# Genie-Kim/PintheMemory

Hardware: AMD Instinct MI355X
Metric: train imgs/sec 768x768 bs=8 R50-DeepLabV3+ +mem (higher is better)
Workload: dtype f32

## Files before the change

include/pinmem_hip.h:

```cpp
#ifndef PINMEM_HIP_H
#define PINMEM_HIP_H
#include <stddef.h>
#include <stdint.h>

#ifdef __cplusplus
extern "C" {
#endif

typedef enum pm_status { PM_OK = 0, PM_EINVAL = -1, PM_EWORKSPACE = -2, PM_ELAUNCH = -3, PM_EUNSUPPORTED = -4 } pm_status;

typedef enum pm_dtype { PM_F32 = 0, PM_BF16 = 1 } pm_dtype;
#define PM_TF_ZERO_PAD64 1

typedef struct pm_tensor {
  void* ptr;
  int32_t n, h, w, c;
  int64_t pitch;
  int32_t dtype;
  int32_t flags;
} pm_tensor;

#define PM_ABI_VERSION 410

typedef struct pm_conv_params {
  int32_t struct_size;
  int32_t kh, kw, stride, pad, dil;
  int32_t prec;
  void* wino_v;
  int64_t wino_v_bytes;
  void* wxf;
  int64_t wxf_bytes;
  int32_t wxf_valid;
} pm_conv_params;

typedef struct pm_conv_epilogue {
  int64_t struct_size;
  const float* bias;
  const float* scale;
  const float* shift;
  const float* residual;
  int64_t residual_pitch;
  int32_t relu;
  float* bn_partials;
  int64_t bn_partials_bytes;
} pm_conv_epilogue;

const char* pm_last_error(void);
int pm_version(void);

size_t pm_conv_workspace(const pm_tensor* x, const pm_tensor* y, const pm_conv_params* p, int which );
size_t pm_conv_winograd_v_bytes(const pm_tensor* x, const pm_tensor* y, const pm_conv_params* p);
size_t pm_conv_wxf_bytes(const pm_tensor* x, const pm_tensor* y, const pm_conv_params* p);
size_t pm_conv_wxf_bytes_dgrad(const pm_tensor* dy, const pm_tensor* dx, const pm_conv_params* p);
typedef struct pm_wxf_job {
  const float* w;
  void* wxf;
  int64_t wxf_bytes;
  int32_t cout, kh, kw, cin;
  int32_t dgrad;
  int32_t reserved;
} pm_wxf_job;
int pm_conv_wxf_refresh_bf16(const pm_wxf_job* jobs, int n, void* stream);
int pm_conv_wxf_refresh_f32(const pm_wxf_job* jobs, int n, void* stream);
size_t pm_conv_bn_partials_bytes(const pm_tensor* x, const pm_tensor* y, const pm_conv_params* p);
int pm_conv_fwd(const pm_tensor* x, const float* w_krsc, const pm_tensor* y, const pm_conv_params* p,
                const pm_conv_epilogue* ep, void* ws, size_t ws_bytes, void* stream);
int pm_conv_bwd_data(const pm_tensor* dy, const float* w_krsc, const pm_tensor* dx, const pm_conv_params* p,
                     const pm_tensor* add, void* ws, size_t ws_bytes, void* stream);
int pm_conv_bwd_data_masked(const pm_tensor* dy, const float* w_krsc, const pm_tensor* dx, const pm_conv_params* p,
                            const pm_tensor* add, const uint8_t* add_mask, void* ws, size_t ws_bytes, void* stream);
int pm_conv_bwd_weight(const pm_tensor* x, const pm_tensor* dy, float* dw_krsc, float* dbias, const pm_conv_params* p,
                       void* ws, size_t ws_bytes, void* stream);

typedef struct pm_routing {
  int32_t struct_size;
  int32_t winograd;
  int32_t winograd_fused;
  int32_t conv16;
  int32_t conv16_wide;
  int32_t conv16_persistent;
  int32_t wgrad16;
  int32_t bf16_wgrad;
  int32_t split;
} pm_routing;
int pm_routing_get(pm_routing* out);
int pm_routing_set(const pm_routing* r);


int pm_set_winograd(int mode);
int pm_set_winograd_fused(int on);
int pm_set_conv16(int on);
int pm_set_bf16_wgrad(int on);
int pm_set_wgrad16(int on);
int pm_set_split(int on);

int pm_profile_enable(int on);
int pm_profile_dump(const char* csv_path);
int pm_profile_read(int mode, int bm, int bn, int km, int nst, double* total_ms, double* total_flops, int64_t* launches, int clear);
int pm_profile_read_prec(int mode, int bm, int bn, int km, int nst, int prec, double* total_ms, double* total_flops, int64_t* launches, int clear);
int pm_profile_read_bytes(int mode, int bm, int bn, int km, int nst, int prec, double* total_bytes);

size_t pm_bn_workspace(const pm_tensor* x);
int pm_bn_stats(const pm_tensor* x, float* moments, void* ws, size_t ws_bytes, void* stream);
int pm_bn_stats_finalize(const pm_tensor* x, float eps, float* mean, float* invstd, float* running_mean , float* running_var ,
                         float momentum, void* ws, size_t ws_bytes, void* stream);
int pm_bn_merge(const float* parts, int world, int c, float* moments, void* stream);
int pm_bn_merge_finalize(const float* parts, int world, int c, float eps, float* mean, float* invstd, float* running_mean ,
                         float* running_var , float momentum, void* stream);
int pm_bn_finalize(const float* moments, int c, float eps, float* mean, float* invstd,
                   float* running_mean, float* running_var, float momentum, void* stream);
int pm_bn_apply(const pm_tensor* x, const float* mean, const float* invstd, const float* gamma, const float* beta,
                const pm_tensor* residual , int relu, const pm_tensor* y, void* stream);
int pm_bn_apply_mask(const pm_tensor* x, const float* mean, const float* invstd, const float* gamma, const float* beta,
                     const pm_tensor* residual , int relu, const pm_tensor* y, uint8_t* mask , void* stream);
int pm_bn_bwd_reduce_mask(const pm_tensor* dy, const uint8_t* mask, const pm_tensor* x, const float* mean, const float* invstd,
                          const pm_tensor* gmask , float* sums, void* ws, size_t ws_bytes, void* stream);
int pm_bn_apply_mask_affine(const pm_tensor* x, const float* mean, const float* invstd, const float* gamma, const float* beta,
                            const pm_tensor* r, const float* r_mean, const float* r_invstd, const float* r_gamma, const float* r_beta,
                            int relu, const pm_tensor* y, uint8_t* mask , void* stream);
int pm_bn_bwd_apply_mask(const pm_tensor* dy, const uint8_t* mask, const pm_tensor* x, const float* mean, const float* invstd, const float* gamma,
                         const float* sums, float count, const pm_tensor* dx, void* stream);
int pm_bn_bwd_reduce(const pm_tensor* dy, const pm_tensor* y , const pm_tensor* x, const float* mean, const float* invstd,
                     const float* gamma , const float* beta , int relu, const pm_tensor* gmask ,
                     float* sums, void* ws, size_t ws_bytes, void* stream);
int pm_bn_bwd_apply(const pm_tensor* dy, const pm_tensor* y , const pm_tensor* x, const float* mean, const float* invstd,
                    const float* gamma, const float* beta , const float* sums, float count, int relu, const pm_tensor* dx,
                    const pm_tensor* dres , void* stream);
int pm_bn_partials_finalize(const float* partials, int64_t pixels, int c, float eps, float* mean, float* invstd, float* running_mean ,
                            float* running_var , float momentum, float* moments , void* stream);
int pm_bn_fold(const float* gamma, const float* beta, const float* running_mean, const float* running_var, const float* conv_bias,
               int c, float eps, float* scale, float* shift, void* stream);
int pm_bn_fold_multi(const void* table, const int* cs, const int* offs, int n, int max_c, int total, float eps, float* arena, void* stream);
int pm_relu_bwd(const pm_tensor* dy, const pm_tensor* y, const pm_tensor* dx, void* stream);
int pm_add(const pm_tensor* a, const pm_tensor* b, const pm_tensor* y, void* stream);
int pm_add_n(const pm_tensor* const* xs, int n, const pm_tensor* y, void* stream);
int pm_copy(const pm_tensor* src, const pm_tensor* dst, void* stream);
int pm_scale_shift_act(const pm_tensor* x, const float* scale, const float* shift, const pm_tensor* residual, int relu,
                       const pm_tensor* y, void* stream);

int pm_cast(const pm_tensor* x, const pm_tensor* y, void* stream);

int pm_maxpool3x3s2_fwd(const pm_tensor* x, const pm_tensor* y, uint8_t* argmax, void* stream);
int pm_maxpool3x3s2_bwd(const pm_tensor* dy, const uint8_t* argmax, const pm_tensor* dx, void* stream);
int pm_maxpool3x3s2_bn_relu_fwd(const pm_tensor* x, const float* mean, const float* invstd, const float* gamma, const float* beta, const pm_tensor* y,
                                uint8_t* argmax, void* stream);
int pm_bn_bwd_reduce_pool(const pm_tensor* dy_pooled, const uint8_t* argmax, const pm_tensor* x, const float* mean, const float* invstd, const float* gamma,
                          const float* beta, float* sums, void* ws, size_t ws_bytes, void* stream);
int pm_bn_bwd_apply_pool(const pm_tensor* dy_pooled, const uint8_t* argmax, const pm_tensor* x, const float* mean, const float* invstd, const float* gamma,
                         const float* beta, const float* sums, float count, const pm_tensor* dx, void* stream);
int pm_global_avgpool_fwd(const pm_tensor* x, const pm_tensor* y , void* stream);
int pm_global_avgpool_bwd(const pm_tensor* dy, const pm_tensor* dx, int accumulate, void* stream);

int pm_resize_bilinear_fwd(const pm_tensor* x, const pm_tensor* y, void* stream);
int pm_resize_bilinear_bwd(const pm_tensor* dy, const pm_tensor* dx, int accumulate, void* stream);
size_t pm_resize_bilinear_bwd_workspace(const pm_tensor* dy, const pm_tensor* dx);
int pm_resize_bilinear_bwd_separable(const pm_tensor* dy, const pm_tensor* dx, int accumulate, void* ws, size_t ws_bytes, void* stream);

int pm_resize_bilinear_hp_fwd(const pm_tensor* x, const pm_tensor* y, int flip_w, void* stream);
int pm_softmax_mean_update(const pm_tensor* logits, double* buffer, int counter, void* stream);
int pm_sliding_stitch(const pm_tensor* logits, const int32_t* tiles_xyxy, int ntiles, int H, int W, int flip_w, double* acc, int accumulate, void* stream);
int pm_argmax_f64(const double* buffer, int n, int h, int w, int c, int64_t* out_cls, double* out_prob , void* stream);

int pm_image_u8_to_nhwc4(const uint8_t* img_nhw3, int64_t pixels, const float* mean3, const float* std3, float* out_nhwc4, void* stream);
int pm_labels_u8_to_i64(const uint8_t* lab, int64_t n, int64_t* out, void* stream);

typedef struct pm_aug_image {
  uint8_t order[4];
  uint8_t enabled;
  uint8_t flip;
  uint8_t hue_shift;
  uint8_t reserved;
  float brightness, contrast, saturation;
  int32_t radius;
  double w[6];
} pm_aug_image;
int pm_aug_blur_weights(double sigma, int32_t* radius, double* w6);
size_t pm_augment_workspace(int n);
int pm_augment_u8(const uint8_t* img_nhw3, int n, int H, int W, const pm_aug_image* params_dev, int32_t struct_size, const float* mean3, const float* std3,
                  float* out_nhwc4, uint8_t* out_u8, void* ws, size_t ws_bytes, void* stream);
int pm_labels_u8_flip_to_i64(const uint8_t* lab, int n, int H, int W, const pm_aug_image* params_dev, int32_t struct_size, int64_t* out, void* stream);

int pm_nchw_to_nhwc(const float* x_nchw, int c_src, const pm_tensor* y, void* stream);
int pm_nhwc_to_nchw(const pm_tensor* x, float* y_nchw, void* stream);
int pm_label_nearest(const int64_t* lab, int n, int H, int W, int64_t* out, int h, int w, void* stream);

// ... 69 lines not shown
```

pinthememory_amd/csrc/conv_igemm.hip:

```cpp
#include <stdlib.h>
#include <algorithm>
#include <type_traits>
#include <vector>

#include "pm_common.h"

#include "conv_igemm_kernel.h"

namespace {

template <int ZL, bool O16 = false>
__global__ __launch_bounds__(256) void splitk_reduce_vec_kernel(const float* __restrict__ ws, int ksplit, long slab, int M, int Nn,
                                                                float* __restrict__ C, long c_pitch, const float* bias,
                                                                const float* scale, const float* shift, const float* residual,
                                                                long res_pitch, int relu, const unsigned char* res_mask) {
  constexpr int GP = 256 / ZL;
  __shared__ float4 red[ZL > 1 ? ZL : 1][GP];
  const int gl = threadIdx.x % GP, zl = threadIdx.x / GP;
  const long groups = (long)M * Nn / 4;
  for (long g0 = (long)blockIdx.x * GP; g0 < groups; g0 += (long)gridDim.x * GP) {
    const long grp = g0 + gl;
    float4 v = make_float4(0.f, 0.f, 0.f, 0.f);
    if (grp < groups)
#pragma unroll 8
// ... 268 lines not shown
constexpr int NST1_MAX_STEPS = 64;
constexpr bool has_nst1(int mode, int kmode, int bn) { return mode != MODE_WGRAD && kmode == K_FAST && bn >= 64; }
inline int lds_stages(int mode, int kmode, int bn, int kper) { return has_nst1(mode, kmode, bn) && kper <= NST1_MAX_STEPS * BK ? 1 : 2; }
template <int MODE, int BM, int BN, int WM, int WN, int KM, int PREC>
void launch_prec(const ConvK& k, dim3 grid, size_t smem, hipStream_t st) {
  if constexpr (has_nst1(MODE, KM, BN)) {
    if (lds_stages(MODE, KM, BN, k.kper) == 1) return launch_nst<MODE, BM, BN, WM, WN, KM, PREC, 1>(k, grid, smem, st);
  }
  launch_nst<MODE, BM, BN, WM, WN, KM, PREC, 2>(k, grid, smem, st);
}
template <int MODE, int BM, int BN, int WM, int WN, int KM>
void launch_inst(const ConvK& k, dim3 grid, size_t smem, hipStream_t st) {
  if constexpr (MODE == MODE_FWD && KM == K_FAST && BN >= 64) {
    if (k.prec == 2) return launch_prec<MODE, BM, BN, WM, WN, KM, 2>(k, grid, smem, st);
  }
  if constexpr (MODE == MODE_WGRAD && BN >= 64) {
    if (k.prec == 3) return launch_prec<MODE, BM, BN, WM, WN, KM, 3>(k, grid, smem, st);
    if (k.prec == 4) return launch_prec<MODE, BM, BN, WM, WN, KM, 4>(k, grid, smem, st);
  }
  if (k.prec != 0) launch_prec<MODE, BM, BN, WM, WN, KM, 1>(k, grid, smem, st);
  else launch_prec<MODE, BM, BN, WM, WN, KM, 0>(k, grid, smem, st);
}
template <int MODE, int BM, int BN, int WM, int WN>
void launch_one(const ConvK& k, dim3 grid, size_t smem, hipStream_t st) {
  if (k.kmode == K_SMALL) launch_inst<MODE, BM, BN, WM, WN, K_SMALL>(k, grid, smem, st);
  else if (k.kmode == K_FAST && MODE != MODE_WGRAD) launch_inst<MODE, BM, BN, WM, WN, (MODE != MODE_WGRAD ? K_FAST : K_MID)>(k, grid, smem, st);
  else launch_inst<MODE, BM, BN, WM, WN, K_MID>(k, grid, smem, st);
}

struct ProfRec {
  hipEvent_t a, b;
  int mode, bm, bn, km, prec, nst;
  int M, Nn, K, batch, ksplit;
  double flops;
  double bytes;
};
bool g_prof_on = false;
std::vector<ProfRec> g_prof;
struct ProfScope {
  ProfRec rec{};
  hipStream_t st;
  ProfScope(hipStream_t st_, int mode, int bm, int bn, int km, int prec, int nst, long M, long Nn, long K, int batch, int ksplit, double flops, double bytes = 0.0) : st(st_) {
    if (!g_prof_on) return;
    (void)hipEventCreate(&rec.a), (void)hipEventCreate(&rec.b);
    rec.mode = mode, rec.bm = bm, rec.bn = bn, rec.km = km, rec.prec = prec, rec.nst = nst, rec.M = (int)M, rec.Nn = (int)Nn, rec.K = (int)K, rec.batch = batch, rec.ksplit = ksplit;
    rec.flops = flops, rec.bytes = bytes;
    (void)hipEventRecord(rec.a, st);
  }
  void done() {
    if (!g_prof_on) return;
    (void)hipEventRecord(rec.b, st);
    g_prof.push_back(rec);
  }
};

template <class K>
void set_epilogue(K& k, const pm_conv_epilogue& e) {
  k.bias = e.bias, k.scale = e.scale, k.shift = e.shift, k.residual = e.residual, k.res_pitch = e.residual_pitch, k.relu = e.relu;
}
inline void set_epilogue(ConvK& k, const pm_conv_epilogue& e, const unsigned char* res_mask) {
  set_epilogue(k, e);
  k.res_mask = res_mask, k.stats = e.bn_partials;
}
inline bool split_takes(int mode, const Plan& p, const ConvK& k, int batch) {
  return pm_route.split != 0 && p.bn >= 64 && !k.io16 && (batch > 1 || split_k_ok(mode, k.K));
}

template <int MODE>
int launch(const ConvK& k0, const Plan& p, hipStream_t st, int batch = 1, double flops = -1.0) {
  ConvK k = k0;
  k.tiles_m = p.tiles_m;
  k.tiles_n = p.tiles_n;
  k.ksplit = p.ksplit;
  k.kper = p.kper;
  dim3 grid(p.tiles_m * p.tiles_n, batch, p.ksplit);
  if (batch != 1) k.stage_ep = 0;
  if (k.prec == 0 && split_takes(MODE, p, k, batch)) k.prec = 5;
  {
    const int units = batch * p.ksplit, rem = units & 7, ntile = p.tiles_m * p.tiles_n;
    k.batch_xcd = units >= 8 && (rem == 0 || ((rem == 1 || rem == 2 || rem == 4) && ntile % (8 / rem) == 0));
  }
  const int km = (MODE == MODE_WGRAD && k.kmode == K_FAST) ? K_MID : ((k.prec == 5 && MODE != MODE_WGRAD && k.kmode == K_FAST && k.kh * k.kw == 1 && k.stride == 1 && k.pad == 0 && !k.sub) ? K_PW : k.kmode);
  ProfScope prof(st, MODE, p.bm, p.bn, km, k.prec, lds_stages(MODE, k.kmode, p.bn, k.kper), k.M, k.Nn, k.K, batch, p.ksplit,
                 flops >= 0.0 ? flops : 2.0 * (double)k.M * (double)k.Nn * (double)k.K * batch,
                 (double)batch * ((double)k.a_bytes + (double)k.b_bytes + ((k.io16 && p.ksplit == 1) ? 2.0 : 4.0) * (double)k.M * (double)k.Nn * (double)p.ksplit));
  if constexpr (MODE != MODE_WGRAD) {
    if (pm_route.split && (k.prec == 0 || k.prec == 5) && !k.io16 && batch == 1 && p.ksplit == 1 && !k.stats && k.kh * k.kw == 1 && k.stride == 1 && k.pad == 0 && !k.sub) {
      pm_gemm_pw g;
      g.A = k.A, g.B = k.B, g.C = k.C, g.res_mask = k.res_mask;
      set_epilogue(g, pm_conv_epilogue{(int64_t)sizeof(pm_conv_epilogue), k.bias, k.scale, k.shift, k.residual, k.res_pitch, k.relu, nullptr, 0});
      g.a_pitch = MODE == MODE_FWD ? k.x_pitch : k.y_pitch, g.c_pitch = k.c_pitch;
      g.b_sn = MODE == MODE_FWD ? k.K : 1, g.b_sk = MODE == MODE_FWD ? 1 : k.Nn;
      g.M = k.M, g.Nn = k.Nn, g.K = k.K;
      if (pm_pwstream_ok(&g)) {
        prof.rec.bm = 32, prof.rec.bn = 64, prof.rec.km = 4, prof.rec.prec = 5, prof.rec.nst = 0;
        const int e = pm_pwstream_launch(&g, st);
        prof.done();
        return e;
      }
    }
  }
  constexpr bool akc = MODE != MODE_WGRAD, bkc = MODE == MODE_FWD;
  if (k.prec == 5) {
    if (int e = pm_conv_split_launch(MODE, p.bm, p.bn, k, grid.x, grid.y, grid.z, pm_conv_split_stage_bytes(MODE, p.bm, p.bn), st)) return e;
    prof.rec.nst = 1;
    prof.done();
    return pm_check_launch("conv_split");
  }
  const bool tr = MODE == MODE_WGRAD && (k.prec == 3 || k.prec == 4) && p.bn >= 64;
  auto smem = [&](int bm, int bn) {
    if (tr) return (size_t)2 * ((k.prec == 4 ? 2 : 1) * BK * (bm + 32) + (k.prec == 4 ? 2 : 1) * BK * (bn + 32)) * 2;
    return (size_t)2 * ((akc ? bm * LDK : BK * bm) + (bkc ? bn * LDK : BK * bn)) * sizeof(float);
  };
  if (p.bm == 64) {
    if (p.bn == 128) launch_one<MODE, 64, 128, 2, 2>(k, grid, smem(64, 128), st);
    else launch_one<MODE, 64, 64, 2, 2>(k, grid, smem(64, 64), st);
  } else if (p.bn == 128) {
    launch_one<MODE, 128, 128, 2, 2>(k, grid, smem(128, 128), st);
  } else if (p.bn == 64) {
    launch_one<MODE, 128, 64, 2, 2>(k, grid, smem(128, 64), st);
  } else {
    launch_one<MODE, 128, 32, 4, 1>(k, grid, smem(128, 32), st);
  }
  prof.done();
  return pm_check_launch("conv_igemm");
}

template <int MODE>
int run_gemm(ConvK& k, const Plan& pl, float* slab, float* out, long out_pitch, const pm_conv_epilogue& e, hipStream_t st, double flops = -1.0,
             const unsigned char* res_mask = nullptr) {
  return run_planned(pl.ksplit, k.M, k.Nn, slab, out, out_pitch, e, k.io16 != 0, res_mask, st, [&](float* C, bool slabs) {
    k.C = C, k.c_pitch = slabs ? k.Nn : out_pitch, k.c_split = slabs ? (long)k.M * k.Nn : 0;
    if (!slabs) set_epilogue(k, e, res_mask);
    return launch<MODE>(k, pl, st, 1, flops);
  });
}

int check_common(const pm_tensor* x, const pm_tensor* y, const pm_conv_params* p) {
  PM_REQUIRE(x && y && p && x->ptr && y->ptr, PM_EINVAL, "conv: null tensor");
  PM_REQUIRE(p->struct_size == (int32_t)sizeof(pm_conv_params), PM_EINVAL, "conv: pm_conv_params.struct_size %d != %zu -- caller built against another pinmem_hip.h (library ABI %d)",
             p->struct_size, sizeof(pm_conv_params), PM_ABI_VERSION);
  PM_REQUIRE(p->kh >= 1 && p->kw >= 1 && p->dil >= 1 && p->pad >= 0, PM_EINVAL, "conv: bad geometry");
  PM_REQUIRE(p->stride == 1 || p->stride == 2, PM_EUNSUPPORTED, "conv: stride %d unsupported (1 or 2)", p->stride);
  const int ho = (x->h + 2 * p->pad - p->dil * (p->kh - 1) - 1) / p->stride + 1;
  const int wo = (x->w + 2 * p->pad - p->dil * (p->kw - 1) - 1) / p->stride + 1;
  PM_REQUIRE(ho == y->h && wo == y->w && x->n == y->n, PM_EINVAL, "conv: output %dx%d does not match geometry (%dx%d)", y->h, y->w, ho, wo);
  PM_REQUIRE((x->dtype == PM_F32 || x->dtype == PM_BF16) && (y->dtype == PM_F32 || y->dtype == PM_BF16), PM_EUNSUPPORTED, "conv: dtype %d / %d", x->dtype, y->dtype);
  for (const pm_tensor* t : {x, y}) {
    if (pm_is_bf16(t)) PM_REQUIRE(pm_vec8(t), PM_EINVAL, "conv: bf16 tensors must be 16B aligned with pitch %% 8 == 0 and channels %% 8 == 0");
    else PM_REQUIRE(pm_vec_ok(t), PM_EINVAL, "conv: tensors must be 16B aligned with pitch %% 4 == 0");
  }
  PM_REQUIRE(x->c % 4 == 0, PM_EUNSUPPORTED, "conv: Cin %% 4 != 0 unsupported (pad the input channels)");
  PM_REQUIRE((y->c % 4 == 0) || (p->kh * p->kw == 1), PM_EUNSUPPORTED, "conv: Cout %% 4 != 0 only for 1x1");
  PM_REQUIRE(x->pitch >= x->c && y->pitch >= y->c, PM_EINVAL, "conv: pitch < channels");
  PM_REQUIRE(pm_pixels(x) * x->pitch < (1ll << 29) && pm_pixels(y) * y->pitch < (1ll << 29) && (int64_t)y->c * x->c * p->kh * p->kw < (1ll << 29),
             PM_EUNSUPPORTED, "conv: tensor too large for 32-bit byte offsets (2 GiB per tensor)");
  return PM_OK;
}

void fill_geom(ConvK& k, const pm_tensor* x, const pm_tensor* y, const pm_conv_params* p) {
  k.N = x->n, k.H = x->h, k.W = x->w, k.Cin = x->c, k.x_pitch = x->pitch;
  k.Ho = y->h, k.Wo = y->w, k.Cout = y->c, k.y_pitch = y->pitch;
  k.kh = p->kh, k.kw = p->kw, k.stride = p->stride, k.pad = p->pad, k.dil = p->dil;
  k.sshift = p->stride == 2 ? 1 : 0;
  k.prec = p->prec != 0 ? 1 : 0;
  k.T_eff = p->kh * p->kw, k.tk_w = p->kw, k.ky0 = k.kx0 = 0, k.ksy = k.ksx = 1;
  k.sub = k.sub_cy = k.sub_cx = 0, k.Hc = x->h, k.Wc = x->w;
  k.bias = k.scale = k.shift = k.residual = nullptr;
  k.res_pitch = 0, k.res_mask = nullptr, k.relu = 0, k.stats = nullptr, k.io16 = 0;
  k.stage_ep = 1;
  k.spl_prio = 1;
  k.n_group = 8;
  k.batch_xcd = 0;
  k.a_bs = k.b_bs = k.c_bs = 0;
}

struct WinoPlan {
  bool use;
  pm_wino_geom g;
  int Kp, P;
  size_t v_bytes, m_bytes, u_bytes;
  Plan pl;
};
inline bool wino_wgrad_pays(int cin, int cout) { return (long)cin * cout >= 256 * 256; }
WinoPlan wino_plan(const pm_tensor* xin, int cout, const pm_conv_params* p, bool wgrad = false) {
  WinoPlan wp{};
  if (wgrad && !wino_wgrad_pays(xin->c, cout)) return wp;
  if (pm_route.winograd == 0 || p->kh != 3 || p->kw != 3 || p->stride != 1 || p->pad != p->dil || p->prec != 0) return wp;
  const int cin = xin->c;
  if (cin < 128 || cout < 128 || (cout & 3) || (cin & 3)) return wp;
  int m = 0;
  double best_ratio = 0.6;
  for (int cand = pm_route.winograd; cand >= 2; cand -= 2) {
    const pm_wino_geom g = pm_wino_make_geom(xin->n, xin->h, xin->w, p->dil, cand);
    const double cover = (double)(cand * g.TY * p->dil) * (double)(cand * g.TX * p->dil) / ((double)xin->h * xin->w);
    const double ratio = cover * (cand + 2) * (cand + 2) / (9.0 * cand * cand);
    if (ratio <= best_ratio) best_ratio = ratio, m = cand, wp.g = g;
  }
  if (!m) return wp;
  wp.P = (m + 2) * (m + 2);
  wp.Kp = (cin + BK - 1) / BK * BK;
  if (wp.g.tiles * (long)std::max(wp.Kp, cout) * 4 >= (1ll << 31)) return wp;
  wp.v_bytes = pm_align_up((size_t)wp.P * wp.g.tiles * wp.Kp * sizeof(float), 256);
  wp.m_bytes = pm_align_up((size_t)wp.P * wp.g.tiles * cout * sizeof(float), 256);
  wp.u_bytes = pm_align_up((size_t)wp.P * cout * wp.Kp * sizeof(float), 256);
  wp.pl.bm = 128, wp.pl.bn = 128;
  if (pm_cdiv(cout, 128) * 128 > cout * 1.12 && pm_cdiv(cout, 64) * 64 < pm_cdiv(cout, 128) * 128) wp.pl.bn = 64;
  if (wp.g.tiles <= 4608 && !pm_route.split) wp.pl.bm = 64;
  wp.pl.tiles_m = pm_cdiv(wp.g.tiles, wp.pl.bm), wp.pl.tiles_n = pm_cdiv(cout, wp.pl.bn);
  wp.pl.ksplit = 1, wp.pl.kper = wp.Kp, wp.pl.ws_bytes = 0;
  wp.use = true;
  return wp;
}
inline size_t wino_ws(const WinoPlan& wp) { return wp.v_bytes + wp.m_bytes + wp.u_bytes; }

int wino_conv(const pm_tensor* xin, const float* w, int w_cout, int w_cin, bool dgrad, const pm_tensor* yout, const WinoPlan& wp,
              const pm_conv_epilogue& ep, void* ws, hipStream_t st, float* v_keep = nullptr, float* u_ext = nullptr, bool u_valid = false) {
  float* V = v_keep ? v_keep : (float*)ws;
  float* Mo = (float*)((char*)ws + wp.v_bytes);
  float* U = u_ext ? u_ext : (float*)((char*)ws + wp.v_bytes + wp.m_bytes);
  const int cout = yout->c;
  if (int e = pm_wino_input_xf((const float*)xin->ptr, xin->pitch, xin->c, wp.Kp, wp.g, V, st)) return e;
  if (!(u_ext && u_valid))
    if (int e = pm_wino_filter_xf(w, w_cout, w_cin, wp.Kp, dgrad, wp.g.m, U, st)) return e;
  const pm_tensor xv = {V, 1, 1, (int32_t)wp.g.tiles, wp.Kp, wp.Kp};
  const pm_tensor yv = {Mo, 1, 1, (int32_t)wp.g.tiles, cout, cout};
  const pm_conv_params p1 = {(int32_t)sizeof(pm_conv_params), 1, 1, 1, 0, 1, 0};
  ConvK k;
  fill_geom(k, &xv, &yv, &p1);
  k.A = V, k.B = U, k.C = Mo;
  k.M = (int)wp.g.tiles, k.Nn = cout, k.K = wp.Kp;
  k.a_bytes = (unsigned)(wp.g.tiles * wp.Kp * 4), k.b_bytes = (unsigned)((long)cout * wp.Kp * 4), k.kmode = K_FAST;
  k.c_pitch = cout, k.c_split = 0;
  k.a_bs = wp.g.tiles * wp.Kp, k.b_bs = (long)cout * wp.Kp, k.c_bs = wp.g.tiles * cout;
  if (pm_route.winograd_fused && wp.g.m == 4 && wp.Kp % 16 == 0) {
    ProfScope prof(st, 3, 32, 32, 0, 0, 1, wp.g.tiles, cout, wp.Kp, wp.P, 1, 2.0 * wp.P * (double)wp.g.tiles * cout * xin->c);
    const int e = pm_wino_fused_f4(V, U, cout, wp.Kp, wp.g, (float*)yout->ptr, yout->pitch, ep.bias, ep.scale, ep.shift, ep.residual, ep.residual_pitch, ep.relu, st);
    prof.done();
    return e;
  }
  if (int e = launch<MODE_FWD>(k, wp.pl, st, wp.P, 2.0 * wp.P * (double)wp.g.tiles * cout * xin->c)) return e;
  return pm_wino_output_xf(Mo, cout, wp.g, (float*)yout->ptr, yout->pitch, ep.bias, ep.scale, ep.shift, ep.residual, ep.residual_pitch, ep.relu, st);
}

struct WinoWgradPlan {
  Plan pl;
  size_t slab_bytes;
};
WinoWgradPlan wino_wgrad_plan(const WinoPlan& wp, int cout) {
  WinoWgradPlan q{};
  q.pl.bm = 128, q.pl.bn = 128;
  if (pm_cdiv(wp.Kp, 128) * 128 > wp.Kp * 1.12 && pm_cdiv(wp.Kp, 64) * 64 < pm_cdiv(wp.Kp, 128) * 128) q.pl.bn = 64;
  q.pl.tiles_m = pm_cdiv(cout, 128), q.pl.tiles_n = pm_cdiv(wp.Kp, q.pl.bn);
  const long ksteps = (wp.g.tiles + BK - 1) / BK;
  const long per_split = (long)q.pl.tiles_m * q.pl.tiles_n * wp.P;
  long ks = std::max<long>(1, std::min<long>((768 + per_split / 2) / per_split, ksteps / 8));
  const long steps_per = (ksteps + ks - 1) / ks;
  ks = (ksteps + steps_per - 1) / steps_per;
  q.pl.ksplit = (int)ks, q.pl.kper = (int)(steps_per * BK), q.pl.ws_bytes = 0;
  q.slab_bytes = pm_align_up((size_t)ks * wp.P * cout * wp.Kp * sizeof(float), 256);
  return q;
}
inline size_t wino_wgrad_ws(const WinoPlan& wp, const WinoWgradPlan& q) { return wp.v_bytes + wp.m_bytes + q.slab_bytes; }

int wino_wgrad(const pm_tensor* x, const pm_tensor* dy, float* dw, const WinoPlan& wp, const WinoWgradPlan& q, void* ws, hipStream_t st,
               float* v_kept = nullptr) {
  float* V = v_kept ? v_kept : (float*)ws;
  float* Z = (float*)((char*)ws + wp.v_bytes);
  float* slab = (float*)((char*)ws + wp.v_bytes + wp.m_bytes);
  const int cout = dy->c;
  if (!v_kept)
    if (int e = pm_wino_input_xf((const float*)x->ptr, x->pitch, x->c, wp.Kp, wp.g, V, st)) return e;
  if (int e = pm_wino_dy_xf((const float*)dy->ptr, dy->pitch, cout, wp.g, Z, st)) return e;
  const pm_tensor xv = {V, 1, 1, (int32_t)wp.g.tiles, wp.Kp, wp.Kp};
  const pm_tensor zv = {Z, 1, 1, (int32_t)wp.g.tiles, cout, cout};
  const pm_conv_params p1 = {(int32_t)sizeof(pm_conv_params), 1, 1, 1, 0, 1, 0};
  ConvK k;
  fill_geom(k, &xv, &zv, &p1);
  k.A = Z, k.B = V, k.C = slab;
  k.M = cout, k.Nn = wp.Kp, k.K = (int)wp.g.tiles;
  k.a_bytes = (unsigned)(wp.g.tiles * cout * 4), k.b_bytes = (unsigned)(wp.g.tiles * wp.Kp * 4), k.kmode = K_MID;
  k.c_pitch = wp.Kp, k.c_split = (long)wp.P * cout * wp.Kp;
  k.a_bs = wp.g.tiles * cout, k.b_bs = wp.g.tiles * wp.Kp, k.c_bs = (long)cout * wp.Kp;
  if (int e = launch<MODE_WGRAD>(k, q.pl, st, wp.P, 2.0 * wp.P * (double)wp.g.tiles * cout * x->c)) return e;
  return pm_wino_dw_xf(slab, q.pl.ksplit, cout, x->c, wp.Kp, wp.g.m, dw, st);
}

struct Bf16Plan {
  bool use;
  bool c16;
  pm_conv16 k16;
  bool inplace;
  int Cp;
  long M, Nn, Kf;
  size_t xb_bytes, wb_bytes;
  Plan pl;
};
Bf16Plan bf16_plan(const pm_tensor* xin, const pm_tensor* yout, const pm_conv_params* p) {
  Bf16Plan b{};
  if ((p->prec != 2 && !pm_is_bf16(xin) && !pm_is_bf16(yout)) || xin->c < 32) return b;
  b.Cp = (xin->c + 63) / 64 * 64;
  const long T = (long)p->kh * p->kw;
  b.M = pm_pixels(yout), b.Nn = yout->c, b.Kf = T * b.Cp / 2;
  b.inplace = pm_is_bf16(xin) && (xin->c % 64 == 0 || ((xin->flags & PM_TF_ZERO_PAD64) && xin->pitch >= b.Cp));
  const size_t xb = b.inplace ? (size_t)pm_pixels(xin) * xin->pitch * 2 : (size_t)pm_pixels(xin) * b.Cp * 2, wb = (size_t)yout->c * T * b.Cp * 2;
  if (xb >= (1ull << 31) || wb >= (1ull << 31)) return b;
  b.xb_bytes = b.inplace ? 0 : pm_align_up(xb, 256), b.wb_bytes = pm_align_up(wb, 256);
  b.pl = make_plan(MODE_FWD, b.M, b.Nn, b.Kf, true);
  if (b.pl.bn < 64) return b;
  b.use = true;
  constexpr long C16_MIN_M = 256;
  b.c16 = false;
  if (pm_route.conv16 && b.M >= C16_MIN_M && p->stride >= 1) {
    pm_conv16& k = b.k16;
    k = pm_conv16{};
    k.N = xin->n, k.H = xin->h, k.W = xin->w, k.Ho = yout->h, k.Wo = yout->w;
    k.a_pitch = b.inplace ? xin->pitch : b.Cp, k.Cp = b.Cp;
    k.kh = p->kh, k.kw = p->kw, k.stride = p->stride, k.pad = p->pad, k.dil = p->dil;
    k.M = (int)b.M, k.Nn = (int)b.Nn, k.K = (int)(T * b.Cp), k.ksteps = k.K / 64;
    k.c_pitch = yout->pitch, k.c_f32 = pm_is_bf16(yout) ? 0 : 1;
    pm_conv16_plan(&k);
    b.c16 = pm_route.conv16 == 2 || k.wide || k.bm == 64 || k.ksteps_per == 1 || (b.pl.bm == 64 && k.ksteps >= 16);
  }
  return b;
}
inline size_t bf16_ws(const Bf16Plan& b) {
  return b.xb_bytes + b.wb_bytes + std::max(pm_align_up(b.pl.ws_bytes, 256), b.c16 ? pm_conv16_slab_bytes(&b.k16) : (size_t)0);
}

int conv_bf16(const pm_tensor* xin, const float* w, int w_cout, int w_cin, bool rotate, const pm_tensor* yout, const pm_conv_params* pe, const Bf16Plan& b,
              const pm_conv_epilogue& e0, void* ws, hipStream_t st, char* wb_ext = nullptr, bool wb_valid = false) {
  char* xb = b.inplace ? (char*)xin->ptr : (char*)ws;
  char* wb = wb_ext ? wb_ext : (char*)ws + b.xb_bytes;
  float* slab = (float*)((char*)ws + b.xb_bytes + b.wb_bytes);
  const int T = pe->kh * pe->kw;
  if (!b.inplace) {
    if (pm_is_bf16(xin)) {
      if (int e = pm16_pad_rows((const pm_bf16*)xin->ptr, xin->pitch, xin->c, b.Cp, pm_pixels(xin), (pm_bf16*)xb, st)) return e;
    } else if (int e = pm_bf16_cast_rows((const float*)xin->ptr, xin->pitch, xin->c, b.Cp, pm_pixels(xin), xb, st)) return e;
  }
  if (!(wb_ext && wb_valid))
    if (int e = pm_bf16_cast_weights(w, w_cout, T, w_cin, b.Cp, rotate, wb, st)) return e;
  const long xpitch16 = b.inplace ? xin->pitch : b.Cp;
  if (b.c16) {
    const bool o16 = pm_is_bf16(yout);
    const bool ok = (!e0.bn_partials || o16) &&
                    (o16 ? ((yout->c | yout->pitch | (e0.residual ? e0.residual_pitch : 0)) & 7) == 0 && pm_aligned16(yout->ptr) && pm_aligned16(e0.residual)
                         : !(e0.scale || e0.residual || e0.relu));
    if (ok) {
      pm_conv16 k = b.k16;
      k.A = (const pm_bf16*)xb, k.B = (const pm_bf16*)wb;
      const double fl = 2.0 * (double)b.M * (double)b.Nn * (double)T * (double)xin->c * (g_prof_on ? pm_conv16_executed_fraction(&k) : 1.0);
      ProfScope prof(st, k.wide ? 5 : 4, k.bm, k.bn, pm_conv16w_persistent(&k), 5, k.wide ? 3 : (k.ksteps_per == 1 ? 1 : 2), k.M, k.Nn, k.K / 2, 1, k.ksplit, fl);
      return run_planned(k.ksplit, b.M, b.Nn, slab, (float*)yout->ptr, (long)yout->pitch, e0, o16, nullptr, st, [&](float* C, bool slabs) {
        k.C = C;
        if (!slabs) set_epilogue(k, e0), k.stats = o16 ? e0.bn_partials : nullptr;
        const int e = pm_conv16_launch(&k, st);
        prof.done();
        return e;
      });
    }
  }
  const pm_tensor xv = {xb, xin->n, xin->h, xin->w, b.Cp / 2, xpitch16 / 2};
  ConvK k;
  fill_geom(k, &xv, yout, pe);
  k.prec = 2;
  k.A = (const float*)xb, k.B = (const float*)wb;
  k.M = (int)b.M, k.Nn = (int)b.Nn, k.K = (int)b.Kf;
  k.a_bytes = (unsigned)((size_t)pm_pixels(xin) * xpitch16 * 2), k.b_bytes = (unsigned)((size_t)yout->c * T * b.Cp * 2), k.kmode = K_FAST;
  const double flops = 2.0 * (double)b.M * (double)b.Nn * (double)T * (double)xin->c;
  k.io16 = pm_is_bf16(yout) ? 1 : 0;
  return run_gemm<MODE_FWD>(k, b.pl, slab, (float*)yout->ptr, (long)yout->pitch, e0, st, flops);
}
inline pm_conv_params dgrad_as_fwd(const pm_conv_params* p) {
  pm_conv_params q = *p;
// ... 356 lines not shown
  *out = pm_route;
  return PM_OK;
}
extern "C" int pm_routing_set(const pm_routing* r) {
  PM_REQUIRE(r && r->struct_size == (int32_t)sizeof(pm_routing), PM_EINVAL, "pm_routing_set: struct_size %d != %zu (library ABI %d)", r ? r->struct_size : -1, sizeof(pm_routing),
             PM_ABI_VERSION);
  PM_REQUIRE(r->winograd == 0 || r->winograd == 2 || r->winograd == 4, PM_EINVAL, "pm_routing_set: winograd %d (0, 2 or 4)", r->winograd);
  PM_REQUIRE(r->conv16 >= 0 && r->conv16 <= 2 && r->conv16_wide >= 0 && r->conv16_wide <= 3, PM_EINVAL, "pm_routing_set: conv16 %d / conv16_wide %d", r->conv16, r->conv16_wide);
  pm_route = *r;
  return PM_OK;
}
extern "C" int pm_set_winograd(int mode) {
  PM_REQUIRE(mode == 0 || mode == 2 || mode == 4, PM_EINVAL, "pm_set_winograd: mode %d (0 off, 2 F(2x2,3x3), 4 prefer F(4x4,3x3))", mode);
  pm_route.winograd = mode;
  return PM_OK;
}
extern "C" int pm_set_conv16(int on) {
  PM_REQUIRE(on >= 0 && on <= 8, PM_EINVAL, "pm_set_conv16: %d (0 register-staged, 1 per shape, 2 LDS-DMA everywhere / narrow tiles only, 3 LDS-DMA everywhere / wide tiles "
             "wherever the shape allows, 4 per shape without the wide kernel, 5 / 6 = 1 (the streaming 1x1 kernel left the library in round 6), 7 as 3 with the 256 x 256 tile, "
             "8 as 3 with one block per tile instead of the persistent ring)", on);
  pm_route.conv16 = (on == 3 || on == 7 || on == 8) ? 2 : ((on == 4 || on == 5 || on == 6) ? 1 : on);
  pm_route.conv16_wide = (on == 3 || on == 8) ? 2 : (on == 7 ? 3 : ((on == 2 || on == 4) ? 0 : pm_route_defaults.conv16_wide));
  pm_route.conv16_persistent = on == 8 ? 0 : (on == 3 ? 1 : pm_route_defaults.conv16_persistent);
  return PM_OK;
}
extern "C" int pm_set_winograd_fused(int on) {
  pm_route.winograd_fused = on != 0;
  return PM_OK;
}
extern "C" int pm_set_wgrad16(int on) {
  pm_route.wgrad16 = on != 0;
  return PM_OK;
}
extern "C" int pm_set_split(int on) {
  pm_route.split = on ? 1 : 0;
  return PM_OK;
}
extern "C" int pm_set_bf16_wgrad(int on) {
  pm_route.bf16_wgrad = on != 0;
  return PM_OK;
}
extern "C" int pm_profile_enable(int on) {
  g_prof_on = on != 0;
  return PM_OK;
}
extern "C" int pm_profile_read_prec(int mode, int bm, int bn, int km, int nst, int prec, double* total_ms, double* total_flops, int64_t* launches, int clear);
extern "C" int pm_profile_read(int mode, int bm, int bn, int km, int nst, double* total_ms, double* total_flops, int64_t* launches, int clear) {
  return pm_profile_read_prec(mode, bm, bn, km, nst, -1, total_ms, total_flops, launches, clear);
}
extern "C" int pm_profile_read_prec(int mode, int bm, int bn, int km, int nst, int prec, double* total_ms, double* total_flops, int64_t* launches, int clear) {
  double ms = 0.0, fl = 0.0;
  int64_t n = 0;
  for (const ProfRec& r : g_prof) {
    if ((mode >= 0 && r.mode != mode) || (bm >= 0 && r.bm != bm) || (bn >= 0 && r.bn != bn) || (km >= 0 && r.km != km) || (nst >= 0 && r.nst != nst) ||
        (prec >= 0 && r.prec != prec))
      continue;
    float t = 0.f;
    if (hipEventSynchronize(r.b) != hipSuccess || hipEventElapsedTime(&t, r.a, r.b) != hipSuccess) continue;
    ms += t, fl += r.flops, ++n;
  }
  if (clear) {
    for (const ProfRec& r : g_prof) (void)hipEventDestroy(r.a), (void)hipEventDestroy(r.b);
    g_prof.clear();
  }
  if (total_ms) *total_ms = ms;
  if (total_flops) *total_flops = fl;
  if (launches) *launches = n;
  return PM_OK;
}

extern "C" int pm_profile_read_bytes(int mode, int bm, int bn, int km, int nst, int prec, double* total_bytes) {
  double b = 0.0;
  for (const ProfRec& r : g_prof) {
    if ((mode >= 0 && r.mode != mode) || (bm >= 0 && r.bm != bm) || (bn >= 0 && r.bn != bn) || (km >= 0 && r.km != km) || (nst >= 0 && r.nst != nst) ||
        (prec >= 0 && r.prec != prec))
      continue;
    b += r.bytes;
  }
  if (total_bytes) *total_bytes = b;
  return PM_OK;
}

extern "C" int pm_profile_dump(const char* path) {
  PM_REQUIRE(path, PM_EINVAL, "pm_profile_dump: null path");
  FILE* f = fopen(path, "w");
  PM_REQUIRE(f, PM_EINVAL, "pm_profile_dump: cannot open %s", path);
  fprintf(f, "mode,bm,bn,km,nst,prec,M,N,K,batch,ksplit,ms,gflop\n");
  for (const ProfRec& r : g_prof) {
    float t = 0.f;
    if (hipEventSynchronize(r.b) != hipSuccess || hipEventElapsedTime(&t, r.a, r.b) != hipSuccess) continue;
    fprintf(f, "%d,%d,%d,%d,%d,%d,%d,%d,%d,%d,%d,%.5f,%.4f\n", r.mode, r.bm, r.bn, r.km, r.nst, r.prec, r.M, r.Nn, r.K, r.batch, r.ksplit, t, r.flops * 1e-9);
  }
  fclose(f);
  return PM_OK;
}

extern "C" size_t pm_conv_workspace(const pm_tensor* x, const pm_tensor* y, const pm_conv_params* p0, int which) {
  const pm_conv_params tp = tier_params(p0, x, y);
  return route_conv(which, x, y, &tp).ws_bytes;
}
extern "C" size_t pm_conv_winograd_v_bytes(const pm_tensor* x, const pm_tensor* y, const pm_conv_params* p0) {
  if (!x || !y || !p0) return 0;
  const pm_conv_params tp = tier_params(p0, x, y);
  return route_conv(MODE_FWD, x, y, &tp).v_keep_bytes;
}
extern "C" size_t pm_conv_wxf_bytes(const pm_tensor* x, const pm_tensor* y, const pm_conv_params* p0) {
  if (!x || !y || !p0) return 0;
  const pm_conv_params tp = tier_params(p0, x, y);
  return route_conv(MODE_FWD, x, y, &tp).wxf_bytes;
}
extern "C" size_t pm_conv_wxf_bytes_dgrad(const pm_tensor* dy, const pm_tensor* dx, const pm_conv_params* p0) {
  if (!dy || !dx || !p0) return 0;
  const pm_conv_params tp = tier_params(p0, dy, dx);
  return route_conv(MODE_DGRAD, dx, dy, &tp).wxf_bytes;
}
extern "C" size_t pm_conv_bn_partials_bytes(const pm_tensor* x, const pm_tensor* y, const pm_conv_params* p0) {
  if (!x || !y || !p0 || check_common(x, y, p0) != PM_OK) return 0;
  const pm_conv_params tp = tier_params(p0, x, y);
  return route_conv(MODE_FWD, x, y, &tp).bn_bytes;
}

extern "C" int pm_conv_wxf_refresh_f32(const pm_wxf_job* jobs, int n, void* stream) {
  PM_REQUIRE(n >= 0 && (jobs || n == 0), PM_EINVAL, "conv_wxf_refresh_f32: bad job table");
  std::vector<const float*> w(n);
  std::vector<float*> U(n);
  std::vector<int> cout(n), cin(n), kp(n), m(n);
  for (int i = 0; i < n; ++i) {
    const pm_wxf_job& q = jobs[i];
    PM_REQUIRE(q.w && q.wxf && q.cout > 0 && q.cin > 0 && q.kh == 3 && q.kw == 3 && q.dgrad == 0, PM_EINVAL,
               "conv_wxf_refresh_f32: job %d: forward transforms of 3x3 filters only", i);
    PM_REQUIRE(pm_aligned16(q.wxf), PM_EINVAL, "conv_wxf_refresh_f32: job %d: buffer must be 16-byte aligned", i);
    const int Kp = (q.cin + BK - 1) / BK * BK;
    const size_t u4 = pm_align_up((size_t)36 * q.cout * Kp * sizeof(float), 256), u2 = pm_align_up((size_t)16 * q.cout * Kp * sizeof(float), 256);
    PM_REQUIRE((size_t)q.wxf_bytes == u4 || (size_t)q.wxf_bytes == u2, PM_EINVAL, "conv_wxf_refresh_f32: job %d: %ld bytes is neither the F(4x4) nor the F(2x2) transform of %d x %d",
               i, (long)q.wxf_bytes, q.cout, q.cin);
    w[i] = q.w, U[i] = (float*)q.wxf, cout[i] = q.cout, cin[i] = q.cin, kp[i] = Kp, m[i] = (size_t)q.wxf_bytes == u4 ? 4 : 2;
  }
  return pm_wino_filter_xf_multi(w.data(), U.data(), cout.data(), cin.data(), kp.data(), m.data(), n, (hipStream_t)stream);
}

extern "C" int pm_conv_fwd(const pm_tensor* x, const float* w, const pm_tensor* y, const pm_conv_params* p0,
                           const pm_conv_epilogue* ep, void* ws, size_t ws_bytes, void* stream) {
  if (int e = check_common(x, y, p0)) return e;
  const pm_conv_params tp = tier_params(p0, x, y);
  const pm_conv_params* p = &tp;
  PM_REQUIRE(!ep || ep->struct_size == (int64_t)sizeof(pm_conv_epilogue), PM_EINVAL,
             "conv_fwd: pm_conv_epilogue.struct_size %ld != %zu -- caller built against another pinmem_hip.h (library ABI %d)", ep ? (long)ep->struct_size : 0l,
             sizeof(pm_conv_epilogue), PM_ABI_VERSION);
  PM_REQUIRE(w && pm_aligned16(w), PM_EINVAL, "conv_fwd: weight null or unaligned");
  pm_conv_epilogue e0 = {(int64_t)sizeof(pm_conv_epilogue), nullptr, nullptr, nullptr, nullptr, 0, 0};
  if (ep) e0 = *ep;
  PM_REQUIRE((e0.scale == nullptr) == (e0.shift == nullptr), PM_EINVAL, "conv_fwd: scale and shift go together");
  const ConvRoute r = route_conv(MODE_FWD, x, y, p);
  if (e0.bn_partials) {
    PM_REQUIRE(!e0.relu && !e0.residual, PM_EINVAL, "conv_fwd: bn_partials are the statistics of the convolution output (no residual / ReLU)");
    PM_REQUIRE(r.bn_bytes != 0 && (size_t)e0.bn_partials_bytes >= r.bn_bytes, PM_EINVAL, "conv_fwd: this call cannot emit bn_partials (ask pm_conv_bn_partials_bytes): %zu needed", r.bn_bytes);
  }
  PM_REQUIRE(ws_bytes >= r.ws_bytes && (ws || r.ws_bytes == 0), PM_EWORKSPACE, "conv_fwd: workspace %zu < %zu", ws_bytes, r.ws_bytes);
  hipStream_t st = (hipStream_t)stream;
  switch (r.kind) {
    case R_WINO: {
      float* keep = (p->wino_v && (size_t)p->wino_v_bytes >= r.wino.v_bytes) ? (float*)p->wino_v : nullptr;
      float* uext = (p->wxf && (size_t)p->wxf_bytes >= r.wino.u_bytes) ? (float*)p->wxf : nullptr;
      return wino_conv(x, w, y->c, x->c, false, y, r.wino, e0, ws, st, keep, uext, p->wxf_valid != 0);
    }
    case R_BF16: {
      char* wext = (p->wxf && (size_t)p->wxf_bytes >= r.b16.wb_bytes) ? (char*)p->wxf : nullptr;
      return conv_bf16(x, w, y->c, x->c, false, y, &r.pe, r.b16, e0, ws, st, wext, p->wxf_valid != 0);
    }
    default:
      PM_REQUIRE(pm_is_f32(x), PM_EUNSUPPORTED, "conv_fwd: a bf16 input needs at least 32 channels (got %d)", x->c);
      return conv_direct<MODE_FWD>(x, y, w, p, r.pl, e0, ws, st);
  }
}

extern "C" int pm_conv_bwd_data(const pm_tensor* dy, const float* w, const pm_tensor* dx, const pm_conv_params* p0, const pm_tensor* add,
                                void* ws, size_t ws_bytes, void* stream) {
  return pm_conv_bwd_data_masked(dy, w, dx, p0, add, nullptr, ws, ws_bytes, stream);
}

extern "C" int pm_conv_bwd_data_masked(const pm_tensor* dy, const float* w, const pm_tensor* dx, const pm_conv_params* p0, const pm_tensor* add,
                                       const uint8_t* add_mask, void* ws, size_t ws_bytes, void* stream) {
  if (int e = check_common(dx, dy, p0)) return e;
  const pm_conv_params tp = tier_params(p0, dy, dx);
  const pm_conv_params* p = &tp;
  PM_REQUIRE(!add || (add->ptr && pm_same_shape(add, dx) && add->dtype == dx->dtype), PM_EINVAL, "conv_bwd_data: `add` must match dx (shape and dtype)");
  PM_REQUIRE(!add || !pm_is_bf16(add) || pm_vec8(add), PM_EINVAL, "conv_bwd_data: bf16 `add` must be 16B aligned with pitch %% 8 == 0");
  PM_REQUIRE(w && pm_aligned16(w), PM_EINVAL, "conv_bwd_data: weight null or unaligned");
  const ConvRoute r = route_conv(MODE_DGRAD, dx, dy, p);
  PM_REQUIRE(ws_bytes >= r.ws_bytes && (ws || r.ws_bytes == 0), PM_EWORKSPACE, "conv_bwd_data: workspace %zu < %zu", ws_bytes, r.ws_bytes);
  if (add_mask) {
    PM_REQUIRE(add && pm_is_f32(add) && pm_is_f32(dy) && pm_vec4(add) && pm_vec4(dx), PM_EINVAL, "conv_bwd_data: a masked `add` is an fp32 tensor with 16-byte rows and c %% 4 == 0");
    PM_REQUIRE(r.kind == R_DIRECT, PM_EUNSUPPORTED,
               "conv_bwd_data: a masked `add` is served by the fp32 implicit-GEMM route only (this call routes to %s)",
               r.kind == R_WINO ? "Winograd" : (r.kind == R_BF16 ? "the bf16 kernels" : "the stride-2 class kernels"));
  }
  hipStream_t st = (hipStream_t)stream;
  const pm_conv_epilogue e1 = {(int64_t)sizeof(pm_conv_epilogue), nullptr, nullptr, nullptr, add ? (const float*)add->ptr : nullptr, add ? add->pitch : 0, 0};
  switch (r.kind) {
    case R_S2_NATIVE: return dgrad_s2_bf16(dy, w, dx, p, add, r.s2n, ws, st);
    case R_S2_PARITY: return dgrad_s2_parity(dy, w, dx, p, add, r, ws, st);
    case R_BF16: {
      char* wext = (p->wxf && (size_t)p->wxf_bytes >= r.b16.wb_bytes) ? (char*)p->wxf : nullptr;
      return conv_bf16(dy, w, dy->c, dx->c, true, dx, &r.pe, r.b16, e1, ws, st, wext, p->wxf_valid != 0);
    }
    case R_WINO: return wino_conv(dy, w, dy->c, dx->c, true, dx, r.wino, e1, ws, st);
    default:
      PM_REQUIRE(pm_is_f32(dy), PM_EUNSUPPORTED, "conv_bwd_data: a bf16 dy needs at least 32 channels and a stride-1 geometry the forward form covers");
      return conv_direct<MODE_DGRAD>(dx, dy, w, p, r.pl, e1, ws, st, add_mask);
  }
}

extern "C" int pm_conv_bwd_weight(const pm_tensor* x0, const pm_tensor* dy0, float* dw, float* dbias, const pm_conv_params* p0, void* ws,
                                  size_t ws_bytes, void* stream) {
  if (int e = check_common(x0, dy0, p0)) return e;
  const pm_conv_params tp = tier_params(p0, x0, dy0);
  const pm_conv_params* p = &tp;
  PM_REQUIRE(dw && pm_aligned16(dw), PM_EINVAL, "conv_bwd_weight: dw null or unaligned");
  const ConvRoute r = route_conv(MODE_WGRAD, x0, dy0, p);
  PM_REQUIRE(ws && ws_bytes >= r.ws_bytes, PM_EWORKSPACE, "conv_bwd_weight: workspace %zu < %zu", ws_bytes, r.ws_bytes);
  hipStream_t st = (hipStream_t)stream;
  const pm_tensor *x = x0, *dy = dy0;
  pm_tensor x32, dy32;
  if (!r.native16 && pm_is_bf16(x0)) {
    if (int e = upcast(x0, (char*)ws + r.x32_off, &x32, st)) return e;
    x = &x32;
  }
  if (pm_is_bf16(dy0) && (!r.native16 || dbias)) {
    if (int e = upcast(dy0, (char*)ws + r.dy32_off, &dy32, st)) return e;
    if (!r.native16) dy = &dy32;
  }
  int e;
  switch (r.kind) {
    case R_BF16_WGRAD: e = conv_wgrad_bf16(x, dy, dw, p, r.b16w, ws, st); break;
    case R_WINO_WGRAD: e = wino_wgrad(x, dy, dw, r.wino, r.wino_w, ws, st, (p->wino_v && (size_t)p->wino_v_bytes >= r.wino.v_bytes) ? (float*)p->wino_v : nullptr); break;
    default: e = conv_wgrad_direct(x, dy, dw, p, r, ws, st);
  }
  if (e || !dbias) return e;
  const pm_tensor* dyb = pm_is_bf16(dy0) ? &dy32 : dy0;
  const long P = pm_pixels(dyb);
  const int rpb = colsum_rows(P, dyb->c), nb = pm_cdiv(P, rpb);
  float* part = (float*)((char*)ws + r.bias_off);
  if (dyb->pitch == ((dyb->c + 3) & ~3) && dyb->pitch <= 64 && pm_aligned16(dyb->ptr))
    hipLaunchKernelGGL(colsum_partial_narrow_kernel, dim3(nb), dim3(256), 0, st, (const float*)dyb->ptr, (int)(dyb->pitch / 4), P, dyb->c, rpb, part);
  else
    hipLaunchKernelGGL(colsum_partial_kernel, dim3(nb, pm_cdiv(dyb->c, 64)), dim3(256), 0, st, (const float*)dyb->ptr, (long)dyb->pitch, P, dyb->c, rpb, part);
  hipLaunchKernelGGL(colsum_final_kernel, dim3(pm_cdiv(dyb->c, 64)), dim3(1024), 0, st, (const float*)part, nb, dyb->c, dbias);
  return pm_check_launch("conv_bias_grad");
}
```

pinthememory_amd/csrc/pm_common.h:

```cpp
#pragma once
#include <hip/hip_runtime.h>
#include <algorithm>
#include <atomic>
#include <stdarg.h>
#include <stdint.h>
#include <stdio.h>

#include "../../include/pinmem_hip.h"

void pm_set_error(const char* fmt, ...);

#define PM_REQUIRE(cond, code, ...)      \
  do {                                   \
    if (!(cond)) {                       \
      pm_set_error(__VA_ARGS__);         \
      return (code);                     \
    }                                    \
  } while (0)

static inline int pm_check_launch(const char* what) {
  hipError_t e = hipGetLastError();
  if (e != hipSuccess) {
    pm_set_error("%s: launch failed: %s", what, hipGetErrorString(e));
    return PM_ELAUNCH;
  }
  return PM_OK;
}

static inline bool pm_aligned16(const void* p) { return (reinterpret_cast<uintptr_t>(p) & 15u) == 0; }
static inline int64_t pm_pixels(const pm_tensor* t) { return (int64_t)t->n * t->h * t->w; }
static inline int pm_cdiv(int64_t a, int64_t b) { return (int)((a + b - 1) / b); }
static inline size_t pm_align_up(size_t v, size_t a) { return (v + a - 1) / a * a; }

static inline bool pm_vec_ok(const pm_tensor* t) { return pm_aligned16(t->ptr) && (t->pitch % 4) == 0; }
static inline bool pm_is_f32(const pm_tensor* t) { return t->dtype == PM_F32; }
static inline bool pm_is_bf16(const pm_tensor* t) { return t->dtype == PM_BF16; }
#define PM_REQUIRE_F32(t, who) PM_REQUIRE(!(t) || pm_is_f32(t), PM_EUNSUPPORTED, "%s: fp32 tensors only (got dtype %d)", who, (t)->dtype)
static inline bool pm_vec8(const pm_tensor* t) { return pm_is_bf16(t) && pm_aligned16(t->ptr) && (t->pitch % 8) == 0 && (t->c % 8) == 0; }

struct pm_wino_geom {
  int N, H, W, d, m, TY, TX;
  long tiles;
};
pm_wino_geom pm_wino_make_geom(int n, int h, int w, int d, int m);
int pm_wino_input_xf(const float* x, long pitch, int C, int Kp, const pm_wino_geom& g, float* V, hipStream_t st);
int pm_wino_filter_xf(const float* w, int Cout, int Cin, int Kp, bool dgrad, int m, float* U, hipStream_t st);
int pm_wino_filter_xf_multi(const float* const* w, float* const* U, const int* cout, const int* cin, const int* kp, const int* m, int n, hipStream_t st);
int pm_wino_output_xf(const float* M, int Cout, const pm_wino_geom& g, float* y, long ypitch, const float* bias, const float* scale, const float* shift,
                      const float* residual, long res_pitch, int relu, hipStream_t st);
int pm_wino_fused_f4(const float* V, const float* U, int Cout, int Kp, const pm_wino_geom& g, float* y, long ypitch, const float* bias, const float* scale,
                     const float* shift, const float* residual, long res_pitch, int relu, hipStream_t st);
int pm_wino_dy_xf(const float* dy, long pitch, int Cout, const pm_wino_geom& g, float* Z, hipStream_t st);
int pm_wino_dw_xf(const float* slab, int ks, int Cout, int Cin, int Kp, int m, float* dw, hipStream_t st);

int pm_bf16_cast_rows(const float* x, long pitch, int C, int Cp, long P, void* out, hipStream_t st);
int pm_bf16_cast_weights(const float* w, int Cout, int T, int Cin, int Cp, bool rotate, void* out, hipStream_t st);
struct PmS2Classes {
  int ky0[4], nky[4], kx0[4], nkx[4];
  void* out[4];
};
int pm_bf16_cast_weights_s2(const float* w, int Cout, int kh, int kw, int Cin, int Cp, const PmS2Classes* cl, hipStream_t st);
int pm_bf16_transpose_taps(const float* x, long pitch, int C, int N, int H, int W, int Ho, int Wo, int kh, int kw, int stride, int pad, int dil, void* out,
                           hipStream_t st);

typedef unsigned short pm_bf16;
int pm16_to_f32(const pm_bf16* x, long pitch, int C, long P, float* out, long out_pitch, hipStream_t st);
int pm16_pad_rows(const pm_bf16* x, long pitch, int C, int Cp, long P, pm_bf16* out, hipStream_t st);

struct pm_conv16 {
  const pm_bf16* A;
  const pm_bf16* B;
  void* C;
  int N, H, W, Ho, Wo;
  long a_pitch;
  int Cp;
  int kh, kw, stride, pad, dil;
  int M, Nn, K, ksteps;
  long c_pitch;
  int c_f32;
  const float *bias, *scale, *shift;
  const void* residual;
  long res_pitch;
  int relu;
  float* stats;
  int bm, bn, tiles_m, tiles_n, ksplit, ksteps_per;
  long c_split;
  int wide;
};
void pm_conv16_plan(pm_conv16* k);
int pm_conv16w_launch(const pm_conv16* k, hipStream_t st);
int pm_conv16w_persistent(const pm_conv16* k);
size_t pm_conv16_slab_bytes(const pm_conv16* k);
double pm_conv16_executed_fraction(const pm_conv16* k);
int pm_conv16_launch(const pm_conv16* k, hipStream_t st);

struct pm_wgrad16 {
  const pm_bf16* X;
  const pm_bf16* DY;
  float* C;
  int N, H, W, Ho, Wo;
  long x_pitch, dy_pitch;
  int Cin, Cout, kh, kw, stride, pad, dil;
  int M, Nn, P;
  int kper, ksplit;
  long c_split;
  int bm, bn, tiles_m, tiles_n;
};
bool pm_wgrad16_plan(pm_wgrad16* k);
int pm_wgrad16_launch(const pm_wgrad16* k, hipStream_t st);

struct pm_gemm_pw {
  const float* A;
  const float* B;
  float* C;
  const float *bias, *scale, *shift, *residual;
  const unsigned char* res_mask;
  long a_pitch, c_pitch, res_pitch;
  int b_sn, b_sk;
  long M;
  int Nn, K, relu;
};
bool pm_pwstream_ok(const pm_gemm_pw* g);
int pm_pwstream_launch(const pm_gemm_pw* g, hipStream_t st);

constexpr int PM_MAX_DEVICES = 64;
inline int pm_device_cus(int dev) {
  static std::atomic<int> cached[PM_MAX_DEVICES];
  const bool keep = dev >= 0 && dev < PM_MAX_DEVICES;
  int n = keep ? cached[dev].load(std::memory_order_relaxed) : 0;
  if (n > 0) return n;
  if (hipDeviceGetAttribute(&n, hipDeviceAttributeMultiprocessorCount, dev) != hipSuccess || n <= 0) n = 256;
  if (keep) cached[dev].store(n, std::memory_order_relaxed);
  return n;
}
struct pm_lds_optin {
  std::atomic<bool> done[PM_MAX_DEVICES] = {};
  int operator()(const void* kernel, int lds_bytes) {
    int dev = 0;
    if (hipGetDevice(&dev) != hipSuccess) dev = 0;
    const bool keep = dev >= 0 && dev < PM_MAX_DEVICES;
    if (!keep || !done[dev].load(std::memory_order_acquire)) {
      if (hipFuncSetAttribute(kernel, hipFuncAttributeMaxDynamicSharedMemorySize, lds_bytes) != hipSuccess) (void)hipGetLastError();
      else if (keep) done[dev].store(true, std::memory_order_release);
    }
    return pm_device_cus(dev);
  }
};

extern pm_routing pm_route;


__device__ __forceinline__ int pm_xcd_remap(int bid, int nwg) {
  const int q = nwg >> 3, r = nwg & 7, xcd = bid & 7, idx = bid >> 3;
  const int base = xcd < r ? xcd * (q + 1) : r * (q + 1) + (xcd - r) * q;
  return base + idx;
}
__device__ __forceinline__ void pm_ld8(const pm_bf16* p, float* v) {
  const uint4 q = *reinterpret_cast<const uint4*>(p);
  v[0] = __uint_as_float(q.x << 16), v[1] = __uint_as_float(q.x & 0xffff0000u), v[2] = __uint_as_float(q.y << 16), v[3] = __uint_as_float(q.y & 0xffff0000u);
  v[4] = __uint_as_float(q.z << 16), v[5] = __uint_as_float(q.z & 0xffff0000u), v[6] = __uint_as_float(q.w << 16), v[7] = __uint_as_float(q.w & 0xffff0000u);
}
__device__ __forceinline__ unsigned pm_pack_bf16(float a, float b) {
  typedef __bf16 bf16x2_t __attribute__((ext_vector_type(2)));
  bf16x2_t o;
  o[0] = (__bf16)a, o[1] = (__bf16)b;
  return __builtin_bit_cast(unsigned, o);
}
__device__ __forceinline__ void pm_st8(pm_bf16* p, const float* v) {
  uint4 q;
  q.x = pm_pack_bf16(v[0], v[1]), q.y = pm_pack_bf16(v[2], v[3]), q.z = pm_pack_bf16(v[4], v[5]), q.w = pm_pack_bf16(v[6], v[7]);
  *reinterpret_cast<uint4*>(p) = q;
}
__device__ __forceinline__ float pm_bf16_to_f32(pm_bf16 h) { return __uint_as_float((unsigned)h << 16); }
__device__ __forceinline__ pm_bf16 pm_f32_to_bf16(float f) { return __builtin_bit_cast(unsigned short, (__bf16)f); }

template <int LDC, int LPR, int RPI>
__device__ __forceinline__ void pm_slab_stats16(const float* Ws, int rr0, int cc, long slab_row0, long M, long Nn, int col, bool cok, const float* bi, const float* sc,
                                                const float* sh, float* stats) {
  const float cnt = (float)max(0l, min(32l, M - slab_row0));
  float s1[8], mu[8], m2[8];
#pragma unroll
  for (int e = 0; e < 8; ++e) s1[e] = 0.f, m2[e] = 0.f;
  auto slab_row = [&](int r0, float* v) {
    const float4 v0 = *reinterpret_cast<const float4*>(Ws + (r0 + rr0) * LDC + cc), v1 = *reinterpret_cast<const float4*>(Ws + (r0 + rr0) * LDC + cc + 4);
    const float t[8] = {v0.x, v0.y, v0.z, v0.w, v1.x, v1.y, v1.z, v1.w};
#pragma unroll
    for (int e = 0; e < 8; ++e) v[e] = pm_bf16_to_f32(pm_f32_to_bf16((t[e] + bi[e]) * sc[e] + sh[e]));
    return slab_row0 + r0 + rr0 < M;
  };
#pragma unroll
  for (int r0 = 0; r0 < 32; r0 += RPI) {
    float v[8];
    const bool rok = slab_row(r0, v);
#pragma unroll
    for (int e = 0; e < 8; ++e) s1[e] += rok ? v[e] : 0.f;
  }
#pragma unroll
  for (int o = LPR; o < 64; o <<= 1)
// ... 215 lines not shown
```

pinthememory_amd/csrc/winograd.hip:

```cpp
#include "pm_common.h"

namespace {

enum { W_BT = 0, W_AT = 1, W_G = 2, W_A = 3, W_GT = 4 };

template <int MT>
__host__ __device__ constexpr float wino_bt(int i, int j) {
  if (MT == 2) {
    constexpr float t[4][4] = {{1, 0, -1, 0}, {0, 1, 1, 0}, {0, -1, 1, 0}, {0, 1, 0, -1}};
    return t[i & 3][j & 3];
  }
  constexpr float t[6][6] = {{4, 0, -5, 0, 1, 0}, {0, -4, -4, 1, 1, 0}, {0, 4, -4, -1, 1, 0}, {0, -2, -1, 2, 1, 0}, {0, 2, -1, -2, 1, 0}, {0, 4, 0, -5, 0, 1}};
  return t[i][j];
}
template <int MT>
__host__ __device__ constexpr float wino_at(int i, int j) {
  if (MT == 2) {
    constexpr float t[2][4] = {{1, 1, 1, 0}, {0, 1, -1, -1}};
    return t[i & 1][j & 3];
  }
  constexpr float t[4][6] = {{1, 1, 1, 1, 1, 0}, {0, 1, -1, 2, -2, 0}, {0, 1, 1, 4, 4, 0}, {0, 1, -1, 8, -8, 1}};
  return t[i][j];
}
template <int MT>
__host__ __device__ constexpr float wino_g(int i, int j) {
  if (MT == 2) {
    constexpr float t[4][3] = {{1, 0, 0}, {0.5f, 0.5f, 0.5f}, {0.5f, -0.5f, 0.5f}, {0, 0, 1}};
    return t[i & 3][j];
  }
  constexpr float t[6][3] = {{1.f / 4, 0, 0},          {-1.f / 6, -1.f / 6, -1.f / 6}, {-1.f / 6, 1.f / 6, -1.f / 6},
                             {1.f / 24, 1.f / 12, 1.f / 6}, {1.f / 24, -1.f / 12, 1.f / 6},  {0, 0, 1}};
  return t[i][j];
}
template <int MT, int WHICH>
__host__ __device__ constexpr float wino_coef(int r, int c) {
  return WHICH == W_BT ? wino_bt<MT>(r, c) : WHICH == W_AT ? wino_at<MT>(r, c) : WHICH == W_G ? wino_g<MT>(r, c) : WHICH == W_A ? wino_at<MT>(c, r) : wino_g<MT>(c, r);
}

template <int W>
struct Vec {
  float v[W];
};
template <int W>
__device__ __forceinline__ Vec<W> vzero() {
  Vec<W> r;
#pragma unroll
  for (int i = 0; i < W; ++i) r.v[i] = 0.f;
  return r;
}
template <int W>
__device__ __forceinline__ Vec<W> vload(const float* p) {
  Vec<W> r;
  if constexpr (W == 4) {
    const float4 q = PM_LD4(p);
    r.v[0] = q.x, r.v[1] = q.y, r.v[2] = q.z, r.v[3] = q.w;
  } else if constexpr (W == 2) {
    const float2 q = *reinterpret_cast<const float2*>(p);
    r.v[0] = q.x, r.v[1] = q.y;
  } else {
    r.v[0] = *p;
  }
  return r;
}
template <int W>
__device__ __forceinline__ void vstore(float* p, const Vec<W>& r) {
  if constexpr (W == 4) PM_ST4(p, make_float4(r.v[0], r.v[1], r.v[2], r.v[3]));
  else if constexpr (W == 2) *reinterpret_cast<float2*>(p) = make_float2(r.v[0], r.v[1]);
  else *p = r.v[0];
}

template <int MT, int WHICH, int R, int C, int W>
__device__ __forceinline__ void mat_apply(const Vec<W> (&in)[C], Vec<W> (&out)[R]) {
#pragma unroll
  for (int r = 0; r < R; ++r) {
    Vec<W> acc = vzero<W>();
    bool first = true;
#pragma unroll
    for (int c = 0; c < C; ++c) {
      const float k = wino_coef<MT, WHICH>(r, c);
      if (k == 0.f) continue;
#pragma unroll
      for (int i = 0; i < W; ++i) {
        if (first) acc.v[i] = k == 1.f ? in[c].v[i] : (k == -1.f ? -in[c].v[i] : k * in[c].v[i]);
        else if (k == 1.f) acc.v[i] += in[c].v[i];
        else if (k == -1.f) acc.v[i] -= in[c].v[i];
        else acc.v[i] = fmaf(k, in[c].v[i], acc.v[i]);
      }
      first = false;
    }
    out[r] = acc;
  }
}

struct TileId {
  int n, ry, rx, ty, tx;
};
__device__ __forceinline__ TileId decode_tile(unsigned tile, const pm_wino_geom& g) {
  TileId t;
  t.tx = (int)(tile % (unsigned)g.TX);
  unsigned q = tile / (unsigned)g.TX;
  t.ty = (int)(q % (unsigned)g.TY);
  q /= (unsigned)g.TY;
  t.rx = (int)(q % (unsigned)g.d);
  q /= (unsigned)g.d;
  t.ry = (int)(q % (unsigned)g.d);
  t.n = (int)(q / (unsigned)g.d);
  return t;
}

template <int MT, int W>
__global__ __launch_bounds__(256) void wino_input_kernel(const float* __restrict__ x, long xp, int C, int Kp, const pm_wino_geom g, float* __restrict__ V) {
  constexpr int A = MT + 2;
  const unsigned kg = Kp / W;
  const unsigned total = (unsigned)g.tiles * kg;
  const long plane = g.tiles * (long)Kp;
  for (unsigned i = blockIdx.x * 256u + threadIdx.x; i < total; i += gridDim.x * 256u) {
    const unsigned tile = i / kg;
    const int c = (int)(i - tile * kg) * W;
    const TileId t = decode_tile(tile, g);
    const bool cok = c < C;
    Vec<W> tt[A][A];
#pragma unroll
    for (int b = 0; b < A; ++b) {
      const int xx = t.rx + g.d * (MT * t.tx + b - 1);
      const bool xok = cok && (unsigned)xx < (unsigned)g.W;
      Vec<W> col[A], o[A];
#pragma unroll
      for (int a = 0; a < A; ++a) {
        const int yy = t.ry + g.d * (MT * t.ty + a - 1);
        col[a] = (xok && (unsigned)yy < (unsigned)g.H) ? vload<W>(x + ((long)(t.n * g.H + yy) * g.W + xx) * xp + c) : vzero<W>();
      }
      mat_apply<MT, W_BT>(col, o);
#pragma unroll
      for (int a = 0; a < A; ++a) tt[a][b] = o[a];
    }
    float* out = V + (long)tile * Kp + c;
#pragma unroll
    for (int a = 0; a < A; ++a) {
      Vec<W> o[A];
      mat_apply<MT, W_BT>(tt[a], o);
#pragma unroll
      for (int b = 0; b < A; ++b) vstore<W>(out + (a * A + b) * plane, o[b]);
    }
  }
}

template <int MT, int W>
__global__ __launch_bounds__(256) void wino_output_kernel(const float* __restrict__ M, int Cout, const pm_wino_geom g, float* __restrict__ y, long yp,
                                                          const float* __restrict__ bias, const float* __restrict__ scale,
                                                          const float* __restrict__ shift, const float* __restrict__ residual, long rp, int relu) {
  constexpr int A = MT + 2;
  const unsigned cg = Cout / W;
  const unsigned total = (unsigned)g.tiles * cg;
  const long plane = g.tiles * (long)Cout;
  for (unsigned i = blockIdx.x * 256u + threadIdx.x; i < total; i += gridDim.x * 256u) {
    const unsigned tile = i / cg;
    const int c = (int)(i - tile * cg) * W;
    const TileId t = decode_tile(tile, g);
    const float* in = M + (long)tile * Cout + c;
    Vec<W> s[MT][A];
#pragma unroll
    for (int b = 0; b < A; ++b) {
      Vec<W> col[A], o[MT];
#pragma unroll
      for (int a = 0; a < A; ++a) col[a] = vload<W>(in + (a * A + b) * plane);
      mat_apply<MT, W_AT>(col, o);
#pragma unroll
      for (int a = 0; a < MT; ++a) s[a][b] = o[a];
    }
    Vec<W> bi = vzero<W>(), sc = vzero<W>(), sh = vzero<W>();
    if (bias) bi = vload<W>(bias + c);
    if (scale) sc = vload<W>(scale + c), sh = vload<W>(shift + c);
#pragma unroll
    for (int a = 0; a < MT; ++a) {
      const int yy = t.ry + g.d * (MT * t.ty + a);
      Vec<W> o[MT];
      mat_apply<MT, W_AT>(s[a], o);
#pragma unroll
      for (int b = 0; b < MT; ++b) {
        const int xx = t.rx + g.d * (MT * t.tx + b);
        if (yy >= g.H || xx >= g.W) continue;
        const long pix = (long)(t.n * g.H + yy) * g.W + xx;
        Vec<W> v = o[b];
        if (bias) {
#pragma unroll
          for (int q = 0; q < W; ++q) v.v[q] += bi.v[q];
        }
        if (scale) {
#pragma unroll
          for (int q = 0; q < W; ++q) v.v[q] = v.v[q] * sc.v[q] + sh.v[q];
        }
        if (residual) {
          const Vec<W> rr = vload<W>(residual + pix * rp + c);
#pragma unroll
          for (int q = 0; q < W; ++q) v.v[q] += rr.v[q];
        }
        if (relu) {
#pragma unroll
          for (int q = 0; q < W; ++q) v.v[q] = fmaxf(v.v[q], 0.f);
        }
        vstore<W>(y + pix * yp + c, v);
      }
    }
  }
}

template <int MT, bool DGRAD>
__device__ __forceinline__ void wino_filter_block(const float* __restrict__ w, int Cout, int Cin, int Kp, float* __restrict__ U, int bx, int by,
                                                  float (*sg)[32][33]) {
  constexpr int A = MT + 2;
  const int tx = threadIdx.x & 31, ty = threadIdx.x >> 5;
  const int R = DGRAD ? Cin : Cout;
  const int Kr = DGRAD ? Cout : Cin;
  const int r0 = by * 32, k0 = bx * 32;
  const int co0 = DGRAD ? k0 : r0, ci0 = DGRAD ? r0 : k0;
  for (int j = ty; j < 32; j += 8) {
    const int co = co0 + j, ci = ci0 + tx;
    const bool ok = co < Cout && ci < Cin;
#pragma unroll
    for (int tap = 0; tap < 9; ++tap) sg[tap][j][tx] = ok ? w[((long)co * 9 + tap) * Cin + ci] : 0.f;
  }
  __syncthreads();
  const long plane = (long)R * Kp;
  const int j = threadIdx.x >> 3, q = threadIdx.x & 7;
  const int row = r0 + j, k = k0 + 4 * q;
  if (row >= R || k >= Kp) return;
  Vec<4> gg[A][3];
#pragma unroll
  for (int kx = 0; kx < 3; ++kx) {
    Vec<4> col[3], o[A];
#pragma unroll
    for (int ky = 0; ky < 3; ++ky)
#pragma unroll
      for (int e = 0; e < 4; ++e) col[ky].v[e] = DGRAD ? sg[(2 - ky) * 3 + (2 - kx)][4 * q + e][j] : sg[ky * 3 + kx][j][4 * q + e];
    mat_apply<MT, W_G>(col, o);
#pragma unroll
    for (int a = 0; a < A; ++a) gg[a][kx] = o[a];
  }
  float* out = U + (long)row * Kp + k;
#pragma unroll
  for (int a = 0; a < A; ++a) {
    Vec<4> o[A];
    mat_apply<MT, W_G>(gg[a], o);
#pragma unroll
    for (int b = 0; b < A; ++b) {
#pragma unroll
      for (int e = 0; e < 4; ++e)
        if (k + e >= Kr) o[b].v[e] = 0.f;
      vstore<4>(out + (a * A + b) * plane, o[b]);
    }
  }
}
template <int MT, bool DGRAD>
__global__ __launch_bounds__(256) void wino_filter_kernel(const float* __restrict__ w, int Cout, int Cin, int Kp, float* __restrict__ U) {
  __shared__ float sg[9][32][33];
  wino_filter_block<MT, DGRAD>(w, Cout, Cin, Kp, U, blockIdx.x, blockIdx.y, sg);
}

constexpr int WR_BATCH = 48;
struct WinoRefreshJobs {
  const float* w[WR_BATCH];
  float* U[WR_BATCH];
  int cout[WR_BATCH], cin[WR_BATCH], kp[WR_BATCH], m[WR_BATCH];
  int start[WR_BATCH + 1];
  int n;
};
__global__ __launch_bounds__(256) void wino_filter_multi_kernel(const WinoRefreshJobs t) {
  __shared__ float sg[9][32][33];
  int j = 0;
  while (j + 1 < t.n && (int)blockIdx.x >= t.start[j + 1]) ++j;
  const int local = (int)blockIdx.x - t.start[j];
  const int nbx = t.kp[j] / 32;
  const int bx = local % nbx, by = local / nbx;
  if (t.m[j] == 4) wino_filter_block<4, false>(t.w[j], t.cout[j], t.cin[j], t.kp[j], t.U[j], bx, by, sg);
  else wino_filter_block<2, false>(t.w[j], t.cout[j], t.cin[j], t.kp[j], t.U[j], bx, by, sg);
}

template <int MT, int W>
__global__ __launch_bounds__(256) void wino_dy_kernel(const float* __restrict__ dy, long yp, int Cout, const pm_wino_geom g, float* __restrict__ Z) {
  constexpr int A = MT + 2;
  const unsigned cg = Cout / W;
  const unsigned total = (unsigned)g.tiles * cg;
  const long plane = g.tiles * (long)Cout;
// ... 70 lines not shown
  const float* V;
  const float* U;
  float* y;
  long yp;
  int Cout, Kp;
  pm_wino_geom g;
  const float* bias;
  const float* scale;
  const float* shift;
  const float* residual;
  long rp;
  int relu;
  int ncb;
};

constexpr int WF_THREADS = 768, WF_TB = 32, WF_CB = 32, WF_BK = 16, WF_P = 36;
constexpr size_t WF_LDS = (size_t)WF_P * WF_TB * (WF_CB + 1) * sizeof(float);

__global__ __launch_bounds__(WF_THREADS) void wino_fused_f4_kernel(const WinoFusedArgs a) {
  extern __shared__ __align__(16) float4 lds4[];
  const int tid = threadIdx.x, lane = tid & 63, wave = tid >> 6;
  const int lid = pm_xcd_remap(blockIdx.x, gridDim.x);
  const int tb = lid / a.ncb, cb = lid - tb * a.ncb;
  const long tile0 = (long)tb * WF_TB;
  const int co0 = cb * WF_CB;

  const int rem = tid & 255, row = rem >> 2, chunk = rem & 3, pgrp = tid >> 8;
  const bool is_a = row < WF_TB;
  bool valid;
  const float* gp;
  long plane;
  if (is_a) {
    const long tile = tile0 + row;
    valid = tile < a.g.tiles;
    gp = a.V + (valid ? tile : 0) * a.Kp + chunk * 4;
    plane = a.g.tiles * (long)a.Kp;
  } else {
    const int co = co0 + row - WF_TB;
    valid = co < a.Cout;
    gp = a.U + (long)(valid ? co : 0) * a.Kp + chunk * 4;
    plane = (long)a.Cout * a.Kp;
  }
  gp += (long)pgrp * plane;
  const long pstep = 3 * plane;
  const int ldsw = pgrp * 256 + row * 4 + (chunk ^ ((row >> 2) & 3));
  float4 r[12];
  auto gload = [&](int k0) {
#pragma unroll
    for (int it = 0; it < 12; ++it) r[it] = valid ? PM_LD4(gp + it * pstep + k0) : make_float4(0.f, 0.f, 0.f, 0.f);
  };
  auto lstore = [&]() {
#pragma unroll
    for (int it = 0; it < 12; ++it) lds4[it * 768 + ldsw] = r[it];
  };

  f32x16 acc[3];
#pragma unroll
  for (int j = 0; j < 3; ++j)
#pragma unroll
    for (int q = 0; q < 16; ++q) acc[j][q] = 0.f;
  const int l31 = lane & 31, half = lane >> 5;
  const int sa = (l31 >> 2) & 3, sb = ((32 + l31) >> 2) & 3;
  const int ia0 = l31 * 4 + ((2 * half) ^ sa), ia1 = l31 * 4 + ((2 * half + 1) ^ sa);
  const int ib0 = (32 + l31) * 4 + ((2 * half) ^ sb), ib1 = (32 + l31) * 4 + ((2 * half + 1) ^ sb);
  auto compute = [&]() {
#pragma unroll
    for (int j = 0; j < 3; ++j) {
      const float4* T = lds4 + (wave * 3 + j) * 256;
      const float4 a0 = T[ia0], a1 = T[ia1], b0 = T[ib0], b1 = T[ib1];
      acc[j] = __builtin_amdgcn_mfma_f32_32x32x2f32(a0.x, b0.x, acc[j], 0, 0, 0);
      acc[j] = __builtin_amdgcn_mfma_f32_32x32x2f32(a0.y, b0.y, acc[j], 0, 0, 0);
      acc[j] = __builtin_amdgcn_mfma_f32_32x32x2f32(a0.z, b0.z, acc[j], 0, 0, 0);
      acc[j] = __builtin_amdgcn_mfma_f32_32x32x2f32(a0.w, b0.w, acc[j], 0, 0, 0);
      acc[j] = __builtin_amdgcn_mfma_f32_32x32x2f32(a1.x, b1.x, acc[j], 0, 0, 0);
      acc[j] = __builtin_amdgcn_mfma_f32_32x32x2f32(a1.y, b1.y, acc[j], 0, 0, 0);
      acc[j] = __builtin_amdgcn_mfma_f32_32x32x2f32(a1.z, b1.z, acc[j], 0, 0, 0);
      acc[j] = __builtin_amdgcn_mfma_f32_32x32x2f32(a1.w, b1.w, acc[j], 0, 0, 0);
    }
  };

  const int nk = a.Kp / WF_BK;
  gload(0);
  lstore();
  __syncthreads();
  for (int kt = 0; kt < nk; ++kt) {
    if (kt + 1 < nk) gload((kt + 1) * WF_BK);
    compute();
    __syncthreads();
    if (kt + 1 < nk) {
      lstore();
      __syncthreads();
    }
  }

  float* Ms = reinterpret_cast<float*>(lds4);
#pragma unroll
  for (int j = 0; j < 3; ++j) {
    const int pnt = wave * 3 + j;
#pragma unroll
    for (int q = 0; q < 16; ++q) Ms[(pnt * WF_TB + (q & 3) + 8 * (q >> 2) + 4 * half) * (WF_CB + 1) + l31] = acc[j][q];
  }
  __syncthreads();
  constexpr int MT = 4, A = 6;
  for (int idx = tid; idx < WF_TB * WF_CB; idx += WF_THREADS) {
    const int t = idx >> 5, c = idx & 31;
    const long tile = tile0 + t;
    const int co = co0 + c;
    if (tile >= a.g.tiles || co >= a.Cout) continue;
    const TileId ti = decode_tile((unsigned)tile, a.g);
    Vec<1> sv[MT][A];
#pragma unroll
    for (int b = 0; b < A; ++b) {
      Vec<1> col[A], o[MT];
#pragma unroll
      for (int aa = 0; aa < A; ++aa) col[aa].v[0] = Ms[((aa * A + b) * WF_TB + t) * (WF_CB + 1) + c];
      mat_apply<MT, W_AT>(col, o);
#pragma unroll
      for (int aa = 0; aa < MT; ++aa) sv[aa][b] = o[aa];
    }
    const float bi = a.bias ? a.bias[co] : 0.f, sc = a.scale ? a.scale[co] : 0.f, sh = a.scale ? a.shift[co] : 0.f;
#pragma unroll
    for (int aa = 0; aa < MT; ++aa) {
      const int yy = ti.ry + a.g.d * (MT * ti.ty + aa);
      Vec<1> o[MT];
      mat_apply<MT, W_AT>(sv[aa], o);
#pragma unroll
      for (int b = 0; b < MT; ++b) {
        const int xx = ti.rx + a.g.d * (MT * ti.tx + b);
        if (yy >= a.g.H || xx >= a.g.W) continue;
        const long pix = (long)(ti.n * a.g.H + yy) * a.g.W + xx;
        float v = o[b].v[0];
        if (a.bias) v += bi;
        if (a.scale) v = v * sc + sh;
        if (a.residual) v += a.residual[pix * a.rp + co];
        if (a.relu) v = fmaxf(v, 0.f);
        a.y[pix * a.yp + co] = v;
      }
    }
  }
}

inline unsigned nblocks(long total) { return (unsigned)std::min<long>((total + 255) / 256, 1 << 20); }

}

pm_wino_geom pm_wino_make_geom(int n, int h, int w, int d, int m) {
  pm_wino_geom g;
  g.N = n, g.H = h, g.W = w, g.d = d, g.m = m;
  g.TY = (pm_cdiv(h, d) + m - 1) / m, g.TX = (pm_cdiv(w, d) + m - 1) / m;
  g.tiles = (long)n * d * d * g.TY * g.TX;
  return g;
}

int pm_wino_input_xf(const float* x, long pitch, int C, int Kp, const pm_wino_geom& g, float* V, hipStream_t st) {
  if (g.m == 4) hipLaunchKernelGGL((wino_input_kernel<4, 2>), dim3(nblocks(g.tiles * (Kp / 2))), dim3(256), 0, st, x, pitch, C, Kp, g, V);
  else hipLaunchKernelGGL((wino_input_kernel<2, 4>), dim3(nblocks(g.tiles * (Kp / 4))), dim3(256), 0, st, x, pitch, C, Kp, g, V);
  return pm_check_launch("wino_input");
}

int pm_wino_filter_xf(const float* w, int Cout, int Cin, int Kp, bool dgrad, int m, float* U, hipStream_t st) {
  const int R = dgrad ? Cin : Cout;
  dim3 grid(Kp / 32, pm_cdiv(R, 32));
  if (m == 4) {
    if (dgrad) hipLaunchKernelGGL((wino_filter_kernel<4, true>), grid, dim3(256), 0, st, w, Cout, Cin, Kp, U);
    else hipLaunchKernelGGL((wino_filter_kernel<4, false>), grid, dim3(256), 0, st, w, Cout, Cin, Kp, U);
  } else {
    if (dgrad) hipLaunchKernelGGL((wino_filter_kernel<2, true>), grid, dim3(256), 0, st, w, Cout, Cin, Kp, U);
    else hipLaunchKernelGGL((wino_filter_kernel<2, false>), grid, dim3(256), 0, st, w, Cout, Cin, Kp, U);
  }
  return pm_check_launch("wino_filter");
}

int pm_wino_filter_xf_multi(const float* const* w, float* const* U, const int* cout, const int* cin, const int* kp, const int* m, int n, hipStream_t st) {
  for (int i0 = 0; i0 < n; i0 += WR_BATCH) {
    WinoRefreshJobs t;
    t.n = std::min(WR_BATCH, n - i0);
    long blocks = 0;
    for (int i = 0; i < t.n; ++i) {
      t.w[i] = w[i0 + i], t.U[i] = U[i0 + i], t.cout[i] = cout[i0 + i], t.cin[i] = cin[i0 + i], t.kp[i] = kp[i0 + i], t.m[i] = m[i0 + i];
      t.start[i] = (int)blocks;
      blocks += (long)(kp[i0 + i] / 32) * pm_cdiv(cout[i0 + i], 32);
    }
    t.start[t.n] = (int)blocks;
    if (blocks == 0) continue;
    hipLaunchKernelGGL(wino_filter_multi_kernel, dim3((unsigned)blocks), dim3(256), 0, st, t);
    if (int e = pm_check_launch("wino_filter_multi")) return e;
  }
  return PM_OK;
}

int pm_wino_output_xf(const float* M, int Cout, const pm_wino_geom& g, float* y, long ypitch, const float* bias, const float* scale, const float* shift,
                      const float* residual, long res_pitch, int relu, hipStream_t st) {
  if (g.m == 4)
    hipLaunchKernelGGL((wino_output_kernel<4, 2>), dim3(nblocks(g.tiles * (Cout / 2))), dim3(256), 0, st, M, Cout, g, y, ypitch, bias, scale, shift, residual,
                       res_pitch, relu);
  else
    hipLaunchKernelGGL((wino_output_kernel<2, 4>), dim3(nblocks(g.tiles * (Cout / 4))), dim3(256), 0, st, M, Cout, g, y, ypitch, bias, scale, shift, residual,
                       res_pitch, relu);
  return pm_check_launch("wino_output");
}

int pm_wino_dy_xf(const float* dy, long pitch, int Cout, const pm_wino_geom& g, float* Z, hipStream_t st) {
  if (g.m == 4) hipLaunchKernelGGL((wino_dy_kernel<4, 2>), dim3(nblocks(g.tiles * (Cout / 2))), dim3(256), 0, st, dy, pitch, Cout, g, Z);
  else hipLaunchKernelGGL((wino_dy_kernel<2, 4>), dim3(nblocks(g.tiles * (Cout / 4))), dim3(256), 0, st, dy, pitch, Cout, g, Z);
  return pm_check_launch("wino_dy");
}

int pm_wino_dw_xf(const float* slab, int ks, int Cout, int Cin, int Kp, int m, float* dw, hipStream_t st) {
  const unsigned nb = (unsigned)std::min<long>(((long)Cout * Cin + 255) / 256, 1 << 16);
  if (m == 4) hipLaunchKernelGGL(wino_dw_kernel<4>, dim3(nb), dim3(256), 0, st, slab, ks, Cout, Cin, Kp, dw);
  else hipLaunchKernelGGL(wino_dw_kernel<2>, dim3(nb), dim3(256), 0, st, slab, ks, Cout, Cin, Kp, dw);
  return pm_check_launch("wino_dw");
}

int pm_wino_fused_f4(const float* V, const float* U, int Cout, int Kp, const pm_wino_geom& g, float* y, long ypitch, const float* bias, const float* scale,
                     const float* shift, const float* residual, long res_pitch, int relu, hipStream_t st) {
  static pm_lds_optin optin;
  (void)optin(reinterpret_cast<const void*>(&wino_fused_f4_kernel), (int)WF_LDS);
  WinoFusedArgs a;
  a.V = V, a.U = U, a.y = y, a.yp = ypitch, a.Cout = Cout, a.Kp = Kp, a.g = g;
  a.bias = bias, a.scale = scale, a.shift = shift, a.residual = residual, a.rp = res_pitch, a.relu = relu;
  a.ncb = (Cout + WF_CB - 1) / WF_CB;
  const long ntb = (g.tiles + WF_TB - 1) / WF_TB;
  hipLaunchKernelGGL(wino_fused_f4_kernel, dim3((unsigned)(ntb * a.ncb)), dim3(WF_THREADS), WF_LDS, st, a);
  return pm_check_launch("wino_fused_f4");
}
```

pinthememory_amd/hip/kernels.py:

```python
import ctypes
from ctypes import byref

import os
import weakref

import torch

from . import lib as L
from .lib import PmConvEpilogue, PmConvParams, check, ptr, stream, tdesc, workspace


def _lib():
    return L.load()


CONV_PREC = 0
ACT_DTYPE = torch.float32


def set_conv_precision(name):
    global CONV_PREC, ACT_DTYPE
    CONV_PREC = {'f32': 0, 'fp32': 0, 'bf16': 2, 'bf16_operands': 2, 'bf16_staged': 1}[name]
    ACT_DTYPE = torch.bfloat16 if name == 'bf16' else torch.float32

# ... 58 lines not shown
            _U_OWNERS[p.data_ptr()] = weakref.ref(p)


def unregister_filter_owners(params=None):
    ptrs = None if params is None else {p.data_ptr() for p in params}
    for k in [k for k in _U_OWNERS if ptrs is None or k in ptrs]:
        del _U_OWNERS[k]
    _U_CACHE.drop_if(lambda ent: ptrs is None or ent.ptr in ptrs)


def _filter_owner(w_krsc):
    ref = _U_OWNERS.get(w_krsc.data_ptr())
    p = ref() if ref is not None else None
    if p is None:
        if ref is not None:
            del _U_OWNERS[w_krsc.data_ptr()]
        return None
    return p if (p.data_ptr() == w_krsc.data_ptr() and p.numel() == w_krsc.numel() and p.is_leaf) else None


class _KeptFilter:
    __slots__ = ('ptr', 'shape', 'nbytes', 'device', 'prec', 'dgrad', 'owner', 'version', 'buf', 'event', 'stream', 'used')


class _FilterCache(dict):
    def __init__(self):
        self.nbytes = 0
        self.streams = {}

    def _stream(self):
        raw = stream()
        cur = self.streams.get(raw)
        if cur is None:
            cur = self.streams[raw] = L.stream_obj()
        return raw, cur

    def _drop(self, key):
        ent = self.pop(key)
        self.nbytes -= ent.nbytes
        if ent.buf.is_cuda:
            for s in self.streams.values():
                ent.buf.record_stream(s)

    def drop_if(self, pred):
        for key in [k for k, ent in self.items() if pred(ent)]:
            self._drop(key)

    def clear(self):
        self.drop_if(lambda ent: True)

    def lookup(self, p, w_krsc, nbu, dgrad=False):
        if KEEP_WINOGRAD_U is False or not nbu:
            return None
        registered = _filter_owner(w_krsc)
        if registered is None and KEEP_WINOGRAD_U is not True:
            return None
        owner = w_krsc if registered is None else registered
        key = (w_krsc.data_ptr(), tuple(w_krsc.shape), nbu, w_krsc.device.index, p.prec, dgrad)
        ent = self.get(key)
        if ent is not None and ent.owner() is not owner:
            self._drop(key)
            ent = None
        if ent is None:
            self.drop_if(lambda e: e.owner() is None)
            while self and (len(self) >= _U_CACHE_MAX or self.nbytes + nbu > _U_CACHE_BYTES):
                self._drop(next(iter(self)))
            ent = _KeptFilter()
            ent.ptr, ent.shape, ent.nbytes, ent.device, ent.prec, ent.dgrad = key
            ent.owner = (lambda: w_krsc) if registered is None else weakref.ref(registered)
            ent.version, ent.buf, ent.event, ent.stream = -1, torch.empty(nbu // 4, dtype=torch.float32, device=w_krsc.device), None, None
            self.nbytes += nbu
        else:
            del self[key]
        self[key] = ent
        ent.used = True
        version = owner._version
        valid = ent.version == version
        if not valid:
            ent.version = -1
        p.wxf, p.wxf_bytes, p.wxf_valid = ent.buf.data_ptr(), nbu, 1 if valid else 0
        raw, cur = self._stream()
        if valid and ent.event is not None and ent.stream != raw:
            cur.wait_event(ent.event)
        return None if valid else (ent, version)

    def commit(self, *pending):
        raw, cur = self._stream()
        event = cur.record_event()
        for ent, version in pending:
            ent.version, ent.event, ent.stream = version, event, raw

    def forget_events(self):
        for ent in self.values():
            ent.event = ent.stream = None


_U_CACHE = _FilterCache()
clear_filters, forget_filter_events = _U_CACHE.clear, _U_CACHE.forget_events

_REFRESH = {2: ('pm_conv_wxf_refresh_bf16', False), 0: ('pm_conv_wxf_refresh_f32', True)}


def refresh_filters():
    if KEEP_WINOGRAD_U is False or not _U_CACHE or CONV_PREC not in _REFRESH:
        return 0
    entry_point, forward_3x3_only = _REFRESH[CONV_PREC]
    dev = torch.cuda.current_device()
    todo = []
    for ent in _U_CACHE.values():
        if ent.prec != CONV_PREC or ent.device != dev or not ent.used:
            continue
        cout, kh, kw, cin = ent.shape
        if forward_3x3_only and (ent.dgrad or kh != 3 or kw != 3):
            continue
        ent.used = False
        owner = ent.owner()
        if owner is None or owner.data_ptr() != ent.ptr or ent.version == owner._version or not ent.buf.is_cuda:
            continue
        todo.append((ent, owner._version))
    if not todo:
        return 0
    jobs = (L.PmWxfJob * len(todo))()
    for j, (ent, version) in zip(jobs, todo):
        cout, kh, kw, cin = ent.shape
        j.w, j.wxf, j.wxf_bytes, j.cout, j.kh, j.kw, j.cin, j.dgrad = ent.ptr, ent.buf.data_ptr(), ent.nbytes, cout, kh, kw, cin, 1 if ent.dgrad else 0
        ent.version = -1
    check(getattr(_lib(), entry_point)(jobs, len(todo), stream()), entry_point)
    _U_CACHE.commit(*todo)
    return len(todo)


_SIZES = {}
_GEN = [0]


def _sizes(key, fn):
    v = _SIZES.get(key)
    if v is None:
        if len(_SIZES) > 8192:
            _SIZES.clear()
        v = _SIZES[key] = fn()
    return v


_XFORM_COUNT = [0, False]


def filter_transform_count(enable=None):
    if enable is not None:
        _XFORM_COUNT[1] = bool(enable)
    return _XFORM_COUNT[0]


def conv_fwd(x, w_krsc, stride, pad, dil, bias=None, scale=None, shift=None, residual=None, relu=False, out=None, keep_v=None, bn_partials=None, out_dtype=None):
    cout, kh, kw, cin = w_krsc.shape
    n, h, w_, c = x.shape
    assert c == cin, 'conv: Cin mismatch %d vs %d' % (c, cin)
    ho, wo = conv_out_hw(h, w_, kh, stride, pad, dil)
    y = out if out is not None else new((n, ho, wo, cout), x, pitch_pad=True, dtype=out_dtype if out_dtype is not None else ACT_DTYPE)
    assert residual is None or residual.dtype == y.dtype, 'conv_fwd: the fused residual has the dtype of the output'
    xd, yd = tdesc(x), tdesc(y)
    p = L.conv_params(kh, kw, stride, pad, dil, CONV_PREC)
    lib = _lib()
    nbv, nbu, nb, npb = _sizes(('f', x.shape, x.stride(), x.dtype, xd.flags, w_krsc.shape, y.stride(), y.dtype, stride, pad, dil, CONV_PREC, _GEN[0]),
                               lambda: (lib.pm_conv_winograd_v_bytes(byref(xd), byref(yd), byref(p)), lib.pm_conv_wxf_bytes(byref(xd), byref(yd), byref(p)),
                                        lib.pm_conv_workspace(byref(xd), byref(yd), byref(p), 0), lib.pm_conv_bn_partials_bytes(byref(xd), byref(yd), byref(p))))
    if keep_v is not None:
        nbv = nbv if KEEP_WINOGRAD_V else 0
        v = torch.empty(nbv // 4, dtype=torch.float32, device=x.device) if nbv else None
        keep_v.append(v)
        if v is not None:
            p.wino_v, p.wino_v_bytes = v.data_ptr(), nbv
    u_ent = None
    if (kh == 3 and CONV_PREC == 0) or CONV_PREC == 2:
        u_ent = _U_CACHE.lookup(p, w_krsc, nbu)
    if _XFORM_COUNT[1] and p.wxf_valid == 0 and nbu:
        _XFORM_COUNT[0] += 1
    ws = workspace(nb, x.device) if nb else None
    part = None
    if bn_partials is not None:
        ep16 = BN_EPILOGUE16 or (BN_EP16_MIN_BYTES > 0 and y.numel() * 2 >= BN_EP16_MIN_BYTES)
        ep32 = BN_EPILOGUE or (BN_EP_MIN_BYTES > 0 and y.numel() * 4 >= BN_EP_MIN_BYTES)
        npb = npb if ((ep16 if y.dtype == torch.bfloat16 else ep32) and residual is None and not relu and scale is None) else 0
        part = torch.empty(npb // 4, dtype=torch.float32, device=x.device) if npb else None
        bn_partials.append(part)
    ep = None
    if bias is not None or scale is not None or residual is not None or relu or part is not None:
        rd = tdesc(residual) if residual is not None else None
        ep = L.conv_epilogue(ptr(bias), ptr(scale), ptr(shift), rd.ptr if rd else None, rd.pitch if rd else 0, 1 if relu else 0, ptr(part),
                            part.numel() * 4 if part is not None else 0)
    check(lib.pm_conv_fwd(byref(xd), w_krsc.data_ptr(), byref(yd), byref(p), byref(ep) if ep else None, ptr(ws), nb, stream()), 'pm_conv_fwd')
    if u_ent is not None:
        _U_CACHE.commit(u_ent)
    return y


def conv_bwd_data(dy, w_krsc, x_shape, stride, pad, dil, add=None, dtype=None, add_mask=None):
    cout, kh, kw, cin = w_krsc.shape
    dx = new(x_shape, dy, dtype=dtype)
    dyd, dxd = tdesc(dy), tdesc(dx)
    p = L.conv_params(kh, kw, stride, pad, dil, CONV_PREC)
    lib = _lib()
    nb, nbu = _sizes(('d', dy.shape, dy.stride(), dy.dtype, dyd.flags, w_krsc.shape, dx.shape, dx.stride(), dx.dtype, stride, pad, dil, CONV_PREC, _GEN[0]),
                     lambda: (lib.pm_conv_workspace(byref(dxd), byref(dyd), byref(p), 1), lib.pm_conv_wxf_bytes_dgrad(byref(dyd), byref(dxd), byref(p))))
    ws = workspace(nb, dy.device) if nb else None
    ad = tdesc(add) if add is not None else None
    u_ent = _U_CACHE.lookup(p, w_krsc, nbu, dgrad=True) if CONV_PREC == 2 else None
    if add_mask is not None:
        check(lib.pm_conv_bwd_data_masked(byref(dyd), w_krsc.data_ptr(), byref(dxd), byref(p), byref(ad), add_mask.data_ptr(), ptr(ws), nb, stream()), 'pm_conv_bwd_data_masked')
    else:
        check(lib.pm_conv_bwd_data(byref(dyd), w_krsc.data_ptr(), byref(dxd), byref(p), byref(ad) if ad else None, ptr(ws), nb, stream()), 'pm_conv_bwd_data')
    if u_ent is not None:
        _U_CACHE.commit(u_ent)
    return dx


def conv_bwd_weight(x, dy, w_shape_krsc, stride, pad, dil, want_bias=False, wino_v=None, on_stream=None):
    cout, kh, kw, cin = w_shape_krsc
    dw = torch.empty(w_shape_krsc, dtype=torch.float32, device=x.device)
    db = torch.empty(cout, dtype=torch.float32, device=x.device) if want_bias else None
    xd, dyd = tdesc(x), tdesc(dy)
    p = L.conv_params(kh, kw, stride, pad, dil, CONV_PREC)
    if wino_v is not None:
        p.wino_v, p.wino_v_bytes = wino_v.data_ptr(), wino_v.numel() * 4
    lib = _lib()
    nb = _sizes(('w', x.shape, x.stride(), x.dtype, dy.shape, dy.stride(), dy.dtype, w_shape_krsc, stride, pad, dil, CONV_PREC, wino_v is not None, _GEN[0]),
                lambda: lib.pm_conv_workspace(byref(xd), byref(dyd), byref(p), 2))
    raw = stream() if on_stream is None else on_stream.cuda_stream
    ws = workspace(nb, x.device, on_stream)
    check(lib.pm_conv_bwd_weight(byref(xd), byref(dyd), dw.data_ptr(), ptr(db), byref(p), ptr(ws), nb, raw), 'pm_conv_bwd_weight')
    return dw, db


def bn_stats(x):
    c = x.shape[3]
    mom = torch.empty(3 * c, dtype=torch.float32, device=x.device)
    xd = tdesc(x)
    lib = _lib()
    nb = _sizes(('bn', x.shape, x.dtype), lambda: lib.pm_bn_workspace(byref(xd)))
    ws = workspace(nb, x.device)
    check(lib.pm_bn_stats(byref(xd), mom.data_ptr(), ptr(ws), nb, stream()), 'pm_bn_stats')
    return mom


def bn_stats_finalize(x, eps, running_mean=None, running_var=None, momentum=0.1):
    c = x.shape[3]
    mean = torch.empty(c, dtype=torch.float32, device=x.device)
    invstd = torch.empty_like(mean)
    xd = tdesc(x)
    lib = _lib()
    nb = _sizes(('bn', x.shape, x.dtype), lambda: lib.pm_bn_workspace(byref(xd)))
    ws = workspace(nb, x.device)
    check(lib.pm_bn_stats_finalize(byref(xd), eps, mean.data_ptr(), invstd.data_ptr(), ptr(running_mean), ptr(running_var), momentum, ptr(ws), nb, stream()),
          'pm_bn_stats_finalize')
    return mean, invstd


def bn_partials_finalize(part, pixels, c, eps, running_mean=None, running_var=None, momentum=0.1):
    mean = torch.empty(c, dtype=torch.float32, device=part.device)
    invstd = torch.empty_like(mean)
    check(_lib().pm_bn_partials_finalize(part.data_ptr(), pixels, c, eps, mean.data_ptr(), invstd.data_ptr(), ptr(running_mean), ptr(running_var), momentum, None,
                                         stream()), 'pm_bn_partials_finalize')
    return mean, invstd


def bn_partials_moments(part, pixels, c):
    mom = torch.empty(3 * c, dtype=torch.float32, device=part.device)
    check(_lib().pm_bn_partials_finalize(part.data_ptr(), pixels, c, 0.0, None, None, None, None, 0.0, mom.data_ptr(), stream()), 'pm_bn_partials_finalize')
    return mom


def bn_merge(parts, world, c):
    out = torch.empty(3 * c, dtype=torch.float32, device=parts.device)
    check(_lib().pm_bn_merge(parts.data_ptr(), world, c, out.data_ptr(), stream()), 'pm_bn_merge')
    return out


def bn_merge_finalize(parts, world, c, eps, running_mean=None, running_var=None, momentum=0.1):
    mean = torch.empty(c, dtype=torch.float32, device=parts.device)
    invstd = torch.empty_like(mean)
    check(_lib().pm_bn_merge_finalize(parts.data_ptr(), world, c, eps, mean.data_ptr(), invstd.data_ptr(), ptr(running_mean), ptr(running_var), momentum,
                                      stream()), 'pm_bn_merge_finalize')
    return mean, invstd


def bn_finalize(moments, c, eps, running_mean=None, running_var=None, momentum=0.1):
    mean = torch.empty(c, dtype=torch.float32, device=moments.device)
    invstd = torch.empty_like(mean)
    check(_lib().pm_bn_finalize(moments.data_ptr(), c, eps, mean.data_ptr(), invstd.data_ptr(), ptr(running_mean), ptr(running_var), momentum, stream()),
          'pm_bn_finalize')
    return mean, invstd


def bn_fold_multi(table, cs, offs, n, max_c, total, eps):
    arena = torch.empty(2 * total, dtype=torch.float32, device=table.device)
    check(_lib().pm_bn_fold_multi(table.data_ptr(), cs.data_ptr(), offs.data_ptr(), n, max_c, total, eps, arena.data_ptr(), stream()), 'pm_bn_fold_multi')
    return arena


def bn_fold(gamma, beta, running_mean, running_var, eps, conv_bias=None):
    c = gamma.numel()
    scale = torch.empty(c, dtype=torch.float32, device=gamma.device)
    shift = torch.empty_like(scale)
    check(_lib().pm_bn_fold(gamma.data_ptr(), beta.data_ptr(), running_mean.data_ptr(), running_var.data_ptr(), ptr(conv_bias), c, eps, scale.data_ptr(),
                            shift.data_ptr(), stream()), 'pm_bn_fold')
    return scale, shift


def bn_apply(x, mean, invstd, gamma, beta, residual=None, relu=False, out=None, want_mask=False):
    y = out if out is not None else torch.empty_like(x, memory_format=torch.contiguous_format)
    rd = tdesc(residual) if residual is not None else None
    grp = 8 if x.dtype == torch.bfloat16 else 4
    mask = torch.empty((x.shape[0] * x.shape[1] * x.shape[2], x.shape[3] // grp), dtype=torch.uint8, device=x.device) if want_mask else None
    check(_lib().pm_bn_apply_mask(byref(tdesc(x)), mean.data_ptr(), invstd.data_ptr(), gamma.data_ptr(), beta.data_ptr(), byref(rd) if rd else None,
                                  1 if relu else 0, byref(tdesc(y)), ptr(mask), stream()), 'pm_bn_apply_mask')
    return (y, mask) if want_mask else y


def bn_apply_res_affine(x, mean, invstd, gamma, beta, r, r_mean, r_invstd, r_gamma, r_beta, relu=False, want_mask=False):
    y = torch.empty_like(x, memory_format=torch.contiguous_format)
    mask = torch.empty((x.shape[0] * x.shape[1] * x.shape[2], x.shape[3] // 4), dtype=torch.uint8, device=x.device) if want_mask else None
    check(_lib().pm_bn_apply_mask_affine(byref(tdesc(x)), mean.data_ptr(), invstd.data_ptr(), gamma.data_ptr(), beta.data_ptr(), byref(tdesc(r)), r_mean.data_ptr(),
                                         r_invstd.data_ptr(), r_gamma.data_ptr(), r_beta.data_ptr(), 1 if relu else 0, byref(tdesc(y)), ptr(mask), stream()),
          'pm_bn_apply_mask_affine')
    return (y, mask) if want_mask else y


def _bwd_sums(x, with_count, sums):
    c = x.shape[3]
    n = 2 * c + (1 if with_count else 0)
    if sums is None:
        sums = torch.empty(n, dtype=torch.float32, device=x.device)
    assert sums.numel() == n and sums.is_contiguous()
    if with_count:
        sums[2 * c:].fill_(float(x.shape[0] * x.shape[1] * x.shape[2]))
    return sums


def bn_bwd_apply_mask(dy, mask, x, mean, invstd, gamma, sums, count):
    dx = torch.empty(x.shape, dtype=x.dtype, device=x.device)
    check(_lib().pm_bn_bwd_apply_mask(byref(tdesc(dy)), mask.data_ptr(), byref(tdesc(x)), mean.data_ptr(), invstd.data_ptr(), gamma.data_ptr(), sums.data_ptr(),
                                      float(count), byref(tdesc(dx)), stream()), 'pm_bn_bwd_apply_mask')
    return dx


def bn_bwd_reduce_mask(dy, mask, x, mean, invstd, want_gmask=True, with_count=False, sums=None):
    sums = _bwd_sums(x, with_count, sums)
    xd = tdesc(x)
    lib = _lib()
    nb = _sizes(('bn', x.shape, x.dtype), lambda: lib.pm_bn_workspace(byref(xd)))
    ws = workspace(nb, x.device)
    gm = torch.empty(x.shape, dtype=x.dtype, device=x.device) if want_gmask else None
    gd = tdesc(gm) if want_gmask else None
    check(lib.pm_bn_bwd_reduce_mask(byref(tdesc(dy)), mask.data_ptr(), byref(xd), mean.data_ptr(), invstd.data_ptr(), byref(gd) if gd else None,
                                    sums.data_ptr(), ptr(ws), nb, stream()), 'pm_bn_bwd_reduce_mask')
    return sums, gm


def scale_shift_act(x, scale, shift, residual=None, relu=False):
    y = torch.empty(x.shape, dtype=torch.float32, device=x.device)
    rd = tdesc(residual) if residual is not None else None
    check(_lib().pm_scale_shift_act(byref(tdesc(x)), scale.data_ptr(), shift.data_ptr(), byref(rd) if rd else None, 1 if relu else 0, byref(tdesc(y)), stream()),
          'pm_scale_shift_act')
    return y


def bn_bwd_reduce(dy, y, x, mean, invstd, relu, gamma=None, beta=None, want_gmask=False, with_count=False, sums=None):
    relu = int(relu)
    sums = _bwd_sums(x, with_count, sums)
    xd = tdesc(x)
    lib = _lib()
    nb = _sizes(('bn', x.shape, x.dtype), lambda: lib.pm_bn_workspace(byref(xd)))
    ws = workspace(nb, x.device)
    yd = tdesc(y) if relu == 1 else None
    gm = torch.empty(x.shape, dtype=x.dtype, device=x.device) if want_gmask else None
    gd = tdesc(gm) if want_gmask else None
    check(lib.pm_bn_bwd_reduce(byref(tdesc(dy)), byref(yd) if yd else None, byref(xd), mean.data_ptr(), invstd.data_ptr(), ptr(gamma), ptr(beta), relu,
                               byref(gd) if gd else None, sums.data_ptr(), ptr(ws), nb, stream()), 'pm_bn_bwd_reduce')
    return sums, gm
# ... 547 lines not shown
```

pinthememory_amd/hip/lib.py:

```python
import ctypes
import os
from ctypes import POINTER, byref, c_char_p, c_float, c_int, c_int32, c_int64, c_size_t, c_void_p

import torch

_HERE = os.path.dirname(os.path.dirname(os.path.abspath(__file__)))
LIB_PATH = os.environ.get('PM_LIB') or os.path.join(_HERE, 'libpinmem_hip.so')


class PmTensor(ctypes.Structure):
    _fields_ = [('ptr', c_void_p), ('n', c_int32), ('h', c_int32), ('w', c_int32), ('c', c_int32), ('pitch', c_int64), ('dtype', c_int32), ('flags', c_int32)]


PM_F32, PM_BF16 = 0, 1
PM_TF_ZERO_PAD64 = 1


class PmSgdEntry(ctypes.Structure):
    _fields_ = [('param', c_void_p), ('grad', c_void_p), ('momentum_buffer', c_void_p), ('numel', c_int64)]


class PmWxfJob(ctypes.Structure):
    _fields_ = [('w', c_void_p), ('wxf', c_void_p), ('wxf_bytes', c_int64), ('cout', c_int32), ('kh', c_int32), ('kw', c_int32), ('cin', c_int32),
                ('dgrad', c_int32), ('reserved', c_int32)]


class PmConvParams(ctypes.Structure):
    _fields_ = [('struct_size', c_int32), ('kh', c_int32), ('kw', c_int32), ('stride', c_int32), ('pad', c_int32), ('dil', c_int32), ('prec', c_int32),
                ('wino_v', c_void_p), ('wino_v_bytes', c_int64),
                ('wxf', c_void_p), ('wxf_bytes', c_int64), ('wxf_valid', c_int32)]


class PmRouting(ctypes.Structure):
    _fields_ = [('struct_size', c_int32), ('winograd', c_int32), ('winograd_fused', c_int32), ('conv16', c_int32), ('conv16_wide', c_int32),
                ('conv16_persistent', c_int32), ('wgrad16', c_int32), ('bf16_wgrad', c_int32), ('split', c_int32)]


class PmAugImage(ctypes.Structure):
    _fields_ = [('order', ctypes.c_uint8 * 4), ('enabled', ctypes.c_uint8), ('flip', ctypes.c_uint8), ('hue_shift', ctypes.c_uint8), ('reserved', ctypes.c_uint8),
                ('brightness', c_float), ('contrast', c_float), ('saturation', c_float), ('radius', c_int32), ('w', ctypes.c_double * 6)]


class PmConvEpilogue(ctypes.Structure):
    _fields_ = [('struct_size', c_int64), ('bias', c_void_p), ('scale', c_void_p), ('shift', c_void_p), ('residual', c_void_p),
                ('residual_pitch', c_int64), ('relu', c_int32), ('bn_partials', c_void_p), ('bn_partials_bytes', c_int64)]


def conv_params(kh, kw, stride, pad, dil, prec=0):
    return PmConvParams(ctypes.sizeof(PmConvParams), kh, kw, stride, pad, dil, prec)


def conv_epilogue(*fields):
    return PmConvEpilogue(ctypes.sizeof(PmConvEpilogue), *fields)


ABI_VERSION = 410


class PinmemError(RuntimeError):
    pass


_T, _P, _E = POINTER(PmTensor), POINTER(PmConvParams), POINTER(PmConvEpilogue)
_vp, _sz, _i, _f, _i64 = c_void_p, c_size_t, c_int, c_float, c_int64

SIGNATURES = {
    'pm_last_error': (c_char_p, []),
    'pm_version': (c_int, []),
    'pm_conv_winograd_v_bytes': (_sz, [_T, _T, _P]),
    'pm_conv_wxf_bytes': (_sz, [_T, _T, _P]),
    'pm_conv_wxf_bytes_dgrad': (_sz, [_T, _T, _P]),
    'pm_conv_wxf_refresh_bf16': (_i, [_vp, _i, _vp]),
    'pm_conv_wxf_refresh_f32': (_i, [_vp, _i, _vp]),
    'pm_conv_workspace': (_sz, [_T, _T, _P, _i]),
    'pm_conv_fwd': (_i, [_T, _vp, _T, _P, _E, _vp, _sz, _vp]),
    'pm_conv_bwd_data': (_i, [_T, _vp, _T, _P, _T, _vp, _sz, _vp]),
    'pm_conv_bwd_data_masked': (_i, [_T, _vp, _T, _P, _T, _vp, _vp, _sz, _vp]),
    'pm_conv_bwd_weight': (_i, [_T, _T, _vp, _vp, _P, _vp, _sz, _vp]),
    'pm_set_winograd': (_i, [_i]),
    'pm_set_winograd_fused': (_i, [_i]),
    'pm_set_conv16': (_i, [_i]),
    'pm_profile_enable': (_i, [_i]),
    'pm_profile_dump': (_i, [ctypes.c_char_p]),
    'pm_profile_read': (_i, [_i, _i, _i, _i, _i, POINTER(ctypes.c_double), POINTER(ctypes.c_double), POINTER(c_int64), _i]),
    'pm_profile_read_prec': (_i, [_i, _i, _i, _i, _i, _i, POINTER(ctypes.c_double), POINTER(ctypes.c_double), POINTER(c_int64), _i]),
    'pm_profile_read_bytes': (_i, [_i, _i, _i, _i, _i, _i, POINTER(ctypes.c_double)]),
    'pm_bn_workspace': (_sz, [_T]),
    'pm_bn_stats': (_i, [_T, _vp, _vp, _sz, _vp]),
    'pm_bn_merge': (_i, [_vp, _i, _i, _vp, _vp]),
    'pm_bn_merge_finalize': (_i, [_vp, _i, _i, _f, _vp, _vp, _vp, _vp, _f, _vp]),
    'pm_bn_finalize': (_i, [_vp, _i, _f, _vp, _vp, _vp, _vp, _f, _vp]),
    'pm_bn_stats_finalize': (_i, [_T, _f, _vp, _vp, _vp, _vp, _f, _vp, _sz, _vp]),
    'pm_bn_fold': (_i, [_vp, _vp, _vp, _vp, _vp, _i, _f, _vp, _vp, _vp]),
    'pm_bn_fold_multi': (_i, [_vp, _vp, _vp, _i, _i, _i, _f, _vp, _vp]),
    'pm_bn_apply': (_i, [_T, _vp, _vp, _vp, _vp, _T, _i, _T, _vp]),
    'pm_bn_apply_mask': (_i, [_T, _vp, _vp, _vp, _vp, _T, _i, _T, _vp, _vp]),
    'pm_bn_bwd_reduce_mask': (_i, [_T, _vp, _T, _vp, _vp, _T, _vp, _vp, _sz, _vp]),
    'pm_bn_apply_mask_affine': (_i, [_T, _vp, _vp, _vp, _vp, _T, _vp, _vp, _vp, _vp, _i, _T, _vp, _vp]),
    'pm_bn_bwd_apply_mask': (_i, [_T, _vp, _T, _vp, _vp, _vp, _vp, _f, _T, _vp]),
    'pm_bn_bwd_reduce': (_i, [_T, _T, _T, _vp, _vp, _vp, _vp, _i, _T, _vp, _vp, _sz, _vp]),
    'pm_bn_bwd_apply': (_i, [_T, _T, _T, _vp, _vp, _vp, _vp, _vp, _f, _i, _T, _T, _vp]),
    'pm_relu_bwd': (_i, [_T, _T, _T, _vp]),
    'pm_add': (_i, [_T, _T, _T, _vp]),
    'pm_add_n': (_i, [POINTER(_T), _i, _T, _vp]),
    'pm_copy': (_i, [_T, _T, _vp]),
    'pm_scale_shift_act': (_i, [_T, _vp, _vp, _T, _i, _T, _vp]),
    'pm_maxpool3x3s2_fwd': (_i, [_T, _T, _vp, _vp]),
    'pm_maxpool3x3s2_bwd': (_i, [_T, _vp, _T, _vp]),
    'pm_maxpool3x3s2_bn_relu_fwd': (_i, [_T, _vp, _vp, _vp, _vp, _T, _vp, _vp]),
    'pm_bn_bwd_reduce_pool': (_i, [_T, _vp, _T, _vp, _vp, _vp, _vp, _vp, _vp, _sz, _vp]),
    'pm_bn_bwd_apply_pool': (_i, [_T, _vp, _T, _vp, _vp, _vp, _vp, _vp, _f, _T, _vp]),
    'pm_global_avgpool_fwd': (_i, [_T, _T, _vp]),
    'pm_global_avgpool_bwd': (_i, [_T, _T, _i, _vp]),
    'pm_resize_bilinear_fwd': (_i, [_T, _T, _vp]),
    'pm_resize_bilinear_bwd': (_i, [_T, _T, _i, _vp]),
    'pm_resize_bilinear_bwd_workspace': (_sz, [_T, _T]),
    'pm_resize_bilinear_bwd_separable': (_i, [_T, _T, _i, _vp, _sz, _vp]),
    'pm_resize_bilinear_hp_fwd': (_i, [_T, _T, _i, _vp]),
    'pm_softmax_mean_update': (_i, [_T, _vp, _i, _vp]),
    'pm_sliding_stitch': (_i, [_T, _vp, _i, _i, _i, _i, _vp, _i, _vp]),
    'pm_argmax_f64': (_i, [_vp, _i, _i, _i, _i, _vp, _vp, _vp]),
    'pm_image_u8_to_nhwc4': (_i, [_vp, _i64, POINTER(c_float), POINTER(c_float), _vp, _vp]),
    'pm_labels_u8_to_i64': (_i, [_vp, _i64, _vp, _vp]),
    'pm_aug_blur_weights': (_i, [ctypes.c_double, POINTER(c_int32), POINTER(ctypes.c_double)]),
    'pm_augment_workspace': (_sz, [_i]),
    'pm_augment_u8': (_i, [_vp, _i, _i, _i, _vp, c_int32, POINTER(c_float), POINTER(c_float), _vp, _vp, _vp, _sz, _vp]),
    'pm_labels_u8_flip_to_i64': (_i, [_vp, _i, _i, _i, _vp, c_int32, _vp, _vp]),
    'pm_nchw_to_nhwc': (_i, [_vp, _i, _T, _vp]),
    'pm_nhwc_to_nchw': (_i, [_T, _vp, _vp]),
    'pm_label_nearest': (_i, [_vp, _i, _i, _i, _vp, _i, _i, _vp]),
    'pm_upsample_ce_workspace': (_sz, [_i, _i, _i]),
    'pm_upsample_ce_fwd': (_i, [_T, _f, _vp, _i, _i, _vp, _vp, _sz, _vp]),
    'pm_upsample_ce_bwd_workspace': (_sz, [_T, _i, _i]),
    'pm_upsample_ce_bwd': (_i, [_T, _f, _vp, _i, _i, _vp, _vp, _T, _vp, _sz, _vp]),
    'pm_upsample_ce_field_bytes': (_sz, [_T, _i, _i]),
    'pm_upsample_ce_fwd_field': (_i, [_T, _f, _vp, _i, _i, _vp, _vp, _vp, _sz, _vp]),
    'pm_upsample_ce_bwd_field': (_i, [_T, _f, _i, _i, _vp, _vp, _vp, _T, _vp]),
    'pm_upsample_wce_loss_floats': (_sz, [_i]),
    'pm_upsample_wce_workspace': (_sz, [_i, _i, _i]),
    'pm_upsample_wce_fwd': (_i, [_T, _f, _vp, _i, _i, _vp, _i64, _i, _vp, _vp, _sz, _vp]),
    'pm_upsample_wce_fwd_field': (_i, [_T, _f, _vp, _i, _i, _vp, _i64, _i, _vp, _vp, _vp, _sz, _vp]),
    'pm_upsample_wce_bwd_field': (_i, [_T, _f, _i, _i, _i, _vp, _vp, _vp, _T, _vp]),
    'pm_label_class_weights_workspace': (_sz, [_i]),
    'pm_label_class_weights': (_i, [_vp, _i, _i, _i, _i, ctypes.c_double, _i, _i, _vp, _vp, _sz, _vp]),
    'pm_upsample_eval_workspace': (_sz, [_T, _i, _i]),
    'pm_upsample_eval': (_i, [_T, _f, _vp, _i, _i, _vp, _vp, _i, _vp, _vp, _sz, _vp]),
    'pm_mem_read_fwd': (_i, [_T, _vp, _i, _vp, _T, _vp, _vp, _vp]),
    'pm_mem_read_fwd_pq_workspace': (_sz, [_i64, _i]),
    'pm_mem_read_fwd_pq': (_i, [_T, _vp, _i, _vp, _vp, _T, _vp, _vp, _vp, _vp, _sz, _vp]),
    'pm_mem_colsoftmax_workspace': (_sz, [_i64, _i]),
    'pm_mem_colsoftmax': (_i, [_vp, _vp, _i64, _i, _vp, _vp, _sz, _vp]),
    'pm_mem_read_bwd_workspace': (_sz, [_i64, _i, _i]),
    'pm_mem_read_bwd': (_i, [_T, _vp, _i, _vp, _T, _vp, _T, _vp, _vp, _sz, _vp]),
    'pm_mem_write_accum_workspace': (_sz, [_T, _i]),
    'pm_mem_write_accum': (_i, [_T, _vp, _i, _i, _i, _i, _vp, _vp, _sz, _vp]),
    'pm_mem_write_accum_bwd': (_i, [_T, _vp, _i, _i, _i, _i, _vp, _T, _vp]),
    'pm_mem_write_update': (_i, [_vp, _vp, _i, _i, _f, _vp, _vp, _vp]),
    'pm_mem_write_update_bwd': (_i, [_vp, _vp, _i, _i, _f, _vp, _vp, _vp, _vp]),
    'pm_sgd_momentum': (_i, [_vp, _vp, _vp, _i64, _f, _f, _f, _i, _vp]),
    'pm_set_bf16_wgrad': (_i, [_i]),
    'pm_set_wgrad16': (_i, [_i]),
    'pm_set_split': (_i, [_i]),
    'pm_routing_get': (_i, [POINTER(PmRouting)]),
    'pm_routing_set': (_i, [POINTER(PmRouting)]),
    'pm_conv_bn_partials_bytes': (_sz, [_T, _T, POINTER(PmConvParams)]),
    'pm_bn_partials_finalize': (_i, [_vp, _i64, _i, _f, _vp, _vp, _vp, _vp, _f, _vp, _vp]),
    'pm_sgd_momentum_multi': (_i, [_vp, _i, _f, _f, _f, _vp]),
    'pm_sgd_momentum_multi_dev': (_i, [_vp, _i, _f, _vp, _f, _f, _vp]),
    'pm_cast': (_i, [_T, _T, _vp]),
}

_lib = None


def load():
    global _lib
    if _lib is not None:
        return _lib
    if not os.environ.get('PM_LIB'):
        from .. import build as _build
        _build.build()
    lib = ctypes.CDLL(LIB_PATH)
    for name, (res, args) in SIGNATURES.items():
        fn = getattr(lib, name)
        fn.restype, fn.argtypes = res, args
    if lib.pm_version() != ABI_VERSION:
        raise PinmemError('%s reports ABI %d, this binding is written against %d (include/pinmem_hip.h)' % (LIB_PATH, lib.pm_version(), ABI_VERSION))
    _lib = lib
    return lib


def check(code, what=''):
    if code != 0:
        raise PinmemError('%s failed (%d): %s' % (what, code, load().pm_last_error().decode()))


_raw_stream = torch._C._cuda_getCurrentRawStream
_cur_device = torch._C._cuda_getDevice


def stream():
    return _raw_stream(_cur_device())


_ZERO_PAD = {}


def register_zero_pad(base, c, pitch):
    import weakref
# ... 61 lines not shown
```

pinthememory_amd/hip/ops.py:

```python
import os as _os

import torch

from . import kernels as K
from . import lib as L
from .. import dist as D


def nhwc(t):
    v = t.permute(0, 2, 3, 1)
    n, h, w, c = v.shape
    sn, sh, sw, sc = v.stride()
    pitch = sw if w > 1 else (sh if h > 1 else (sn if n > 1 else c))
    ok = (sc == 1 or c == 1) and pitch >= c and (h == 1 or w == 1 or sh == w * pitch) and (n == 1 or h * w == 1 or sn == h * w * pitch)
    if ok and v.dtype == torch.float32:
        return v
    if v.dtype == torch.bfloat16:
        if ok and pitch % 8 == 0 and c % 8 == 0 and v.data_ptr() % 16 == 0:
            return v
        return v.contiguous()
    if h * w == 1:
        return v.contiguous().float()
    return K.nchw_to_nhwc(t.float())


def nchw(v):
    return v.permute(0, 3, 1, 2)


def _grad_view(g):
    v = nhwc(g)
    if v.stride(2) % (8 if v.dtype == torch.bfloat16 else 4) or v.data_ptr() % 16:
        v = v.contiguous()
    return v


class BNState:
    __slots__ = ('running_mean', 'running_var', 'eps', 'momentum', 'training', 'group', 'grad_enabled')

    def __init__(self, bn):
        self.running_mean, self.running_var = bn.running_mean, bn.running_var
        self.eps = bn.eps
        self.momentum = 0.1 if bn.momentum is None else bn.momentum
        self.training = bn.training or bn.running_mean is None
        self.group = D.bn_group(bn)
        self.grad_enabled = torch.is_grad_enabled()
        if bn.training and bn.num_batches_tracked is not None:
            _nbt_pending.append(bn.num_batches_tracked)


_nbt_pending = []


def flush_bn_counters():
    if _nbt_pending:
        torch._foreach_add_(_nbt_pending, 1)
        _nbt_pending.clear()


_OVERLAP_ENV = _os.environ.get('PM_OVERLAP_WGRAD')
OVERLAP_WGRAD = True if _OVERLAP_ENV is None else _OVERLAP_ENV == '1'


def overlap_wgrad():
    if not OVERLAP_WGRAD:
        return False
    return not (_OVERLAP_ENV is None and K.CONV_PREC == 2 and K.ACT_DTYPE == torch.bfloat16)


_side = {}
_proxy = {}


def masked_stream(n_cus, device=None, first=0):
    import ctypes
    dev = torch.cuda.current_device() if device is None else device
    total = torch.cuda.get_device_properties(dev).multi_processor_count
    n_cus = max(1, min(int(n_cus), total))
    words = (total + 31) // 32
    mask = (ctypes.c_uint32 * words)()
    picked = {(first + (i * total) // n_cus) % total for i in range(n_cus)}
    for cu in picked:
        mask[cu // 32] |= 1 << (cu % 32)
    hip = ctypes.CDLL('libamdhip64.so')
    st = ctypes.c_void_p()
    with torch.cuda.device(dev):
        err = hip.hipExtStreamCreateWithCUMask(ctypes.byref(st), ctypes.c_uint32(words), mask)
    if err != 0 or not st.value:
        raise RuntimeError('hipExtStreamCreateWithCUMask(%d CUs) failed: %d' % (n_cus, err))
    return torch.cuda.ExternalStream(st.value, device=dev)


WGRAD_CUS = int(_os.environ.get('PM_WGRAD_CUS', '0'))


def _side_stream():
    dev = torch.cuda.current_device()
    if dev not in _side:
        _side[dev] = masked_stream(WGRAD_CUS, dev) if WGRAD_CUS > 0 else torch.cuda.Stream(device=dev)
    return _side[dev]


class _Defer(torch.autograd.Function):
    @staticmethod
    def forward(ctx, w):
        return w.view_as(w)

    @staticmethod
    def backward(ctx, g):
        L.stream_obj().wait_stream(_side_stream())
        return g


def begin_forward():
    flush_bn_counters()
    _proxy.clear()


def defer_weights(module):
    if not (overlap_wgrad() and torch.is_grad_enabled()):
        return
    for m in module.modules():
        if isinstance(m, torch.nn.Conv2d) and m.bias is None and m.weight.requires_grad and id(m.weight) not in _proxy:
            _proxy[id(m.weight)] = _Defer.apply(m.weight)


def _w(weight):
    p = _proxy.get(id(weight))
    return (p, True) if p is not None else (weight, False)


def _wgrad(x, dy, wshape, geom, want_bias=False, deferred=False, wino_v=None):
    if not deferred:
        return K.conv_bwd_weight(x, dy, wshape, *geom, want_bias=want_bias, wino_v=wino_v)
    side, main = _side_stream(), L.stream_obj()
    ev = torch.cuda.Event()
    ev.record(main)
    side.wait_event(ev)
    out = K.conv_bwd_weight(x, dy, wshape, *geom, want_bias=want_bias, wino_v=wino_v, on_stream=side)
    if wino_v is not None:
        wino_v.record_stream(side)
    x.record_stream(side)
    dy.record_stream(side)
    for t in out:
        if t is not None:
            t.record_stream(side)
    return out


commit_done = {}


def wait_commit():
    if not commit_done or not torch.cuda.is_available():
        return
    ev = commit_done.pop(torch.cuda.current_device(), None)
    if ev is not None:
        torch.cuda.current_stream().wait_event(ev)


def _same_exchange(groups, widths):
    return D.is_dist() and all(g is not None and g is groups[0] for g in groups) and len(set(widths)) == 1


def _bn_train_stats_multi(ys, bns, partials):
    n = len(ys)
    if n > 1 and not _same_exchange([b.group for b in bns], [y.shape[3] for y in ys]):
        return [_bn_train_stats(y, bn, part) for y, bn, part in zip(ys, bns, partials)]
    pixels = [y.shape[0] * y.shape[1] * y.shape[2] for y in ys]
    if bns[0].group is None:
        y, bn, part = ys[0], bns[0], partials[0]
        if part is not None:
            return [K.bn_partials_finalize(part, pixels[0], y.shape[3], bn.eps, bn.running_mean, bn.running_var, bn.momentum)]
        return [K.bn_stats_finalize(y, bn.eps, bn.running_mean, bn.running_var, bn.momentum)]
    c = ys[0].shape[3]
    moms = [K.bn_partials_moments(part, px, c) if part is not None else K.bn_stats(y) for y, part, px in zip(ys, partials, pixels)]
    flat, world = D.gather_moments(moms[0] if n == 1 else torch.cat(moms), bns[0].group)
    parts = flat.view(world, n, 3 * c)
    return [K.bn_merge_finalize(parts[:, i].contiguous().view(-1), world, c, bn.eps, bn.running_mean, bn.running_var, bn.momentum) for i, bn in enumerate(bns)]


def _bn_train_stats(y, bn, partials=None):
    return _bn_train_stats_multi([y], [bn], [partials])[0]


def _bn_train_fwd(y, gamma, beta, bn, residual, relu, out=None, partials=None):
    mean, invstd = _bn_train_stats(y, bn, partials)
    return K.bn_apply(y, mean, invstd, gamma, beta, residual=residual, relu=relu, out=out), mean, invstd


class _BnSums:

    def __init__(self, n, c, group, device):
        self.c, self.group, self.with_count = c, group, group is not None
        self.len = 2 * c + (1 if self.with_count else 0)
        self.stride = (self.len + 3) // 4 * 4
        self.local = torch.empty((n - 1) * self.stride + self.len, dtype=torch.float32, device=device)
        self.summed = self.local

    def slot(self, i):
        return self.local[i * self.stride:i * self.stride + self.len]

    def exchange(self):
        if self.group is not None:
            self.summed = D.all_reduce_sum_copy(self.local, self.group)

    def total(self, i):
        return self.summed[i * self.stride:i * self.stride + self.len]

    def count(self, y):
        return -1.0 if self.with_count else float(y.shape[0] * y.shape[1] * y.shape[2])

    def grads(self, i):
        s = self.slot(i)
        return s[self.c:2 * self.c], s[:self.c]


def _bn_train_bwd(dv, o, y, mean, invstd, gamma, beta, relu, group, want_dres, has_res, mask=None):
    mode = 0 if not relu else (1 if has_res else 2)
    hand_over = mode == 1 and want_dres
    S = _BnSums(1, y.shape[3], group, y.device)
    if hand_over and mask is not None:
        _, gm = K.bn_bwd_reduce_mask(dv, mask, y, mean, invstd, want_gmask=True, with_count=S.with_count, sums=S.slot(0))
    else:
        _, gm = K.bn_bwd_reduce(dv, o, y, mean, invstd, mode, gamma, beta, want_gmask=hand_over, with_count=S.with_count, sums=S.slot(0))
    S.exchange()
    if hand_over:
        dy, dres = K.bn_bwd_apply(gm, None, y, mean, invstd, gamma, S.total(0), S.count(y), 0, False)[0], gm
    else:
        dy, dres = K.bn_bwd_apply(dv, o, y, mean, invstd, gamma, S.total(0), S.count(y), mode, want_dres, beta)
    return (dy, dres, *S.grads(0))


def _bn_bwd_masked(dv, mask, y, mean, invstd, gamma, group):
    S = _BnSums(1, y.shape[3], group, y.device)
    K.bn_bwd_reduce_mask(dv, mask, y, mean, invstd, want_gmask=False, with_count=S.with_count, sums=S.slot(0))
    S.exchange()
    return (K.bn_bwd_apply_mask(dv, mask, y, mean, invstd, gamma, S.total(0), S.count(y)), *S.grads(0))


class _Bottleneck(torch.autograd.Function):

    @staticmethod
    def forward(ctx, x, w1, g1, b1, w2, g2, b2, w3, g3, b3, wd, gd, bd, geoms, bns, deferred):
        xv = nhwc(x)
        k1, k2, k3 = K.krsc(w1), K.krsc(w2), K.krsc(w3)
        ps = []
        y1 = K.conv_fwd(xv, k1, *geoms[0], bn_partials=ps)
        o1, m1, i1 = _bn_train_fwd(y1, g1, b1, bns[0], None, True, partials=ps[0])
        kv = []
        y2 = K.conv_fwd(o1, k2, *geoms[1], keep_v=kv, bn_partials=ps)
        o2, m2, i2 = _bn_train_fwd(y2, g2, b2, bns[1], None, True, partials=ps[1])
        y3 = K.conv_fwd(o2, k3, *geoms[2], bn_partials=ps)
        m3 = None
        if wd is not None:
            kd = K.krsc(wd)
            yd = K.conv_fwd(xv, kd, *geoms[3], bn_partials=ps)
            fold = y3.dtype == torch.float32 and yd.dtype == torch.float32
            if fold or _same_exchange([bns[3].group, bns[2].group], [yd.shape[3], y3.shape[3]]):
                (md, idd), (m3, i3) = _bn_train_stats_multi([yd, y3], [bns[3], bns[2]], [ps[3], ps[2]])
                res = None if fold else K.bn_apply(yd, md, idd, gd, bd, residual=None, relu=False)
            else:
                res, md, idd = _bn_train_fwd(yd, gd, bd, bns[3], None, False, partials=ps[3])
        else:
            kd = yd = md = idd = None
            res = xv
        if m3 is None:
            m3, i3 = _bn_train_stats(y3, bns[2], ps[2])
        if res is None:
            out, mask3 = K.bn_apply_res_affine(y3, m3, i3, g3, b3, yd, md, idd, gd, bd, relu=True, want_mask=True)
        else:
            out, mask3 = K.bn_apply(y3, m3, i3, g3, b3, residual=res, relu=True, want_mask=True)
        ctx.geoms, ctx.groups, ctx.has_ds, ctx.deferred = geoms, [b.group for b in bns], wd is not None, deferred
        ctx.save_for_backward(xv, k1, k2, k3, kd, y1, o1, y2, o2, y3, yd, out, m1, i1, m2, i2, m3, i3, md, idd, g1, g2, g3, gd, b1, b2, b3, kv[0], mask3)
        return nchw(out)

    @staticmethod
    def backward(ctx, dout):
        xv, k1, k2, k3, kd, y1, o1, y2, o2, y3, yd, out, m1, i1, m2, i2, m3, i3, md, idd, g1, g2, g3, gd, b1, b2, b3, v2, mask3 = ctx.saved_tensors
        ge, gr, df = ctx.geoms, ctx.groups, ctx.deferred
        dv = _grad_view(dout)
        pair = None
        if ctx.has_ds and _same_exchange([gr[2], gr[3]], [y3.shape[3], yd.shape[3]]):
            S = _BnSums(2, y3.shape[3], gr[2], y3.device)
            _, gm = K.bn_bwd_reduce_mask(dv, mask3, y3, m3, i3, want_gmask=True, with_count=True, sums=S.slot(0))
            K.bn_bwd_reduce(gm, None, yd, md, idd, 0, gd, None, want_gmask=False, with_count=True, sums=S.slot(1))
            S.exchange()
            dy3, _ = K.bn_bwd_apply(gm, None, y3, m3, i3, g3, S.total(0), -1.0, 0, False)
            dyd, _ = K.bn_bwd_apply(gm, None, yd, md, idd, gd, S.total(1), -1.0, 0, False, None)
            dres, (dg3, db3), pair = gm, S.grads(0), (dyd, *S.grads(1))
        elif dv.dtype == torch.float32 and K.CONV_PREC != 2:
            dy3, dg3, db3 = _bn_bwd_masked(dv, mask3, y3, m3, i3, g3, gr[2])
            dres = None
        else:
            dy3, dres, dg3, db3 = _bn_train_bwd(dv, out, y3, m3, i3, g3, b3, True, gr[2], True, True, mask=mask3)
        dw3, _ = _wgrad(o2, dy3, tuple(k3.shape), ge[2], deferred=df[2])
        do2 = K.conv_bwd_data(dy3, k3, tuple(o2.shape), *ge[2])
        dy2, _, dg2, db2 = _bn_train_bwd(do2, o2, y2, m2, i2, g2, b2, True, gr[1], False, False)
        dw2, _ = _wgrad(o1, dy2, tuple(k2.shape), ge[1], deferred=df[1], wino_v=v2)
        do1 = K.conv_bwd_data(dy2, k2, tuple(o1.shape), *ge[1])
        dy1, _, dg1, db1 = _bn_train_bwd(do1, o1, y1, m1, i1, g1, b1, True, gr[0], False, False)
        dw1, _ = _wgrad(xv, dy1, tuple(k1.shape), ge[0], deferred=df[0])
        dwd = dgd = dbd = None
        skip, skip_mask = (dres, None) if dres is not None else (dv, mask3)
        if ctx.has_ds:
            if pair is not None:
                dyd, dgd, dbd = pair
            elif dres is None:
                dyd, dgd, dbd = _bn_bwd_masked(dv, mask3, yd, md, idd, gd, gr[3])
            else:
                dyd, _, dgd, dbd = _bn_train_bwd(dres, None, yd, md, idd, gd, None, False, gr[3], False, False)
            dwdk, _ = _wgrad(xv, dyd, tuple(kd.shape), ge[3], deferred=df[3])
            dwd = dwdk.permute(0, 3, 1, 2)
            skip, skip_mask = (K.conv_bwd_data(dyd, kd, tuple(xv.shape), *ge[3]) if ctx.needs_input_grad[0] else None), None
        dx = nchw(K.conv_bwd_data(dy1, k1, tuple(xv.shape), *ge[0], add=skip, add_mask=skip_mask)) if ctx.needs_input_grad[0] else None
        p = lambda d: d.permute(0, 3, 1, 2)
        return dx, p(dw1), dg1, db1, p(dw2), dg2, db2, p(dw3), dg3, db3, dwd, dgd, dbd, None, None, None


FOLD_BATCH = _os.environ.get('PM_FOLD_BATCH', '1') == '1'
_fold_cache = None
fold_misses = 0
last_prefold_event = None


class prefold:
    def __init__(self, model):
        self.model, self.active = model, False

    def __enter__(self):
        global _fold_cache, last_prefold_event
        last_prefold_event = None
        m = self.model
        if not FOLD_BATCH or m.training or torch.is_grad_enabled() or _fold_cache is not None:
            return self
        bns = getattr(m, '_pm_bn_list', None)
        if bns is None:
            bns = [b for b in m.modules() if isinstance(b, torch.nn.modules.batchnorm._BatchNorm)]
            m.__dict__['_pm_bn_list'] = bns
        bns = [b for b in bns if b.running_mean is not None and b.weight is not None and b.running_mean.is_cuda and not b.training]
        if not bns or len({b.eps for b in bns}) != 1:
            return self
        ptrs = tuple(t.data_ptr() for b in bns for t in (b.weight, b.bias, b.running_mean, b.running_var))
        plan = m.__dict__.get('_pm_fold_plan')
        if plan is None or plan[0] != ptrs:
            dev = bns[0].running_mean.device
            cs = [b.num_features for b in bns]
            offs, tot = [], 0
            for c in cs:
                offs.append(tot)
                tot += (c + 3) // 4 * 4
            as_i64 = [p - (1 << 64) if p >= (1 << 63) else p for p in ptrs]
            plan = (ptrs, torch.tensor(as_i64, dtype=torch.int64, device=dev), torch.tensor(cs, dtype=torch.int32, device=dev),
                    torch.tensor(offs, dtype=torch.int32, device=dev), cs, offs, tot)
            m.__dict__['_pm_fold_plan'] = plan
        _, table, dcs, doffs, cs, offs, tot = plan
        arena = K.bn_fold_multi(table, dcs, doffs, len(cs), max(cs), tot, bns[0].eps)
        _fold_cache = {b.running_mean.data_ptr(): (arena[o:o + c], arena[tot + o:tot + o + c]) for b, c, o in zip(bns, cs, offs)}
        self.active = True
        last_prefold_event = torch.cuda.current_stream().record_event() if len(bns) == len(m.__dict__['_pm_bn_list']) else None
        return self

    def __exit__(self, *exc):
        global _fold_cache
        if self.active:
            _fold_cache = None
        return False


class _ConvBnAct(torch.autograd.Function):

    @staticmethod
    def forward(ctx, x, w, bias, gamma, beta, residual, geom, bn, relu, out, deferred=False):
        stride, pad, dil = geom
        xv, wk = nhwc(x), K.krsc(w)
        rv = nhwc(residual) if residual is not None else None
        ov = nhwc(out) if out is not None else None
        ctx.geom, ctx.relu, ctx.train, ctx.deferred = geom, relu, bn.training, deferred and bias is None
        needs_grad = bn.grad_enabled and any(ctx.needs_input_grad[:6])
        if not bn.training and not needs_grad:
            hit = _fold_cache.get(bn.running_mean.data_ptr()) if (_fold_cache is not None and bias is None) else None
            if hit is None:
                global fold_misses
                fold_misses += 1
            scale, shift = hit if hit is not None else K.bn_fold(gamma, beta, bn.running_mean, bn.running_var, bn.eps, bias)
            o = K.conv_fwd(xv, wk, stride, pad, dil, scale=scale, shift=shift, residual=rv, relu=relu, out=ov)
            return nchw(o)
        kv, ps = [], []
        y = K.conv_fwd(xv, wk, stride, pad, dil, bias=bias, keep_v=kv if ctx.needs_input_grad[1] else None, bn_partials=ps if bn.training else None)
        if bn.training:
            o, mean, invstd = _bn_train_fwd(y, gamma, beta, bn, rv, relu, ov, partials=ps[0])
        else:
            mean, invstd = bn.running_mean, torch.rsqrt(bn.running_var + bn.eps)
            o = K.bn_apply(y, mean, invstd, gamma, beta, residual=rv, relu=relu, out=ov)
        ctx.group, ctx.has_bias, ctx.has_res = bn.group, bias is not None, residual is not None
        ctx.save_for_backward(xv, wk, y, o, mean, invstd, gamma, beta, kv[0] if kv else None)
        return nchw(o)

    @staticmethod
    def backward(ctx, dout):
        xv, wk, y, o, mean, invstd, gamma, beta, vk = ctx.saved_tensors
        stride, pad, dil = ctx.geom
        dv = _grad_view(dout)
        want_dres = ctx.has_res and ctx.needs_input_grad[5]
        if ctx.train:
            dy, dres, dgamma, dbeta = _bn_train_bwd(dv, o, y, mean, invstd, gamma, beta, ctx.relu, ctx.group, want_dres, ctx.has_res)
        else:
            c = y.shape[3]
            mode = 0 if not ctx.relu else (1 if ctx.has_res else 2)
            sums, g = K.bn_bwd_reduce(dv, o, y, mean, invstd, mode, gamma, beta, want_gmask=mode != 0)
            g = dv if g is None else g
            dy = K.scale_shift_act(g, gamma * invstd, torch.zeros_like(gamma))
            dres, dgamma, dbeta = (g if want_dres else None), sums[c:], sums[:c]
        dx = nchw(K.conv_bwd_data(dy, wk, tuple(xv.shape), stride, pad, dil, dtype=xv.dtype)) if ctx.needs_input_grad[0] else None
        dw = db = None
        if ctx.needs_input_grad[1] or (ctx.has_bias and ctx.needs_input_grad[2]):
            dwk, db = _wgrad(xv, dy, tuple(wk.shape), (stride, pad, dil), want_bias=ctx.has_bias, deferred=ctx.deferred, wino_v=vk)
            dw = dwk.permute(0, 3, 1, 2)
        return dx, dw, db, dgamma, dbeta, (nchw(dres) if dres is not None else None), None, None, None, None, None


class _Stem(torch.autograd.Function):

    @staticmethod
    def forward(ctx, x, w, gamma, beta, geom, bn):
        xv, wk = nhwc(x), K.krsc(w)
        kv, ps = [], []
        y = K.conv_fwd(xv, wk, *geom, keep_v=kv if ctx.needs_input_grad[1] else None, bn_partials=ps)
        mean, invstd = _bn_train_stats(y, bn, ps[0])
        out, arg = K.maxpool_bn_relu_fwd(y, mean, invstd, gamma, beta)
        ctx.geom, ctx.group = geom, bn.group
        ctx.save_for_backward(xv, wk, y, mean, invstd, gamma, beta, arg, kv[0] if kv else None)
        return nchw(out)

    @staticmethod
    def backward(ctx, dout):
        xv, wk, y, mean, invstd, gamma, beta, arg, vk = ctx.saved_tensors
        dv = _grad_view(dout)
        S = _BnSums(1, y.shape[3], ctx.group, y.device)
        K.bn_bwd_reduce_pool(dv, arg, y, mean, invstd, gamma, beta, with_count=S.with_count, sums=S.slot(0))
        S.exchange()
        dy = K.bn_bwd_apply_pool(dv, arg, y, mean, invstd, gamma, beta, S.total(0), S.count(y))
        dx = nchw(K.conv_bwd_data(dy, wk, tuple(xv.shape), *ctx.geom, dtype=xv.dtype)) if ctx.needs_input_grad[0] else None
        dw = None
        if ctx.needs_input_grad[1]:
            dwk, _ = _wgrad(xv, dy, tuple(wk.shape), ctx.geom, wino_v=vk)
            dw = dwk.permute(0, 3, 1, 2)
        return (dx, dw, *S.grads(0), None, None)


def stem_tail(x, w, conv, bn):
    st = BNState(bn)
    if st.training and torch.is_grad_enabled() and K.ACT_DTYPE == torch.float32 and x.dtype == torch.float32 and w.shape[0] % 4 == 0:
        return _Stem.apply(x, w, bn.weight, bn.bias, _geom(conv), st)
    return maxpool3x3s2(_ConvBnAct.apply(x, w, None, bn.weight, bn.bias, None, _geom(conv), st, True, None))


class _ConvBnActN(torch.autograd.Function):

    @staticmethod
    def forward(ctx, n, geoms, bns, outs, deferreds, *ts):
        xs, ws, gammas, betas = ts[0:n], ts[n:2 * n], ts[2 * n:3 * n], ts[3 * n:4 * n]
        xvs, wks = [nhwc(x) for x in xs], [K.krsc(w) for w in ws]
        ys, kvs, parts = [], [], []
        for i in range(n):
            kv, ps = [], []
            ys.append(K.conv_fwd(xvs[i], wks[i], *geoms[i], keep_v=kv if ctx.needs_input_grad[5 + n + i] else None, bn_partials=ps))
            kvs.append(kv[0] if kv else None)
            parts.append(ps[0])
        stats = _bn_train_stats_multi(ys, bns, parts)
        os_ = [K.bn_apply(ys[i], stats[i][0], stats[i][1], gammas[i], betas[i], residual=None, relu=True, out=nhwc(outs[i]) if outs[i] is not None else None) for i in range(n)]
        ctx.n, ctx.geoms, ctx.group, ctx.deferreds = n, geoms, bns[0].group, deferreds
        ctx.save_for_backward(*xvs, *wks, *ys, *os_, *[st[0] for st in stats], *[st[1] for st in stats], *gammas, *betas, *kvs)
        return tuple(nchw(o) for o in os_)

    @staticmethod
    def backward(ctx, *douts):
        n = ctx.n
        sv = ctx.saved_tensors
        xvs, wks, ys, os_, means, invs, gammas, betas, kvs = (sv[i * n:(i + 1) * n] for i in range(9))
        S = _BnSums(n, ys[0].shape[3], ctx.group, ys[0].device)
        for i in range(n):
            K.bn_bwd_reduce(_grad_view(douts[i]), os_[i], ys[i], means[i], invs[i], 2, gammas[i], betas[i], want_gmask=False, with_count=True, sums=S.slot(i))
        S.exchange()
        dxs, dws, dgs, dbs = [], [], [], []
        for i in range(n):
            dy, _ = K.bn_bwd_apply(_grad_view(douts[i]), os_[i], ys[i], means[i], invs[i], gammas[i], S.total(i), -1.0, 2, False, betas[i])
            dxs.append(nchw(K.conv_bwd_data(dy, wks[i], tuple(xvs[i].shape), *ctx.geoms[i], dtype=xvs[i].dtype)) if ctx.needs_input_grad[5 + i] else None)
            dwk, _ = _wgrad(xvs[i], dy, tuple(wks[i].shape), ctx.geoms[i], deferred=ctx.deferreds[i], wino_v=kvs[i])
            dws.append(dwk.permute(0, 3, 1, 2))
            dg, db = S.grads(i)
            dgs.append(dg), dbs.append(db)
        return (None, None, None, None, None, *dxs, *dws, *dgs, *dbs)


def conv_bn_act_n(xs, seqs, outs):
    convs, bns_m = [q[0] for q in seqs], [q[1] for q in seqs]
    ok = (torch.is_grad_enabled() and all(b.training for b in bns_m) and all(cv.bias is None for cv in convs)
          and _same_exchange([D.bn_group(b) for b in bns_m], [cv.out_channels for cv in convs]))
    if not ok:
        return [conv_bn_act(x, cv, bn, relu=True, out=o) for x, cv, bn, o in zip(xs, convs, bns_m, outs)]
    states = [BNState(b) for b in bns_m]
    wd = [_w(cv.weight) for cv in convs]
    n = len(xs)
    return list(_ConvBnActN.apply(n, [_geom(cv) for cv in convs], states, list(outs), [d for _, d in wd], *xs, *[w for w, _ in wd],
                                  *[b.weight for b in bns_m], *[b.bias for b in bns_m]))


class _Conv(torch.autograd.Function):

    @staticmethod
    def forward(ctx, x, w, bias, geom):
        stride, pad, dil = geom
        xv, wk = nhwc(x), K.krsc(w)
        y = K.conv_fwd(xv, wk, stride, pad, dil, bias=bias, out_dtype=torch.float32)
        ctx.geom, ctx.has_bias = geom, bias is not None
        ctx.save_for_backward(xv, wk)
        return nchw(y)

    @staticmethod
    def backward(ctx, dout):
        xv, wk = ctx.saved_tensors
        stride, pad, dil = ctx.geom
        dv = _grad_view(dout)
        dx = nchw(K.conv_bwd_data(dv, wk, tuple(xv.shape), stride, pad, dil, dtype=xv.dtype)) if ctx.needs_input_grad[0] else None
        dwk, db = _wgrad(xv, dv, tuple(wk.shape), (stride, pad, dil), want_bias=ctx.has_bias)
        return dx, dwk.permute(0, 3, 1, 2), db, None


class _MaxPool(torch.autograd.Function):
    @staticmethod
    def forward(ctx, x):
        xv = nhwc(x)
        y, arg = K.maxpool_fwd(xv)
        ctx.shape = tuple(xv.shape)
        ctx.save_for_backward(arg)
        return nchw(y)

    @staticmethod
    def backward(ctx, dout):
        (arg,) = ctx.saved_tensors
        return nchw(K.maxpool_bwd(_grad_view(dout), arg, ctx.shape))


class _GlobalAvgPool(torch.autograd.Function):
    @staticmethod
    def forward(ctx, x):
        xv = nhwc(x)
        ctx.shape = tuple(xv.shape)
        return nchw(K.global_avgpool_fwd(xv))

    @staticmethod
    def backward(ctx, dout):
        return nchw(K.global_avgpool_bwd(_grad_view(dout), ctx.shape))


class _Resize(torch.autograd.Function):
    @staticmethod
    def forward(ctx, x, size, out):
        xv = nhwc(x)
        ctx.shape = tuple(xv.shape)
        return nchw(K.resize_fwd(xv, (int(size[0]), int(size[1])), out=nhwc(out) if out is not None else None))

    @staticmethod
    def backward(ctx, dout):
        return nchw(K.resize_bwd(_grad_view(dout), ctx.shape)), None, None


class _Concat(torch.autograd.Function):

    @staticmethod
    def forward(ctx, buf, *parts):
        ctx.widths = [p.shape[1] for p in parts]
        return buf.view_as(buf)
# ... 4 lines not shown
        for wd in ctx.widths:
            outs.append(dout[:, off:off + wd])
            off += wd
        return (None,) + tuple(outs)


class _Add(torch.autograd.Function):
    @staticmethod
    def forward(ctx, a, b):
        return nchw(K.add(nhwc(a), nhwc(b)))

    @staticmethod
    def backward(ctx, g):
        return g, g


class _Fanout(torch.autograd.Function):

    @staticmethod
    def forward(ctx, x, n):
        return tuple(x.view_as(x) for _ in range(n))

    @staticmethod
    def backward(ctx, *gs):
        gs = [_grad_view(g) for g in gs if g is not None]
        return (nchw(K.add_n(gs)) if len(gs) > 1 else nchw(gs[0])), None


def fanout(x, n):
    if n < 2 or n > 8 or not (torch.is_grad_enabled() and x.requires_grad):
        return (x,) * n
    return _Fanout.apply(x, n)


class _UpsampleCE(torch.autograd.Function):

    @staticmethod
    def forward(ctx, logits, labels, inv_temp, want_grad, weights=None, per_image=False):
        lv = nhwc(logits)
        labels = labels.contiguous()
        ctx.inv_temp, ctx.hw, ctx.per_image = inv_temp, tuple(labels.shape[1:]), (None if weights is None else per_image)
        if not want_grad:
            return (K.upsample_ce_fwd(lv, labels, inv_temp) if weights is None else K.upsample_wce_fwd(lv, labels, weights, per_image, inv_temp))[0]
        if weights is None:
            out, field = K.upsample_ce_fwd_field(lv, labels, inv_temp)
        else:
            out, field = K.upsample_wce_fwd_field(lv, labels, weights, per_image, inv_temp)
        ctx.save_for_backward(lv, out, field)
        return out[0]

    @staticmethod
    def backward(ctx, g):
        gs = g.reshape(1).float().contiguous()
        lv, out, field = ctx.saved_tensors
        if ctx.per_image is None:
            dl = K.upsample_ce_bwd_field(lv, ctx.hw, out, field, gs, ctx.inv_temp)
        else:
            dl = K.upsample_wce_bwd_field(lv, ctx.hw, out, field, gs, ctx.per_image, ctx.inv_temp)
        return nchw(dl), None, None, None, None, None


class _MemRead(torch.autograd.Function):

    @staticmethod
    def forward(ctx, x, mem, noise, noise_q=None, with_pq=False):
        xv = nhwc(x)
        mem = mem.contiguous()
        if with_pq:
            qr, score, pmem, pq = K.mem_read_fwd_pq(xv, mem, noise, noise_q)
        else:
            qr, score, pmem = K.mem_read_fwd(xv, mem, noise)
        n, h, w, _ = xv.shape
        m = mem.shape[0]
        ctx.save_for_backward(xv, mem, pmem)
        score, pmem = score.view(n, h, w, m), pmem.view(n, h, w, m)
        ctx.with_pq = with_pq
        if with_pq:
            pq = pq.view(n, h, w, m)
            ctx.mark_non_differentiable(pmem, pq)
            return nchw(qr), score, pmem, pq
        ctx.mark_non_differentiable(pmem)
        return nchw(qr), score, pmem

    @staticmethod
    def backward(ctx, dqr, dscore, _dp, _dq=None):
        xv, mem, pmem = ctx.saved_tensors
        n, h, w, d = xv.shape
        dq = _grad_view(dqr) if dqr is not None else torch.zeros((n, h, w, 2 * d), dtype=torch.float32, device=xv.device)
        ds = dscore.contiguous() if dscore is not None else None
        dx, dmem = K.mem_read_bwd(xv, mem, pmem, dq, ds, want_dmem=ctx.needs_input_grad[1])
        return nchw(dx), dmem, None, None, None


class _MemWriteAccum(torch.autograd.Function):

    @staticmethod
    def forward(ctx, z, labels, m):
        zv = nhwc(z)
        labels = labels.contiguous()
        ctx.m = m
        ctx.save_for_backward(zv, labels)
        return K.mem_write_accum(zv, labels, m, normalize=True)

    @staticmethod
    def backward(ctx, dnomden):
        zv, labels = ctx.saved_tensors
        m, d = ctx.m, zv.shape[3]
        dnom = dnomden[:(m + 1) * d].contiguous()
        return nchw(K.mem_write_accum_bwd(zv, labels, m, dnom, normalize=True)), None, None


class _MemWriteUpdate(torch.autograd.Function):

    @staticmethod
    def forward(ctx, mem, nomden, momentum):
        mem = mem.contiguous()
        out, u = K.mem_write_update(mem, nomden, momentum, want_u=True)
        ctx.momentum = momentum
        ctx.save_for_backward(u, nomden)
        return out

    @staticmethod
    def backward(ctx, dout):
        u, nomden = ctx.saved_tensors
        m, d = u.shape
        dnom = K.mem_write_update_bwd(u, nomden, ctx.momentum, dout.contiguous())
        g = torch.zeros_like(nomden)
        g[:(m + 1) * d] = dnom.reshape(-1)
        return None, g, None


def _geom(conv):
    assert conv.kernel_size[0] == conv.kernel_size[1] and conv.stride[0] == conv.stride[1] and conv.groups == 1
    assert conv.padding[0] == conv.padding[1] and conv.dilation[0] == conv.dilation[1]
    return conv.stride[0], conv.padding[0], conv.dilation[0]


def conv_bn_act(x, conv, bn, relu=True, residual=None, out=None):
    w, deferred = _w(conv.weight)
    return _ConvBnAct.apply(x, w, conv.bias, bn.weight, bn.bias, residual, _geom(conv), BNState(bn), relu, out, deferred)


def bottleneck(x, blk):
    ds = blk.downsample
    mods = [(blk.conv1, blk.bn1), (blk.conv2, blk.bn2), (blk.conv3, blk.bn3)] + ([(ds[0], ds[1])] if ds is not None else [])
    geoms = [_geom(c) for c, _ in mods]
    bns = [BNState(b) for _, b in mods]
    ws = [_w(c.weight) for c, _ in mods]
    wd, gd, bd = (ws[3][0], ds[1].weight, ds[1].bias) if ds is not None else (None, None, None)
    return _Bottleneck.apply(x, ws[0][0], blk.bn1.weight, blk.bn1.bias, ws[1][0], blk.bn2.weight, blk.bn2.bias,
                             ws[2][0], blk.bn3.weight, blk.bn3.bias, wd, gd, bd, geoms, bns, [d for _, d in ws] + [False])


def conv(x, conv_mod):
    return _Conv.apply(x, conv_mod.weight, conv_mod.bias, _geom(conv_mod))


def conv_raw(x, weight, bias, geom):
    return _Conv.apply(x, weight, bias, geom)


def maxpool3x3s2(x):
    return _MaxPool.apply(x)


def global_avgpool(x):
    return _GlobalAvgPool.apply(x)


def resize(x, size, out=None):
    return _Resize.apply(x, size, out)


def concat_buffer(like, channels, hw):
    return nchw(K.new((like.shape[0], hw[0], hw[1], sum(channels)), like, dtype=like.dtype if like.dtype == torch.bfloat16 else torch.float32))


def concat(buf, parts):
    return _Concat.apply(buf, *parts)


def add(a, b):
    return _Add.apply(a, b)


class _Cast(torch.autograd.Function):

    @staticmethod
    def forward(ctx, x, dtype):
        ctx.src = x.dtype
        return nchw(K.cast(nhwc(x), dtype))

    @staticmethod
    def backward(ctx, g):
        return nchw(K.cast(_grad_view(g), ctx.src)), None


def cast(x, dtype):
    return x if x.dtype == dtype else _Cast.apply(x, dtype)


def upsample_ce(logits, labels, inv_temp=1.0):
    if not K.upsample_ce_fused_ok(nhwc(logits), tuple(labels.shape[1:])):
        full = resize(logits, tuple(labels.shape[1:]))
        return torch.nn.functional.cross_entropy(full * float(inv_temp), labels, ignore_index=255, reduction='mean')
    return _UpsampleCE.apply(logits, labels, float(inv_temp), bool(torch.is_grad_enabled() and logits.requires_grad))


def weighted_ce(full, labels, weights, per_image):
    lp = torch.nn.functional.log_softmax(full, dim=1)
    weights = weights.to(device=full.device, dtype=lp.dtype)
    if weights.dim() == 1 and not per_image:
        return torch.nn.functional.nll_loss(lp, labels, weight=weights, ignore_index=255, reduction='mean')
    rows = weights.expand(full.shape[0], -1) if weights.dim() == 1 else weights
    num = [torch.nn.functional.nll_loss(lp[b:b + 1], labels[b:b + 1], weight=rows[b], ignore_index=255, reduction='sum') for b in range(full.shape[0])]
    valid = (labels >= 0) & (labels < full.shape[1])
    den = [torch.where(valid[b], rows[b][labels[b].clamp(0, full.shape[1] - 1)], lp.new_zeros(())).sum() for b in range(full.shape[0])]
    if per_image:
        return sum(nu / de for nu, de in zip(num, den))
    return sum(num) / sum(den)


def upsample_wce(logits, labels, weights, per_image, inv_temp=1.0):
    per_image = bool(per_image)
    if not K.upsample_ce_fused_ok(nhwc(logits), tuple(labels.shape[1:])):
        return weighted_ce(resize(logits, tuple(labels.shape[1:])) * float(inv_temp), labels, weights, per_image)
    return _UpsampleCE.apply(logits, labels, float(inv_temp), bool(torch.is_grad_enabled() and logits.requires_grad), weights.detach(), per_image)


def mem_read(x, mem, noise=None):
    return _MemRead.apply(x, mem, noise, None, False)


def mem_read_pq(x, mem, noise=None, noise_q=None):
    return _MemRead.apply(x, mem, noise, noise_q, True)


def mem_write_accum(z, labels, m):
    return _MemWriteAccum.apply(z, labels, m)


def mem_write_update(mem, nomden, momentum):
    return _MemWriteUpdate.apply(mem, nomden, float(momentum))
```

pinthememory_amd/network/deepv3plus.py:

```python
import torch
import torch.nn as nn

from . import Resnet, memory
from .mynn import Norm2d, Upsample, channels_last_weights, initialize_weights
from ..hip import kernels as K
from ..hip import ops
from .. import loss as _loss


def _cbr(cin, cout, k, **kw):
    return nn.Sequential(nn.Conv2d(cin, cout, kernel_size=k, bias=False, **kw), Norm2d(cout), nn.ReLU(inplace=True))


def run_cbr(seq, x, out=None, residual=None):
    return ops.conv_bn_act(x, seq[0], seq[1], relu=True, out=out, residual=residual)


def fused_ce_ok(criterion):
    return (isinstance(criterion, nn.CrossEntropyLoss) and criterion.ignore_index == 255 and criterion.reduction == 'mean'
            and criterion.weight is None and getattr(criterion, 'label_smoothing', 0.0) == 0.0)


def _plain_nll(c):
    return c.ignore_index == 255 and getattr(c, 'reduction', 'mean') == 'mean' and getattr(c, 'label_smoothing', 0.0) == 0.0 and getattr(c, 'size_average', True) in (None, True)
# ... 32 lines not shown
        feats = [_cbr(in_dim, reduction_dim, 1)]
        feats += [_cbr(in_dim, reduction_dim, 3, dilation=r, padding=r) for r in rates]
        self.features = nn.ModuleList(feats)
        self.img_pooling = nn.AdaptiveAvgPool2d(1)
        self.img_conv = _cbr(in_dim, 256, 1)

    def forward(self, x):
        widths = [self.img_conv[0].out_channels] + [f[0].out_channels for f in self.features]
        buf = ops.concat_buffer(x, widths, x.shape[2:])
        xs = ops.fanout(x, 1 + len(self.features))
        if isinstance(self.img_pooling, nn.AdaptiveAvgPool2d) and self.img_pooling.output_size in (1, (1, 1)):
            pooled = ops.global_avgpool(xs[0])
        else:
            pooled = self.img_pooling(xs[0])
        outs, off = [None], widths[0]
        for wd in widths[1:]:
            outs.append(buf[:, off:off + wd])
            off += wd
        res = ops.conv_bn_act_n([pooled] + list(xs[1:]), [self.img_conv] + list(self.features), outs)
        parts = [ops.resize(res[0], x.shape[2:], out=buf[:, :widths[0]])] + res[1:]
        return ops.concat(buf, parts)


class _Base(nn.Module):
    eval_logits_lowres = False

    def _adopt_trunk(self, trunk):
        self.register_forward_hook(lambda mod, inp, out: ops.flush_bn_counters())
        if trunk == 'resnet-50':
            resnet = Resnet.resnet50(wt_layer=self.args.wt_layer)
        elif trunk == 'resnet-101':
            resnet = Resnet.resnet101(pretrained=True, wt_layer=self.args.wt_layer)
        else:
            raise ValueError("Not a valid network arch")
        resnet.layer0 = nn.Sequential(resnet.conv1, resnet.bn1, resnet.relu, resnet.maxpool)
        self.layer0 = resnet.layer0
        self.layer1, self.layer2, self.layer3, self.layer4 = resnet.layer1, resnet.layer2, resnet.layer3, resnet.layer4

    def _trunk(self, x):
        train = self.training
        ops.begin_forward()
        x = Resnet.stem(self.layer0[0], self.layer0[1], x)
        x_tuple = [x, []]
        outs = []
        layers = [self.layer1, self.layer2, self.layer3, self.layer4]
        heads = [getattr(self, n) for n in ('aspp', 'bot_aspp', 'bot_fine', 'final1', 'memory') if hasattr(self, n)]
        ahead = [[layers[0], layers[1]], [layers[2]], [layers[3]], heads]
        for layer, nxt in zip(layers, ahead):
            if train:
                for m in nxt:
                    ops.defer_weights(m)
            x_tuple = layer(x_tuple)
            outs.append(x_tuple[0])
        return outs[0], outs[2], outs[3]

    def _make_memory(self):
        if self.args.memory:
            assert self.args.mem_slot == 19, 'memory.py:336 hard-codes 19 slots'
            self.memory = memory.Memory_sup(memory_size=self.args.mem_slot, input_feature_dim=self.args.mem_dim, feature_dim=self.args.mem_dim,
                                            momentum=self.args.mem_momentum, temperature=self.args.mem_temp, gumbel_read=(not self.args.gumbel_off))

    def _aux_loss(self, aux_out, gts, aux_gts):
        a = ops.conv_bn_act(aux_out, self.dsn[0], self.dsn[1], relu=True)
        if self.dsn[3].p > 0:
            a = self.dsn[3](a)
        a = ops.conv(a, self.dsn[4])
        if aux_gts.dim() == 1:
            aux_gts = gts
        small = K.label_nearest(aux_gts, a.shape[2:])
        return segmentation_loss(self.criterion_aux, a, small)

    def _finish(self, dec2, x_size, aux_out, gts, aux_gts, mem_output, writeloss, readloss, inter_feature):
        if self.training:
            loss1 = segmentation_loss(self.criterion, dec2, gts, x_size[2:])
            return_loss = [loss1, self._aux_loss(aux_out, gts, aux_gts)]
            if self.args.memory:
                return_loss += [mem_output, writeloss, readloss]
            return_loss.append(inter_feature)
            return return_loss
        outputs = [dec2 if self.eval_logits_lowres else Upsample(dec2, x_size[2:])]
        if self.args.memory:
            outputs.append(mem_output)
        outputs.append(inter_feature)
        return outputs

    def _run_memory(self, dec0_up, gts, memory_writing, writing_detach):
        dec0_up, sq, sm, readloss, writeloss = self.memory(dec0_up, gts, memory_writing, writing_detach)
        return dec0_up, [sq, sm, dec0_up.detach()], readloss, writeloss


class DeepV3Plus(_Base):
    def __init__(self, num_classes, trunk='resnet-101', criterion=None, criterion_aux=None, variant='D', skip='m1', skip_num=48, args=None):
        super().__init__()
        self.criterion, self.criterion_aux, self.variant, self.args, self.trunk = criterion, criterion_aux, variant, args, trunk
        assert all(v == 0 for v in args.wt_layer) and not args.use_wtloss, 'whitening is out of scope of the pinmem hot path'
        if trunk != 'resnet-50':
            raise ValueError("Not a valid network arch")
        self._adopt_trunk(trunk)

        def dilate(layer, d):
            for n, m in layer.named_modules():
                if 'conv2' in n:
                    m.dilation, m.padding, m.stride = (d, d), (d, d), (1, 1)
                elif 'downsample.0' in n:
                    m.stride = (1, 1)
        if variant == 'D':
            dilate(self.layer3, 2), dilate(self.layer4, 4)
            os = 8
        elif variant == 'D16':
            dilate(self.layer4, 2)
            os = 16
        else:
            raise ValueError('unknown deepv3 variant: {}'.format(variant))
        self.output_stride = os
        self.aspp = _AtrousSpatialPyramidPoolingModule(2048, 256, output_stride=os)
        self.bot_fine = _cbr(256, 48, 1)
        self.bot_aspp = _cbr(1280, 256, 1)
        self.final1 = nn.Sequential(*(list(_cbr(304, 256, 3, padding=1)) + list(_cbr(256, 256, 3, padding=1))))
        self.final2 = nn.Sequential(nn.Conv2d(256, num_classes, kernel_size=1, bias=True))
        self.dsn = nn.Sequential(nn.Conv2d(1024, 512, kernel_size=3, stride=1, padding=1), Norm2d(512), nn.ReLU(inplace=True), nn.Dropout2d(0.1),
                                 nn.Conv2d(512, num_classes, kernel_size=1, stride=1, padding=0, bias=True))
        initialize_weights(self.dsn)
        initialize_weights(self.aspp)
        initialize_weights(self.bot_aspp)
        initialize_weights(self.bot_fine)
        initialize_weights(self.final1)
        initialize_weights(self.final2)
        self.eps = 1e-5
        self.whitening = False
        self.three_input_layer = False
        self.cov_matrix_layer, self.cov_type = [], []
        self._make_memory()
        channels_last_weights(self)

    def forward(self, x, gts=None, aux_gts=None, img_gt=None, visualize=False, cal_covstat=False, apply_wtloss=True,
                memory_writing=False, writing_detach=True):
        with ops.prefold(self):
            return self._forward(x, gts, aux_gts, img_gt, visualize, cal_covstat, apply_wtloss, memory_writing, writing_detach)

    def _forward(self, x, gts, aux_gts, img_gt, visualize, cal_covstat, apply_wtloss, memory_writing, writing_detach):
        assert not cal_covstat and not visualize, 'whitening statistics are out of scope'
        x_size = x.size()
        low_level, aux_out, x = self._trunk(x)
        x = self.aspp(x)
        dec0_up = run_cbr(self.bot_aspp, x)
        inter_feature = dec0_up
        mem_output = writeloss = readloss = None
        if self.args.memory:
            dec0_up, mem_output, readloss, writeloss = self._run_memory(dec0_up, gts, memory_writing, writing_detach)
        buf = ops.concat_buffer(low_level, [48, 256], low_level.shape[2:])
        dec0_fine = run_cbr(self.bot_fine, low_level, out=buf[:, :48])
        dec0_up = ops.resize(dec0_up, low_level.size()[2:], out=buf[:, 48:])
        dec0 = ops.concat(buf, [dec0_fine, dec0_up])
        dec1 = ops.conv_bn_act(dec0, self.final1[0], self.final1[1], relu=True)
        dec1 = ops.conv_bn_act(dec1, self.final1[3], self.final1[4], relu=True)
        dec2 = ops.conv(dec1, self.final2[0])
        return self._finish(dec2, x_size, aux_out, gts, aux_gts, mem_output, writeloss, readloss, inter_feature)


def DeepR50V3PlusD_OS8(args, num_classes, criterion, criterion_aux):
    print("Model : DeepLabv3+, Backbone : ResNet-50")
    return DeepV3Plus(num_classes, trunk='resnet-50', criterion=criterion, criterion_aux=criterion_aux, variant='D', skip='m1', args=args)


def DeepR50V3PlusD(args, num_classes, criterion, criterion_aux):
    print("Model : DeepLabv3+, Backbone : ResNet-50")
    return DeepV3Plus(num_classes, trunk='resnet-50', criterion=criterion, criterion_aux=criterion_aux, variant='D16', skip='m1', args=args)
```

Measured before the change: 154.0.

## Fuse BN+ReLU (and concat-upsample) into Winograd input transform of 3x3 convs

Adds a conv 'source' descriptor so the fp32 Winograd input transform can apply a preceding batch-norm + ReLU on the fly, or read a concat of a full-resolution tensor and a bilinearly upsampled low-resolution tensor. Bottleneck 3x3 convs and the two decoder 3x3 convs now consume the raw conv output plus BN statistics instead of a materialized normalized activation. The aim is to remove the BN-apply write and re-read passes over large activations. In exchange, backward has to rebuild the activation from the source, and the new templated input kernel does more arithmetic per element. The concat-upsample path is added to the library, but the shown decoder still builds the concat buffer explicitly.

Result: no change. 154.4, median of 6 (+0.3%).

```diff
diff --git a/include/pinmem_hip.h b/include/pinmem_hip.h
--- a/include/pinmem_hip.h
+++ b/include/pinmem_hip.h
@@ -20,7 +20,25 @@
   int32_t flags;
 } pm_tensor;
 
-#define PM_ABI_VERSION 410
+#define PM_ABI_VERSION 420
+
+typedef enum pm_conv_source_kind {
+  PM_SRC_BN_RELU = 1,
+  PM_SRC_CONCAT_UPSAMPLE = 2
+} pm_conv_source_kind;
+typedef struct pm_conv_source {
+  int32_t struct_size;
+  int32_t kind;
+  const float* mean;
+  const float* invstd;
+  const float* gamma;
+  const float* beta;
+  const float* low;
+  int64_t low_pitch;
+  int32_t low_h, low_w;
+  int32_t split;
+  int32_t reserved;
+} pm_conv_source;
 
 typedef struct pm_conv_params {
   int32_t struct_size;
@@ -31,6 +49,7 @@
   void* wxf;
   int64_t wxf_bytes;
   int32_t wxf_valid;
+  const pm_conv_source* source;
 } pm_conv_params;
 
 typedef struct pm_conv_epilogue {
diff --git a/pinthememory_amd/csrc/conv_igemm.hip b/pinthememory_amd/csrc/conv_igemm.hip
--- a/pinthememory_amd/csrc/conv_igemm.hip
+++ b/pinthememory_amd/csrc/conv_igemm.hip
@@ -444,9 +444,29 @@
   }
   PM_REQUIRE(x->c % 4 == 0, PM_EUNSUPPORTED, "conv: Cin %% 4 != 0 unsupported (pad the input channels)");
   PM_REQUIRE((y->c % 4 == 0) || (p->kh * p->kw == 1), PM_EUNSUPPORTED, "conv: Cout %% 4 != 0 only for 1x1");
-  PM_REQUIRE(x->pitch >= x->c && y->pitch >= y->c, PM_EINVAL, "conv: pitch < channels");
+  const int x_stored = (p->source && p->source->kind == PM_SRC_CONCAT_UPSAMPLE && p->source->split > 0) ? std::min(p->source->split, x->c) : x->c;
+  PM_REQUIRE(x->pitch >= x_stored && y->pitch >= y->c, PM_EINVAL, "conv: pitch < channels");
   PM_REQUIRE(pm_pixels(x) * x->pitch < (1ll << 29) && pm_pixels(y) * y->pitch < (1ll << 29) && (int64_t)y->c * x->c * p->kh * p->kw < (1ll << 29),
              PM_EUNSUPPORTED, "conv: tensor too large for 32-bit byte offsets (2 GiB per tensor)");
+  return PM_OK;
+}
+
+int check_source(const char* who, const pm_conv_source* s, const pm_tensor* x, bool wino) {
+  if (!s) return PM_OK;
+  PM_REQUIRE(s->struct_size == (int32_t)sizeof(pm_conv_source), PM_EINVAL, "%s: pm_conv_source.struct_size %d != %zu -- caller built against another pinmem_hip.h (library ABI %d)", who,
+             s->struct_size, sizeof(pm_conv_source), PM_ABI_VERSION);
+  PM_REQUIRE(s->kind == PM_SRC_BN_RELU || s->kind == PM_SRC_CONCAT_UPSAMPLE, PM_EINVAL, "%s: pm_conv_source.kind %d", who, s->kind);
+  PM_REQUIRE(wino && pm_is_f32(x), PM_EUNSUPPORTED,
+             "%s: a pm_conv_source is served by the fp32 Winograd input transform alone -- pm_conv_fwd on that route, or pm_conv_bwd_weight reading the V it kept (not this call)", who);
+  if (s->kind == PM_SRC_BN_RELU) {
+    PM_REQUIRE(s->mean && s->invstd && s->gamma && s->beta && pm_aligned16(s->mean) && pm_aligned16(s->invstd) && pm_aligned16(s->gamma) && pm_aligned16(s->beta), PM_EINVAL,
+               "%s: a bn-relu source needs 16-byte aligned mean / invstd / gamma / beta", who);
+  } else {
+    PM_REQUIRE(s->low && pm_aligned16(s->low) && s->low_h >= 1 && s->low_w >= 1 && s->low_pitch % 4 == 0 && s->split > 0 && s->split < x->c &&
+                   s->low_pitch >= x->c - s->split && (int64_t)x->n * s->low_h * s->low_w * s->low_pitch < (1ll << 29),
+               PM_EINVAL, "%s: a concat-upsample source needs a 16-byte aligned low-resolution tensor of x->c - split channels and 0 < split < x->c", who);
+    PM_REQUIRE(s->split % 4 == 0, PM_EUNSUPPORTED, "%s: the channel boundary %d of a concat-upsample source is not a multiple of the transform's vector width (4)", who, s->split);
+  }
   return PM_OK;
 }
 
@@ -507,12 +527,13 @@
 inline size_t wino_ws(const WinoPlan& wp) { return wp.v_bytes + wp.m_bytes + wp.u_bytes; }
 
 int wino_conv(const pm_tensor* xin, const float* w, int w_cout, int w_cin, bool dgrad, const pm_tensor* yout, const WinoPlan& wp,
-              const pm_conv_epilogue& ep, void* ws, hipStream_t st, float* v_keep = nullptr, float* u_ext = nullptr, bool u_valid = false) {
+              const pm_conv_epilogue& ep, void* ws, hipStream_t st, float* v_keep = nullptr, float* u_ext = nullptr, bool u_valid = false,
+              const pm_conv_source* src = nullptr) {
   float* V = v_keep ? v_keep : (float*)ws;
   float* Mo = (float*)((char*)ws + wp.v_bytes);
   float* U = u_ext ? u_ext : (float*)((char*)ws + wp.v_bytes + wp.m_bytes);
   const int cout = yout->c;
-  if (int e = pm_wino_input_xf((const float*)xin->ptr, xin->pitch, xin->c, wp.Kp, wp.g, V, st)) return e;
+  if (int e = pm_wino_input_xf((const float*)xin->ptr, xin->pitch, xin->c, wp.Kp, wp.g, V, st, src)) return e;
   if (!(u_ext && u_valid))
     if (int e = pm_wino_filter_xf(w, w_cout, w_cin, wp.Kp, dgrad, wp.g.m, U, st)) return e;
   const pm_tensor xv = {V, 1, 1, (int32_t)wp.g.tiles, wp.Kp, wp.Kp};
@@ -1175,6 +1196,7 @@
   if (ep) e0 = *ep;
   PM_REQUIRE((e0.scale == nullptr) == (e0.shift == nullptr), PM_EINVAL, "conv_fwd: scale and shift go together");
   const ConvRoute r = route_conv(MODE_FWD, x, y, p);
+  if (int e = check_source("conv_fwd", p->source, x, r.kind == R_WINO)) return e;
   if (e0.bn_partials) {
     PM_REQUIRE(!e0.relu && !e0.residual, PM_EINVAL, "conv_fwd: bn_partials are the statistics of the convolution output (no residual / ReLU)");
     PM_REQUIRE(r.bn_bytes != 0 && (size_t)e0.bn_partials_bytes >= r.bn_bytes, PM_EINVAL, "conv_fwd: this call cannot emit bn_partials (ask pm_conv_bn_partials_bytes): %zu needed", r.bn_bytes);
@@ -1185,7 +1207,7 @@
     case R_WINO: {
       float* keep = (p->wino_v && (size_t)p->wino_v_bytes >= r.wino.v_bytes) ? (float*)p->wino_v : nullptr;
       float* uext = (p->wxf && (size_t)p->wxf_bytes >= r.wino.u_bytes) ? (float*)p->wxf : nullptr;
-      return wino_conv(x, w, y->c, x->c, false, y, r.wino, e0, ws, st, keep, uext, p->wxf_valid != 0);
+      return wino_conv(x, w, y->c, x->c, false, y, r.wino, e0, ws, st, keep, uext, p->wxf_valid != 0, p->source);
     }
     case R_BF16: {
       char* wext = (p->wxf && (size_t)p->wxf_bytes >= r.b16.wb_bytes) ? (char*)p->wxf : nullptr;
@@ -1210,6 +1232,7 @@
   PM_REQUIRE(!add || (add->ptr && pm_same_shape(add, dx) && add->dtype == dx->dtype), PM_EINVAL, "conv_bwd_data: `add` must match dx (shape and dtype)");
   PM_REQUIRE(!add || !pm_is_bf16(add) || pm_vec8(add), PM_EINVAL, "conv_bwd_data: bf16 `add` must be 16B aligned with pitch %% 8 == 0");
   PM_REQUIRE(w && pm_aligned16(w), PM_EINVAL, "conv_bwd_data: weight null or unaligned");
+  if (int e = check_source("conv_bwd_data", p->source, dy, false)) return e;
   const ConvRoute r = route_conv(MODE_DGRAD, dx, dy, p);
   PM_REQUIRE(ws_bytes >= r.ws_bytes && (ws || r.ws_bytes == 0), PM_EWORKSPACE, "conv_bwd_data: workspace %zu < %zu", ws_bytes, r.ws_bytes);
   if (add_mask) {
@@ -1241,6 +1264,7 @@
   const pm_conv_params* p = &tp;
   PM_REQUIRE(dw && pm_aligned16(dw), PM_EINVAL, "conv_bwd_weight: dw null or unaligned");
   const ConvRoute r = route_conv(MODE_WGRAD, x0, dy0, p);
+  if (int e = check_source("conv_bwd_weight", p->source, x0, r.kind == R_WINO_WGRAD && p->wino_v && (size_t)p->wino_v_bytes >= r.wino.v_bytes)) return e;
   PM_REQUIRE(ws && ws_bytes >= r.ws_bytes, PM_EWORKSPACE, "conv_bwd_weight: workspace %zu < %zu", ws_bytes, r.ws_bytes);
   hipStream_t st = (hipStream_t)stream;
   const pm_tensor *x = x0, *dy = dy0;
diff --git a/pinthememory_amd/csrc/pm_common.h b/pinthememory_amd/csrc/pm_common.h
--- a/pinthememory_amd/csrc/pm_common.h
+++ b/pinthememory_amd/csrc/pm_common.h
@@ -43,7 +43,7 @@
   long tiles;
 };
 pm_wino_geom pm_wino_make_geom(int n, int h, int w, int d, int m);
-int pm_wino_input_xf(const float* x, long pitch, int C, int Kp, const pm_wino_geom& g, float* V, hipStream_t st);
+int pm_wino_input_xf(const float* x, long pitch, int C, int Kp, const pm_wino_geom& g, float* V, hipStream_t st, const pm_conv_source* src = nullptr);
 int pm_wino_filter_xf(const float* w, int Cout, int Cin, int Kp, bool dgrad, int m, float* U, hipStream_t st);
 int pm_wino_filter_xf_multi(const float* const* w, float* const* U, const int* cout, const int* cin, const int* kp, const int* m, int n, hipStream_t st);
 int pm_wino_output_xf(const float* M, int Cout, const pm_wino_geom& g, float* y, long ypitch, const float* bias, const float* scale, const float* shift,
diff --git a/pinthememory_amd/csrc/winograd.hip b/pinthememory_amd/csrc/winograd.hip
--- a/pinthememory_amd/csrc/winograd.hip
+++ b/pinthememory_amd/csrc/winograd.hip
@@ -108,6 +108,108 @@
   return t;
 }
 
+struct SrcNoLine {};
+struct SrcBnRelu {
+  const float* x;
+  long xp;
+  const float *mean, *invstd, *gamma, *beta;
+  template <int W>
+  struct Ch {
+    Vec<W> sc, sh;
+  };
+  template <int W>
+  __device__ __forceinline__ Ch<W> channels(int c, bool ok) const {
+    Ch<W> r;
+    r.sc = r.sh = vzero<W>();
+    if (ok) {
+      const Vec<W> mu = vload<W>(mean + c), is = vload<W>(invstd + c), ga = vload<W>(gamma + c), be = vload<W>(beta + c);
+#pragma unroll
+      for (int e = 0; e < W; ++e) r.sc.v[e] = is.v[e] * ga.v[e], r.sh.v[e] = fmaf(-mu.v[e], r.sc.v[e], be.v[e]);
+    }
+    return r;
+  }
+  using Row = SrcNoLine;
+  using Col = SrcNoLine;
+  __device__ __forceinline__ Row row(int, int) const { return {}; }
+  __device__ __forceinline__ Col col(int) const { return {}; }
+  template <int W>
+  using Raw = Vec<W>;
+  template <int W>
+  __device__ __forceinline__ Raw<W> load(const Row&, const Col&, int n, int yy, int xx, int c, const pm_wino_geom& g) const {
+    return vload<W>(x + ((long)(n * g.H + yy) * g.W + xx) * xp + c);
+  }
+  template <int W>
+  __device__ __forceinline__ Vec<W> value(const Ch<W>& ch, const Row&, const Col&, Raw<W> v, int) const {
+#pragma unroll
+    for (int e = 0; e < W; ++e) v.v[e] = fmaxf(fmaf(v.v[e], ch.sc.v[e], ch.sh.v[e]), 0.f);
+    return v;
+  }
+};
+struct SrcConcatUp {
+  const float* x;
+  long xp;
+  const float* low;
+  long lp;
+  int h, w, split;
+  float sy, sx;
+  template <int W>
+  struct Ch {};
+  template <int W>
+  __device__ __forceinline__ Ch<W> channels(int, bool) const {
+    return {};
+  }
+  struct Line {
+    int o0, o1;
+    float w0, w1;
+  };
+  using Row = Line;
+  using Col = Line;
+  __device__ __forceinline__ Row row(int n, int yy) const {
+    const pm_lerp l = lerp(sy, yy, h);
+    return {(int)((n * h + l.i0) * w * lp), (int)((n * h + l.i1) * w * lp), l.w0, l.w1};
+  }
+  __device__ __forceinline__ Col col(int xx) const {
+    const pm_lerp l = lerp(sx, xx, w);
+    return {(int)(l.i0 * lp), (int)(l.i1 * lp), l.w0, l.w1};
+  }
+  template <int W>
+  struct Raw {
+    Vec<W> a, b, c, d;
+  };
+  template <int W>
+  __device__ __forceinline__ Raw<W> load(const Row& ly, const Col& lx, int n, int yy, int xx, int c, const pm_wino_geom& g) const {
+    Raw<W> r{};
+    if (c < split) {
+      r.a = vload<W>(x + ((long)(n * g.H + yy) * g.W + xx) * xp + c);
+    } else {
+      const float* p = low + (c - split);
+      r.a = vload<W>(p + (ly.o0 + lx.o0)), r.b = vload<W>(p + (ly.o0 + lx.o1)), r.c = vload<W>(p + (ly.o1 + lx.o0)), r.d = vload<W>(p + (ly.o1 + lx.o1));
+    }
+    return r;
+  }
+  template <int W>
+  __device__ __forceinline__ Vec<W> value(const Ch<W>&, const Row& ly, const Col& lx, const Raw<W>& r, int c) const {
+    const Vec<W>&a = r.a, &b = r.b, &cc = r.c, &d = r.d;
+    Vec<W> o;
+#pragma unroll
+    for (int e = 0; e < W; ++e) {
+      const float top = fmaf(lx.w1, b.v[e], lx.w0 * a.v[e]), bot = fmaf(lx.w0, cc.v[e], lx.w1 * d.v[e]);
+      o.v[e] = c < split ? a.v[e] : fmaf(ly.w0, top, ly.w1 * bot);
+    }
+    return o;
+  }
+  static __device__ __forceinline__ pm_lerp lerp(float scale, int dst, int in) {
+    pm_lerp r;
+    r.i0 = min((int)(scale * (float)dst), in - 1);
+    r.i1 = r.i0 + (r.i0 < in - 1 ? 1 : 0);
+    float l1 = fmaf(scale, (float)dst, -(float)r.i0);
+    if (l1 < 0.f) l1 = 0.f;
+    if (l1 > 1.f) l1 = 1.f;
+    r.w1 = l1, r.w0 = 1.f - l1;
+    return r;
+  }
+};
+
 template <int MT, int W>
 __global__ __launch_bounds__(256) void wino_input_kernel(const float* __restrict__ x, long xp, int C, int Kp, const pm_wino_geom g, float* __restrict__ V) {
   constexpr int A = MT + 2;
@@ -129,6 +231,52 @@
       for (int a = 0; a < A; ++a) {
         const int yy = t.ry + g.d * (MT * t.ty + a - 1);
         col[a] = (xok && (unsigned)yy < (unsigned)g.H) ? vload<W>(x + ((long)(t.n * g.H + yy) * g.W + xx) * xp + c) : vzero<W>();
+      }
+      mat_apply<MT, W_BT>(col, o);
+#pragma unroll
+      for (int a = 0; a < A; ++a) tt[a][b] = o[a];
+    }
+    float* out = V + (long)tile * Kp + c;
+#pragma unroll
+    for (int a = 0; a < A; ++a) {
+      Vec<W> o[A];
+      mat_apply<MT, W_BT>(tt[a], o);
+#pragma unroll
+      for (int b = 0; b < A; ++b) vstore<W>(out + (a * A + b) * plane, o[b]);
+    }
+  }
+}
+
+template <int MT, int W, typename SRC>
+__global__ __launch_bounds__(256) void wino_input_src_kernel(const SRC src, int C, int Kp, const pm_wino_geom g, float* __restrict__ V) {
+  constexpr int A = MT + 2;
+  const unsigned kg = Kp / W;
+  const unsigned total = (unsigned)g.tiles * kg;
+  const long plane = g.tiles * (long)Kp;
+  for (unsigned i = blockIdx.x * 256u + threadIdx.x; i < total; i += gridDim.x * 256u) {
+    const unsigned tile = i / kg;
+    const int c = (int)(i - tile * kg) * W;
+    const TileId t = decode_tile(tile, g);
+    const bool cok = c < C;
+    const auto ch = src.template channels<W>(c, cok);
+    typename SRC::Row rows[A];
+#pragma unroll
+    for (int a = 0; a < A; ++a) rows[a] = src.row(t.n, t.ry + g.d * (MT * t.ty + a - 1));
+    Vec<W> tt[A][A];
+#pragma unroll
+    for (int b = 0; b < A; ++b) {
+      const int xx = t.rx + g.d * (MT * t.tx + b - 1);
+      const bool xok = cok && (unsigned)xx < (unsigned)g.W;
+      const typename SRC::Col cl = src.col(xx);
+      Vec<W> col[A], o[A];
+#pragma unroll
+      for (int a = 0; a < A; ++a) {
+        const int yy = t.ry + g.d * (MT * t.ty + a - 1);
+        const bool ok = xok && (unsigned)yy < (unsigned)g.H;
+        typename SRC::template Raw<W> raw{};
+        if (ok) raw = src.template load<W>(rows[a], cl, t.n, yy, xx, c, g);
+        const Vec<W> v = src.template value<W>(ch, rows[a], cl, raw, c);
+        col[a] = ok ? v : vzero<W>();
       }
       mat_apply<MT, W_BT>(col, o);
 #pragma unroll
@@ -505,7 +653,18 @@
   return g;
 }
 
-int pm_wino_input_xf(const float* x, long pitch, int C, int Kp, const pm_wino_geom& g, float* V, hipStream_t st) {
+template <typename SRC>
+int wino_input_src(const SRC& s, int C, int Kp, const pm_wino_geom& g, float* V, hipStream_t st) {
+  if (g.m == 4) hipLaunchKernelGGL((wino_input_src_kernel<4, 2, SRC>), dim3(nblocks(g.tiles * (Kp / 2))), dim3(256), 0, st, s, C, Kp, g, V);
+  else hipLaunchKernelGGL((wino_input_src_kernel<2, 4, SRC>), dim3(nblocks(g.tiles * (Kp / 4))), dim3(256), 0, st, s, C, Kp, g, V);
+  return pm_check_launch("wino_input");
+}
+
+int pm_wino_input_xf(const float* x, long pitch, int C, int Kp, const pm_wino_geom& g, float* V, hipStream_t st, const pm_conv_source* src) {
+  if (src && src->kind == PM_SRC_BN_RELU) return wino_input_src(SrcBnRelu{x, pitch, src->mean, src->invstd, src->gamma, src->beta}, C, Kp, g, V, st);
+  if (src && src->kind == PM_SRC_CONCAT_UPSAMPLE)
+    return wino_input_src(SrcConcatUp{x, pitch, src->low, (long)src->low_pitch, src->low_h, src->low_w, src->split, pm_ac_scale(src->low_h, g.H), pm_ac_scale(src->low_w, g.W)},
+                          C, Kp, g, V, st);
   if (g.m == 4) hipLaunchKernelGGL((wino_input_kernel<4, 2>), dim3(nblocks(g.tiles * (Kp / 2))), dim3(256), 0, st, x, pitch, C, Kp, g, V);
   else hipLaunchKernelGGL((wino_input_kernel<2, 4>), dim3(nblocks(g.tiles * (Kp / 4))), dim3(256), 0, st, x, pitch, C, Kp, g, V);
   return pm_check_launch("wino_input");
diff --git a/pinthememory_amd/hip/kernels.py b/pinthememory_amd/hip/kernels.py
--- a/pinthememory_amd/hip/kernels.py
+++ b/pinthememory_amd/hip/kernels.py
@@ -234,17 +234,49 @@
     return _XFORM_COUNT[0]
 
 
-def conv_fwd(x, w_krsc, stride, pad, dil, bias=None, scale=None, shift=None, residual=None, relu=False, out=None, keep_v=None, bn_partials=None, out_dtype=None):
+def conv_source_ok(x_shape, w_krsc, stride, pad, dil, like):
+    cout, kh, kw, cin = w_krsc.shape
+    if CONV_PREC != 0 or ACT_DTYPE != torch.float32 or like.dtype != torch.float32 or kh != 3:
+        return False
+    n, h, w_, c = x_shape
+    ho, wo = conv_out_hw(h, w_, kh, stride, pad, dil)
+    key = ('s', tuple(x_shape), tuple(w_krsc.shape), stride, pad, dil, _GEN[0])
+
+    def ask():
+        xd = L.PmTensor(like.data_ptr(), n, h, w_, c, c, L.PM_F32, 0)
+        yd = L.PmTensor(like.data_ptr(), n, ho, wo, cout, cout, L.PM_F32, 0)
+        p = L.conv_params(kh, kw, stride, pad, dil, CONV_PREC)
+        return _lib().pm_conv_winograd_v_bytes(byref(xd), byref(yd), byref(p)) > 0
+    return _sizes(key, ask)
+
+
+def _conv_source(x, source):
+    if source is None:
+        return None, x.shape[3]
+    if source[0] == 'concat_upsample':
+        low = source[1]
+        assert low.shape[0] == x.shape[0] and low.dtype == torch.float32
+        return L.conv_source_concat_upsample(low, x.shape[3]), x.shape[3] + low.shape[3]
+    assert source[0] == 'bn_relu'
+    return L.conv_source_bn_relu(*source[1:]), x.shape[3]
+
+
+def conv_fwd(x, w_krsc, stride, pad, dil, bias=None, scale=None, shift=None, residual=None, relu=False, out=None, keep_v=None, bn_partials=None, out_dtype=None,
+             source=None):
     cout, kh, kw, cin = w_krsc.shape
     n, h, w_, c = x.shape
+    src, c = _conv_source(x, source)
     assert c == cin, 'conv: Cin mismatch %d vs %d' % (c, cin)
     ho, wo = conv_out_hw(h, w_, kh, stride, pad, dil)
     y = out if out is not None else new((n, ho, wo, cout), x, pitch_pad=True, dtype=out_dtype if out_dtype is not None else ACT_DTYPE)
     assert residual is None or residual.dtype == y.dtype, 'conv_fwd: the fused residual has the dtype of the output'
     xd, yd = tdesc(x), tdesc(y)
+    xd.c = c
     p = L.conv_params(kh, kw, stride, pad, dil, CONV_PREC)
-    lib = _lib()
-    nbv, nbu, nb, npb = _sizes(('f', x.shape, x.stride(), x.dtype, xd.flags, w_krsc.shape, y.stride(), y.dtype, stride, pad, dil, CONV_PREC, _GEN[0]),
+    if src is not None:
+        p.source = ctypes.pointer(src)
+    lib = _lib()
+    nbv, nbu, nb, npb = _sizes(('f', x.shape, x.stride(), x.dtype, xd.flags, c, w_krsc.shape, y.stride(), y.dtype, stride, pad, dil, CONV_PREC, _GEN[0]),
                                lambda: (lib.pm_conv_winograd_v_bytes(byref(xd), byref(yd), byref(p)), lib.pm_conv_wxf_bytes(byref(xd), byref(yd), byref(p)),
                                         lib.pm_conv_workspace(byref(xd), byref(yd), byref(p), 0), lib.pm_conv_bn_partials_bytes(byref(xd), byref(yd), byref(p))))
     if keep_v is not None:
@@ -297,16 +329,19 @@
     return dx
 
 
-def conv_bwd_weight(x, dy, w_shape_krsc, stride, pad, dil, want_bias=False, wino_v=None, on_stream=None):
+def conv_bwd_weight(x, dy, w_shape_krsc, stride, pad, dil, want_bias=False, wino_v=None, on_stream=None, source=None):
     cout, kh, kw, cin = w_shape_krsc
     dw = torch.empty(w_shape_krsc, dtype=torch.float32, device=x.device)
     db = torch.empty(cout, dtype=torch.float32, device=x.device) if want_bias else None
     xd, dyd = tdesc(x), tdesc(dy)
     p = L.conv_params(kh, kw, stride, pad, dil, CONV_PREC)
+    src, xd.c = _conv_source(x, source)
+    if src is not None:
+        p.source = ctypes.pointer(src)
     if wino_v is not None:
         p.wino_v, p.wino_v_bytes = wino_v.data_ptr(), wino_v.numel() * 4
     lib = _lib()
-    nb = _sizes(('w', x.shape, x.stride(), x.dtype, dy.shape, dy.stride(), dy.dtype, w_shape_krsc, stride, pad, dil, CONV_PREC, wino_v is not None, _GEN[0]),
+    nb = _sizes(('w', x.shape, x.stride(), x.dtype, xd.c, dy.shape, dy.stride(), dy.dtype, w_shape_krsc, stride, pad, dil, CONV_PREC, wino_v is not None, _GEN[0]),
                 lambda: lib.pm_conv_workspace(byref(xd), byref(dyd), byref(p), 2))
     raw = stream() if on_stream is None else on_stream.cuda_stream
     ws = workspace(nb, x.device, on_stream)
diff --git a/pinthememory_amd/hip/lib.py b/pinthememory_amd/hip/lib.py
--- a/pinthememory_amd/hip/lib.py
+++ b/pinthememory_amd/hip/lib.py
@@ -25,10 +25,18 @@
                 ('dgrad', c_int32), ('reserved', c_int32)]
 
 
+class PmConvSource(ctypes.Structure):
+    _fields_ = [('struct_size', c_int32), ('kind', c_int32), ('mean', c_void_p), ('invstd', c_void_p), ('gamma', c_void_p), ('beta', c_void_p),
+                ('low', c_void_p), ('low_pitch', c_int64), ('low_h', c_int32), ('low_w', c_int32), ('split', c_int32), ('reserved', c_int32)]
+
+
+PM_SRC_BN_RELU, PM_SRC_CONCAT_UPSAMPLE = 1, 2
+
+
 class PmConvParams(ctypes.Structure):
     _fields_ = [('struct_size', c_int32), ('kh', c_int32), ('kw', c_int32), ('stride', c_int32), ('pad', c_int32), ('dil', c_int32), ('prec', c_int32),
                 ('wino_v', c_void_p), ('wino_v_bytes', c_int64),
-                ('wxf', c_void_p), ('wxf_bytes', c_int64), ('wxf_valid', c_int32)]
+                ('wxf', c_void_p), ('wxf_bytes', c_int64), ('wxf_valid', c_int32), ('source', POINTER(PmConvSource))]
 
 
 class PmRouting(ctypes.Structure):
@@ -50,11 +58,20 @@
     return PmConvParams(ctypes.sizeof(PmConvParams), kh, kw, stride, pad, dil, prec)
 
 
+def conv_source_bn_relu(mean, invstd, gamma, beta):
+    return PmConvSource(ctypes.sizeof(PmConvSource), PM_SRC_BN_RELU, mean.data_ptr(), invstd.data_ptr(), gamma.data_ptr(), beta.data_ptr())
+
+
+def conv_source_concat_upsample(low, split):
+    d = tdesc(low)
+    return PmConvSource(ctypes.sizeof(PmConvSource), PM_SRC_CONCAT_UPSAMPLE, None, None, None, None, d.ptr, d.pitch, d.h, d.w, split)
+
+
 def conv_epilogue(*fields):
     return PmConvEpilogue(ctypes.sizeof(PmConvEpilogue), *fields)
 
 
-ABI_VERSION = 410
+ABI_VERSION = 420
 
 
 class PinmemError(RuntimeError):
diff --git a/pinthememory_amd/hip/ops.py b/pinthememory_amd/hip/ops.py
--- a/pinthememory_amd/hip/ops.py
+++ b/pinthememory_amd/hip/ops.py
@@ -130,14 +130,14 @@
     return (p, True) if p is not None else (weight, False)
 
 
-def _wgrad(x, dy, wshape, geom, want_bias=False, deferred=False, wino_v=None):
+def _wgrad(x, dy, wshape, geom, want_bias=False, deferred=False, wino_v=None, source=None):
     if not deferred:
-        return K.conv_bwd_weight(x, dy, wshape, *geom, want_bias=want_bias, wino_v=wino_v)
+        return K.conv_bwd_weight(x, dy, wshape, *geom, want_bias=want_bias, wino_v=wino_v, source=source)
     side, main = _side_stream(), L.stream_obj()
     ev = torch.cuda.Event()
     ev.record(main)
     side.wait_event(ev)
-    out = K.conv_bwd_weight(x, dy, wshape, *geom, want_bias=want_bias, wino_v=wino_v, on_stream=side)
+    out = K.conv_bwd_weight(x, dy, wshape, *geom, want_bias=want_bias, wino_v=wino_v, on_stream=side, source=source)
     if wino_v is not None:
         wino_v.record_stream(side)
     x.record_stream(side)
@@ -239,6 +239,13 @@
     return (K.bn_bwd_apply_mask(dv, mask, y, mean, invstd, gamma, S.total(0), S.count(y)), *S.grads(0))
 
 
+CONV_SOURCES = True
+
+
+def _source_ok(shape, like, w_krsc, geom):
+    return CONV_SOURCES and K.KEEP_WINOGRAD_V and like.dtype == torch.float32 and K.conv_source_ok(tuple(shape), w_krsc, *geom, like)
+
+
 class _Bottleneck(torch.autograd.Function):
 
     @staticmethod
@@ -247,9 +254,14 @@
         k1, k2, k3 = K.krsc(w1), K.krsc(w2), K.krsc(w3)
         ps = []
         y1 = K.conv_fwd(xv, k1, *geoms[0], bn_partials=ps)
-        o1, m1, i1 = _bn_train_fwd(y1, g1, b1, bns[0], None, True, partials=ps[0])
         kv = []
-        y2 = K.conv_fwd(o1, k2, *geoms[1], keep_v=kv, bn_partials=ps)
+        if _source_ok(y1.shape, y1, k2, geoms[1]):
+            m1, i1 = _bn_train_stats(y1, bns[0], ps[0])
+            o1 = None
+            y2 = K.conv_fwd(y1, k2, *geoms[1], keep_v=kv, bn_partials=ps, source=('bn_relu', m1, i1, g1, b1))
+        else:
+            o1, m1, i1 = _bn_train_fwd(y1, g1, b1, bns[0], None, True, partials=ps[0])
+            y2 = K.conv_fwd(o1, k2, *geoms[1], keep_v=kv, bn_partials=ps)
         o2, m2, i2 = _bn_train_fwd(y2, g2, b2, bns[1], None, True, partials=ps[1])
         y3 = K.conv_fwd(o2, k3, *geoms[2], bn_partials=ps)
         m3 = None
@@ -297,8 +309,11 @@
         dw3, _ = _wgrad(o2, dy3, tuple(k3.shape), ge[2], deferred=df[2])
         do2 = K.conv_bwd_data(dy3, k3, tuple(o2.shape), *ge[2])
         dy2, _, dg2, db2 = _bn_train_bwd(do2, o2, y2, m2, i2, g2, b2, True, gr[1], False, False)
-        dw2, _ = _wgrad(o1, dy2, tuple(k2.shape), ge[1], deferred=df[1], wino_v=v2)
-        do1 = K.conv_bwd_data(dy2, k2, tuple(o1.shape), *ge[1])
+        if o1 is None:
+            dw2, _ = _wgrad(y1, dy2, tuple(k2.shape), ge[1], deferred=df[1], wino_v=v2, source=('bn_relu', m1, i1, g1, b1))
+        else:
+            dw2, _ = _wgrad(o1, dy2, tuple(k2.shape), ge[1], deferred=df[1], wino_v=v2)
+        do1 = K.conv_bwd_data(dy2, k2, tuple(y1.shape), *ge[1])
         dy1, _, dg1, db1 = _bn_train_bwd(do1, o1, y1, m1, i1, g1, b1, True, gr[0], False, False)
         dw1, _ = _wgrad(xv, dy1, tuple(k1.shape), ge[0], deferred=df[0])
         dwd = dgd = dbd = None
@@ -420,6 +435,35 @@
         return dx, dw, db, dgamma, dbeta, (nchw(dres) if dres is not None else None), None, None, None, None, None
 
 
+class _Decoder(torch.autograd.Function):
+
+    @staticmethod
+    def forward(ctx, x, w0, g0, b0, w1, g1, b1, geoms, bns, deferred):
+        xv = nhwc(x)
+        k0, k1 = K.krsc(w0), K.krsc(w1)
+        kv0, kv1, ps = [], [], []
+        y0 = K.conv_fwd(xv, k0, *geoms[0], keep_v=kv0, bn_partials=ps)
+        m0, i0 = _bn_train_stats(y0, bns[0], ps[0])
+        y1 = K.conv_fwd(y0, k1, *geoms[1], keep_v=kv1, bn_partials=ps, source=('bn_relu', m0, i0, g0, b0))
+        o1, m1, i1 = _bn_train_fwd(y1, g1, b1, bns[1], None, True, partials=ps[1])
+        ctx.geoms, ctx.groups, ctx.deferred = geoms, [b.group for b in bns], deferred
+        ctx.save_for_backward(xv, k0, k1, y0, y1, m0, i0, m1, i1, g0, b0, g1, b1, kv0[0], kv1[0])
+        return nchw(o1)
+
+    @staticmethod
+    def backward(ctx, dout):
+        xv, k0, k1, y0, y1, m0, i0, m1, i1, g0, b0, g1, b1, v0, v1 = ctx.saved_tensors
+        ge, gr, df = ctx.geoms, ctx.groups, ctx.deferred
+        dy1, _, dg1, db1 = _bn_train_bwd(_grad_view(dout), None, y1, m1, i1, g1, b1, True, gr[1], False, False)
+        dw1, _ = _wgrad(y0, dy1, tuple(k1.shape), ge[1], deferred=df[1], wino_v=v1, source=('bn_relu', m0, i0, g0, b0))
+        do0 = K.conv_bwd_data(dy1, k1, tuple(y0.shape), *ge[1])
+        dy0, _, dg0, db0 = _bn_train_bwd(do0, None, y0, m0, i0, g0, b0, True, gr[0], False, False)
+        dw0, _ = _wgrad(xv, dy0, tuple(k0.shape), ge[0], deferred=df[0], wino_v=v0)
+        dx = nchw(K.conv_bwd_data(dy0, k0, tuple(xv.shape), *ge[0], dtype=xv.dtype)) if ctx.needs_input_grad[0] else None
+        p = lambda d: d.permute(0, 3, 1, 2)
+        return dx, p(dw0), dg0, db0, p(dw1), dg1, db1, None, None, None
+
+
 class _Stem(torch.autograd.Function):
 
     @staticmethod
@@ -730,6 +774,16 @@
                              ws[2][0], blk.bn3.weight, blk.bn3.bias, wd, gd, bd, geoms, bns, [d for _, d in ws] + [False])
 
 
+def decoder_convs(x, final1):
+    c0, bn0, c1, bn1 = final1[0], final1[1], final1[3], final1[4]
+    ok = (bn0.training and bn1.training and torch.is_grad_enabled() and x.dtype == torch.float32 and c0.bias is None and c1.bias is None
+          and _source_ok((x.shape[0], x.shape[2], x.shape[3], c0.out_channels), x, K.krsc(c1.weight), _geom(c1)))
+    if not ok:
+        return conv_bn_act(conv_bn_act(x, c0, bn0, relu=True), c1, bn1, relu=True)
+    (w0, d0), (w1, d1) = _w(c0.weight), _w(c1.weight)
+    return _Decoder.apply(x, w0, bn0.weight, bn0.bias, w1, bn1.weight, bn1.bias, [_geom(c0), _geom(c1)], [BNState(bn0), BNState(bn1)], [d0, d1])
+
+
 def conv(x, conv_mod):
     return _Conv.apply(x, conv_mod.weight, conv_mod.bias, _geom(conv_mod))
 
diff --git a/pinthememory_amd/network/deepv3plus.py b/pinthememory_amd/network/deepv3plus.py
--- a/pinthememory_amd/network/deepv3plus.py
+++ b/pinthememory_amd/network/deepv3plus.py
@@ -208,8 +208,7 @@
         dec0_fine = run_cbr(self.bot_fine, low_level, out=buf[:, :48])
         dec0_up = ops.resize(dec0_up, low_level.size()[2:], out=buf[:, 48:])
         dec0 = ops.concat(buf, [dec0_fine, dec0_up])
-        dec1 = ops.conv_bn_act(dec0, self.final1[0], self.final1[1], relu=True)
-        dec1 = ops.conv_bn_act(dec1, self.final1[3], self.final1[4], relu=True)
+        dec1 = ops.decoder_convs(dec0, self.final1)
         dec2 = ops.conv(dec1, self.final2[0])
         return self._finish(dec2, x_size, aux_out, gts, aux_gts, mem_output, writeloss, readloss, inter_feature)
 
```
